# creare-com/pydem

Measured on AMD Instinct MI355X. Metric: Mcells/s (slope+aspect+UCA+TWI end-to-end) per tile; % HBM roofline, higher is better.
Workload: dtype f64

## Files before the change

include/pydem_hip.h:

```cpp
#ifndef PYDEM_HIP_H
#define PYDEM_HIP_H

#include <stdint.h>

#ifdef __cplusplus
extern "C" {
#endif

typedef struct pydem_tile pydem_tile;

enum pydem_field {
    PYDEM_ELEV = 0,
    PYDEM_MAG = 1,
    PYDEM_DIRECTION = 2,
    PYDEM_FLATS = 3,
    PYDEM_SECTION = 4,
    PYDEM_PROPORTION = 5,
    PYDEM_UCA = 6,
    PYDEM_TWI = 7,
    PYDEM_EDGE_TODO = 8,
    PYDEM_EDGE_DONE = 9,
    PYDEM_WEIGHT = 10,
    PYDEM_UCA_WEIGHTED = 11,
    PYDEM_FIELD_COUNT = 12
};

enum pydem_dtype { PYDEM_F64 = 0, PYDEM_F32 = 1, PYDEM_I16 = 2, PYDEM_I32 = 3, PYDEM_U8 = 4, PYDEM_I8 = 5 };

typedef struct pydem_options {
    int32_t drain_pits;
    int32_t drain_pits_min_border;
    int32_t drain_pits_max_iter;
    int32_t drain_pits_max_dist;
    double  drain_pits_max_dist_XY;
    int32_t apply_uca_limit_edges;
    int32_t apply_twi_limits;
    int32_t apply_twi_limits_on_uca;
    int32_t circular_ref_maxcount;
    double  uca_saturation_limit;
    double  twi_min_slope;
    double  twi_min_area;
} pydem_options;

typedef struct pydem_timings {
    double slopes_directions_ms;
    double stencil_kernel_ms;
    double flats_ms;
    double graph_ms;
    double pits_ms;
    double sweep_ms;
    double twi_ms;
    int64_t sweep_rounds;
    int64_t sweep_kernel_launches;
    int64_t n_flats;
    int64_t n_pit_edges;
    int64_t n_pits_undrained;
    int64_t n_unresolved;
    int64_t sweep_tile_passes;
    int64_t n_pits;
    int64_t n_pits_row;
    int64_t n_pits_wave;
    int64_t n_pits_big;
    double uca_weighted_ms;
} pydem_timings;

const char *pydem_hip_last_error(void);
int pydem_hip_device_count(int *count);
int pydem_hip_device_name(int device, char *buf, int buflen);
int pydem_hip_device_memory(int device, int64_t *free_bytes, int64_t *total_bytes);

int pydem_hip_release_scratch(void);

int pydem_tile_create(int64_t n_rows, int64_t n_cols, int device, pydem_tile **out);
int pydem_tile_destroy(pydem_tile *t);
int pydem_tile_set_spacing(pydem_tile *t, const double *dX, const double *dY,
                           const double *dX2, const double *dY2);
int pydem_tile_upload(pydem_tile *t, int field, const void *src, int dtype);
int pydem_tile_download(pydem_tile *t, int field, void *dst);
int pydem_tile_get_line(pydem_tile *t, int field, int axis, int64_t index, void *dst);
int pydem_tile_set_line(pydem_tile *t, int field, int axis, int64_t index, const void *src);
int pydem_tile_get_lines(pydem_tile *t, int count, const int *fields, const int *axes, const int64_t *indices,
                         void *const *dsts);
int pydem_tile_synchronize(pydem_tile *t);
int pydem_tile_timings(pydem_tile *t, pydem_timings *out);
int64_t pydem_tile_device_bytes(pydem_tile *t);

int pydem_tile_synth_fractal(pydem_tile *t, uint32_t seed, int64_t row0, int64_t col0,
                             int n_octaves, int top_shift, double zmin, double zrange);

int pydem_fill_flats(pydem_tile *t, double max_pit_area, int below_sea, double source_tol, int peaks, int pits, int artefacts_only,
                     int *needs_host);
int pydem_pit_candidates(pydem_tile *t, int below_sea, int64_t *npits);
int pydem_pit_candidates_read(pydem_tile *t, int64_t npits, int32_t *cells, double *elev);
int pydem_pit_paths(pydem_tile *t, const int32_t *order, int64_t npits, int max_iter, int max_dist, double max_dist_XY,
                    int64_t *n_failed, int64_t *iter_used, int64_t *rounds, int *needs_host);
int pydem_slopes_directions(pydem_tile *t);
int pydem_find_flats(pydem_tile *t);
int pydem_uca(pydem_tile *t, pydem_options *opt);
int pydem_uca_weighted(pydem_tile *t, pydem_options *opt, int scale_by_cell_area);
int pydem_build_graph(pydem_tile *t, pydem_options *opt);
int pydem_uca_edge_update(pydem_tile *t, pydem_options *opt,
                          const double *const data[4], const uint8_t *const done[4],
                          const uint8_t *const todo[4]);
int pydem_uca_edge_round_inc(pydem_tile *t, pydem_options *opt,
                             const double *const data[4], const uint8_t *const done[4],
                             const uint8_t *const todo[4]);
int pydem_uca_edge_round_inc_dev(pydem_tile *t, pydem_options *opt);
int pydem_uca_edge_flush(pydem_tile *t);
int pydem_twi(pydem_tile *t, pydem_options *opt);

int pydem_tile_pit_edges(pydem_tile *t, int64_t *n, int32_t *src, int32_t *dst, double *w);

int pydem_tile_graph_words(pydem_tile *t, uint32_t *out);

int pydem_tile_restore_pit_slopes(pydem_tile *t);

int pydem_bench_stencil(pydem_tile *t, int iters, double *avg_ms);

int pydem_drain_area(double *area, uint8_t *done, uint8_t *ids, const int32_t *col_indptr, const int32_t *col_indices,
                     const double *col_data, const int32_t *row_indptr, const int32_t *row_indices, int64_t n_rows,
                     int64_t n_cols, double *edge_todo, double *edge_todo_no_mask, int skip_edge, int device);
int pydem_drain_connections(uint8_t *arr, uint8_t *ids, const int32_t *indptr, const int32_t *indices, int64_t n,
                            uint8_t set_to, int device);

typedef struct pydem_comm pydem_comm;
int pydem_comm_unique_id(char *out128);
int pydem_comm_create(int world, int rank, const char *uid128, int device, pydem_comm **out);
int pydem_comm_destroy(pydem_comm *c);
int pydem_comm_begin(pydem_comm *c, int64_t n_doubles);
int pydem_comm_pack_line(pydem_comm *c, pydem_tile *t, int field, int axis, int64_t index, int64_t offset);
int pydem_comm_pack_lines(pydem_comm *c, pydem_tile *t, int count, const int *fields, const int *axes, const int64_t *indices,
                          const int64_t *offsets);
int pydem_comm_put(pydem_comm *c, const double *host_in, int64_t n_doubles, int64_t offset);
int pydem_comm_allreduce(pydem_comm *c, int64_t n_doubles, int op , double *host_out);

typedef struct pydem_board pydem_board;
int pydem_board_create(int device, int n_tiles, int64_t n_doubles, pydem_board **out);
int pydem_board_destroy(pydem_board *b);
int pydem_board_set_desc(pydem_board *b, int index, int32_t n, int32_t m, const int64_t *offsets28, const int32_t *flags8,
                         pydem_tile *tile);
int pydem_board_set_lines(pydem_board *b, int index, int64_t mb_start, int64_t size, pydem_tile *tile, int count,
                          const int *fields, const int *axes, const int64_t *indices, const int64_t *rel_offsets);
int pydem_board_refresh(pydem_board *b, pydem_comm *c, int n_wave, const int *wave_tiles);
int pydem_board_refresh_stage(pydem_board *b, int n_wave, const int *wave_tiles, double *host_out, int64_t cap, int64_t *n_doubles);
int pydem_board_refresh_unstage(pydem_board *b, int n_wave, const int *wave_tiles, const double *host_in, int64_t n_doubles);
int pydem_board_eval(pydem_board *b, int count, const int *tiles, const int *full, unsigned long long *out);
int pydem_board_run_waves(pydem_board *b, pydem_comm *c, int k_waves, unsigned long long *state, unsigned long long *scal_out);
typedef int (*pydem_exchange_fn)(void *ctx, int op, void *buf, int64_t n);
int pydem_board_prepare_waves(pydem_board *b, int staged, unsigned long long ok_tiles);
int pydem_board_run_waves_ex(pydem_board *b, pydem_comm *c, int k_waves, unsigned long long *state, unsigned long long *scal_out,
                             pydem_exchange_fn exchange, void *ctx);
int pydem_comm_count(pydem_comm *c, int *count);
int pydem_tile_edge_queue_ready(pydem_tile *t);
int pydem_board_download(pydem_board *b, double *out);

int pydem_cond_pit_artifacts(const double *elev, int64_t n_rows, int64_t n_cols, const int32_t *lab, int32_t nlab,
                             double max_area, int f32 , uint8_t *raise);
int pydem_cond_fill_flats(const double *data, double *built, int64_t n_rows, int64_t n_cols, const int32_t *lab,
                          int32_t nlab, double source_tol, int peaks, int pits);
int pydem_cond_pit_paths(double *elev, int64_t n_rows, int64_t n_cols, const int64_t *pits, int64_t npits,
                         const double *dX, int64_t n_dX, const double *dY, int max_iter, int max_dist,
                         double max_dist_XY, int dtype_mode ,
                         int64_t *n_failed, int64_t *iter_used);

int pydem_tiff_lzw_encode(const uint8_t *src, int64_t n, uint8_t *dst, int64_t cap, int64_t *out_n);

#ifdef __cplusplus
}
#endif
#endif
```

pydem_amd/_ffi.py:

```python
import ctypes as C
import os

import numpy as np

_HERE = os.path.dirname(os.path.abspath(__file__))
LIB_PATH = os.path.join(_HERE, 'lib', 'libpydem_hip.so')

ELEV, MAG, DIRECTION, FLATS, SECTION, PROPORTION, UCA, TWI, EDGE_TODO, EDGE_DONE, WEIGHT, UCA_WEIGHTED = range(12)
FIELD_DTYPE = {ELEV: np.float64, MAG: np.float64, DIRECTION: np.float64, FLATS: np.uint8,
               SECTION: np.int8, PROPORTION: np.float64, UCA: np.float64, TWI: np.float64,
               EDGE_TODO: np.uint8, EDGE_DONE: np.uint8, WEIGHT: np.float64, UCA_WEIGHTED: np.float64}
_DTYPES = {np.dtype('float64'): 0, np.dtype('float32'): 1, np.dtype('int16'): 2, np.dtype('int32'): 3,
           np.dtype('uint8'): 4, np.dtype('int8'): 5, np.dtype('bool'): 4}


class Options(C.Structure):
    _fields_ = [('drain_pits', C.c_int32), ('drain_pits_min_border', C.c_int32),
                ('drain_pits_max_iter', C.c_int32), ('drain_pits_max_dist', C.c_int32),
                ('drain_pits_max_dist_XY', C.c_double), ('apply_uca_limit_edges', C.c_int32),
                ('apply_twi_limits', C.c_int32), ('apply_twi_limits_on_uca', C.c_int32),
                ('circular_ref_maxcount', C.c_int32), ('uca_saturation_limit', C.c_double),
                ('twi_min_slope', C.c_double), ('twi_min_area', C.c_double)]


class Timings(C.Structure):
    _fields_ = [('slopes_directions_ms', C.c_double), ('stencil_kernel_ms', C.c_double),
                ('flats_ms', C.c_double), ('graph_ms', C.c_double), ('pits_ms', C.c_double),
                ('sweep_ms', C.c_double), ('twi_ms', C.c_double), ('sweep_rounds', C.c_int64),
                ('sweep_kernel_launches', C.c_int64), ('n_flats', C.c_int64), ('n_pit_edges', C.c_int64),
                ('n_pits_undrained', C.c_int64), ('n_unresolved', C.c_int64), ('sweep_tile_passes', C.c_int64),
                ('n_pits', C.c_int64), ('n_pits_row', C.c_int64), ('n_pits_wave', C.c_int64), ('n_pits_big', C.c_int64),
                ('uca_weighted_ms', C.c_double)]

    def as_dict(self):
        return {k: getattr(self, k) for k, _ in self._fields_}


_P = C.c_void_p
_PP = C.POINTER(C.c_void_p)
SYMBOLS = {
    'pydem_hip_last_error': (C.c_char_p, []),
    'pydem_hip_device_count': (C.c_int, [C.POINTER(C.c_int)]),
    'pydem_hip_device_memory': (C.c_int, [C.c_int, C.POINTER(C.c_int64), C.POINTER(C.c_int64)]),
    'pydem_hip_release_scratch': (C.c_int, []),
    'pydem_hip_device_name': (C.c_int, [C.c_int, C.c_char_p, C.c_int]),
    'pydem_tile_create': (C.c_int, [C.c_int64, C.c_int64, C.c_int, _PP]),
    'pydem_tile_destroy': (C.c_int, [_P]),
    'pydem_tile_set_spacing': (C.c_int, [_P, _P, _P, _P, _P]),
    'pydem_tile_upload': (C.c_int, [_P, C.c_int, _P, C.c_int]),
    'pydem_tile_download': (C.c_int, [_P, C.c_int, _P]),
    'pydem_tile_get_line': (C.c_int, [_P, C.c_int, C.c_int, C.c_int64, _P]),
    'pydem_tile_set_line': (C.c_int, [_P, C.c_int, C.c_int, C.c_int64, _P]),
    'pydem_tile_get_lines': (C.c_int, [_P, C.c_int, _P, _P, _P, _P]),
    'pydem_cond_pit_artifacts': (C.c_int, [_P, C.c_int64, C.c_int64, _P, C.c_int32, C.c_double, C.c_int, _P]),
    'pydem_cond_fill_flats': (C.c_int, [_P, _P, C.c_int64, C.c_int64, _P, C.c_int32, C.c_double, C.c_int, C.c_int]),
    'pydem_cond_pit_paths': (C.c_int, [_P, C.c_int64, C.c_int64, _P, C.c_int64, _P, C.c_int64, _P, C.c_int, C.c_int,
                                       C.c_double, C.c_int, _P, _P]),
    'pydem_tiff_lzw_encode': (C.c_int, [_P, C.c_int64, _P, C.c_int64, _P]),
    'pydem_tile_synchronize': (C.c_int, [_P]),
    'pydem_tile_timings': (C.c_int, [_P, C.POINTER(Timings)]),
    'pydem_tile_device_bytes': (C.c_int64, [_P]),
    'pydem_tile_synth_fractal': (C.c_int, [_P, C.c_uint32, C.c_int64, C.c_int64, C.c_int, C.c_int,
                                           C.c_double, C.c_double]),
    'pydem_fill_flats': (C.c_int, [_P, C.c_double, C.c_int, C.c_double, C.c_int, C.c_int, C.c_int, _P]),
    'pydem_pit_candidates': (C.c_int, [_P, C.c_int, C.POINTER(C.c_int64)]),
    'pydem_pit_candidates_read': (C.c_int, [_P, C.c_int64, _P, _P]),
    'pydem_pit_paths': (C.c_int, [_P, _P, C.c_int64, C.c_int, C.c_int, C.c_double, C.POINTER(C.c_int64), C.POINTER(C.c_int64), C.POINTER(C.c_int64), _P]),
    'pydem_slopes_directions': (C.c_int, [_P]),
    'pydem_find_flats': (C.c_int, [_P]),
    'pydem_uca': (C.c_int, [_P, C.POINTER(Options)]),
    'pydem_uca_weighted': (C.c_int, [_P, C.POINTER(Options), C.c_int]),
    'pydem_build_graph': (C.c_int, [_P, C.POINTER(Options)]),
    'pydem_uca_edge_update': (C.c_int, [_P, C.POINTER(Options), _PP, _PP, _PP]),
    'pydem_uca_edge_round_inc': (C.c_int, [_P, C.POINTER(Options), _PP, _PP, _PP]),
    'pydem_uca_edge_round_inc_dev': (C.c_int, [_P, C.POINTER(Options)]),
    'pydem_uca_edge_flush': (C.c_int, [_P]),
    'pydem_twi': (C.c_int, [_P, C.POINTER(Options)]),
    'pydem_tile_pit_edges': (C.c_int, [_P, C.POINTER(C.c_int64), _P, _P, _P]),
    'pydem_tile_graph_words': (C.c_int, [_P, _P]),
    'pydem_tile_restore_pit_slopes': (C.c_int, [_P]),
    'pydem_bench_stencil': (C.c_int, [_P, C.c_int, C.POINTER(C.c_double)]),
    'pydem_drain_area': (C.c_int, [_P, _P, _P, _P, _P, _P, _P, _P, C.c_int64, C.c_int64, _P, _P, C.c_int, C.c_int]),
    'pydem_drain_connections': (C.c_int, [_P, _P, _P, _P, C.c_int64, C.c_uint8, C.c_int]),
    'pydem_comm_unique_id': (C.c_int, [C.c_char_p]),
    'pydem_comm_create': (C.c_int, [C.c_int, C.c_int, C.c_char_p, C.c_int, _PP]),
    'pydem_comm_destroy': (C.c_int, [_P]),
    'pydem_comm_begin': (C.c_int, [_P, C.c_int64]),
    'pydem_comm_pack_line': (C.c_int, [_P, _P, C.c_int, C.c_int, C.c_int64, C.c_int64]),
    'pydem_comm_pack_lines': (C.c_int, [_P, _P, C.c_int, _P, _P, _P, _P]),
    'pydem_comm_put': (C.c_int, [_P, _P, C.c_int64, C.c_int64]),
    'pydem_comm_allreduce': (C.c_int, [_P, C.c_int64, C.c_int, _P]),
    'pydem_board_create': (C.c_int, [C.c_int, C.c_int, C.c_int64, _PP]),
    'pydem_board_destroy': (C.c_int, [_P]),
    'pydem_board_set_desc': (C.c_int, [_P, C.c_int, C.c_int32, C.c_int32, _P, _P, _P]),
    'pydem_board_set_lines': (C.c_int, [_P, C.c_int, C.c_int64, C.c_int64, _P, C.c_int, _P, _P, _P, _P]),
    'pydem_board_refresh': (C.c_int, [_P, _P, C.c_int, _P]),
    'pydem_board_refresh_stage': (C.c_int, [_P, C.c_int, _P, _P, C.c_int64, _P]),
    'pydem_board_refresh_unstage': (C.c_int, [_P, C.c_int, _P, _P, C.c_int64]),
    'pydem_board_eval': (C.c_int, [_P, C.c_int, _P, _P, _P]),
    'pydem_board_download': (C.c_int, [_P, _P]),
    'pydem_board_run_waves': (C.c_int, [_P, _P, C.c_int, _P, _P]),
    'pydem_board_prepare_waves': (C.c_int, [_P, C.c_int, C.c_uint64]),
    'pydem_board_run_waves_ex': (C.c_int, [_P, _P, C.c_int, _P, _P, _P, _P]),
    'pydem_comm_count': (C.c_int, [_P, _P]),
    'pydem_tile_edge_queue_ready': (C.c_int, [_P]),
}

_lib = None


def load():
    global _lib
    if _lib is None:
        if not os.path.exists(LIB_PATH):
            raise RuntimeError("libpydem_hip.so is not built (%s); run `python -m pydem_amd.build`. "
                               "There is no CPU fallback." % LIB_PATH)
        lib = C.CDLL(LIB_PATH)
        for name, (res, args) in SYMBOLS.items():
            fn = getattr(lib, name)
            fn.restype = res
            fn.argtypes = args
        _lib = lib
    return _lib


class HipError(RuntimeError):
    pass


def check(rc):
    if rc != 0:
        raise HipError("libpydem_hip error %d: %s" % (rc, load().pydem_hip_last_error().decode()))


def device_count():
    n = C.c_int(0)
    check(load().pydem_hip_device_count(C.byref(n)))
    return n.value


def release_scratch():
    check(load().pydem_hip_release_scratch())


def device_memory(device=0):
    f, tot = C.c_int64(0), C.c_int64(0)
    check(load().pydem_hip_device_memory(int(device), C.byref(f), C.byref(tot)))
    return f.value, tot.value


class Tile(object):

    def __init__(self, n_rows, n_cols, device=0):
        self.lib = load()
        self.shape = (int(n_rows), int(n_cols))
        self._h = C.c_void_p()
        check(self.lib.pydem_tile_create(n_rows, n_cols, device, C.byref(self._h)))

    def close(self):
        if self._h:
            self.lib.pydem_tile_destroy(self._h)
            self._h = C.c_void_p()

    def __del__(self):
        try:
            self.close()
        except Exception:
            pass

    def set_spacing(self, dX, dY, dX2, dY2):
        arrs = [np.ascontiguousarray(a, np.float64) for a in (dX, dY, dX2, dY2)]
        n = self.shape[0]
        assert arrs[0].size == n - 1 and arrs[1].size == n - 1 and arrs[2].size == n and arrs[3].size == n
        check(self.lib.pydem_tile_set_spacing(self._h, *[a.ctypes.data_as(_P) for a in arrs]))

    def upload(self, field, arr):
        arr = np.ascontiguousarray(arr)
        if arr.shape != self.shape:
            raise ValueError("field %d: array of shape %r uploaded to a tile of shape %r" % (field, arr.shape, self.shape))
        if FIELD_DTYPE[field] != np.float64:
            arr = np.ascontiguousarray(arr.astype(FIELD_DTYPE[field], copy=False))
            dt = _DTYPES[arr.dtype]
        else:
            if arr.dtype not in _DTYPES or arr.dtype == np.bool_:
                arr = np.ascontiguousarray(arr, np.float64)
            dt = _DTYPES[arr.dtype]
        check(self.lib.pydem_tile_upload(self._h, field, arr.ctypes.data_as(_P), dt))

    def download(self, field):
        out = np.empty(self.shape, FIELD_DTYPE[field])
        check(self.lib.pydem_tile_download(self._h, field, out.ctypes.data_as(_P)))
        return out

    def get_line(self, field, axis, index):
        out = np.empty(self.shape[1] if axis == 0 else self.shape[0], FIELD_DTYPE[field])
        check(self.lib.pydem_tile_get_line(self._h, field, axis, index, out.ctypes.data_as(_P)))
        return out

    def get_lines(self, requests):
        k = len(requests)
        outs = [np.empty(self.shape[1] if axis == 0 else self.shape[0], FIELD_DTYPE[field]) for field, axis, _ in requests]
        fields = (C.c_int * k)(*[r[0] for r in requests])
        axes = (C.c_int * k)(*[r[1] for r in requests])
        idx = (C.c_int64 * k)(*[r[2] for r in requests])
        dsts = (C.c_void_p * k)(*[o.ctypes.data for o in outs])
        check(self.lib.pydem_tile_get_lines(self._h, k, fields, axes, idx, dsts))
        return outs

    def set_line(self, field, axis, index, values):
        v = np.ascontiguousarray(values, FIELD_DTYPE[field])
        assert v.size == (self.shape[1] if axis == 0 else self.shape[0])
        check(self.lib.pydem_tile_set_line(self._h, field, axis, index, v.ctypes.data_as(_P)))

    def synth_fractal(self, seed=0, row0=0, col0=0, n_octaves=12, top_shift=12, zmin=1.0, zrange=1000.0):
        check(self.lib.pydem_tile_synth_fractal(self._h, seed, row0, col0, n_octaves, top_shift, zmin, zrange))

    def slopes_directions(self):
        check(self.lib.pydem_slopes_directions(self._h))

    def find_flats(self):
        check(self.lib.pydem_find_flats(self._h))

    def fill_flats(self, max_pit_area, below_sea, source_tol, peaks, pits, artefacts_only=False):
        flag = C.c_int(0)
        check(self.lib.pydem_fill_flats(self._h, float(max_pit_area or 0.0), int(bool(below_sea)), float(source_tol), int(bool(peaks)),
                                        int(bool(pits)), int(bool(artefacts_only)), C.byref(flag)))
        return flag.value == 0

    def pit_drain_paths(self, below_sea, max_iter, max_dist, max_dist_XY, sort_dtype=None):
        import time
        t0 = time.perf_counter()
        n = C.c_int64(0)
        check(self.lib.pydem_pit_candidates(self._h, int(bool(below_sea)), C.byref(n)))
        if n.value < 0:
            return None
        cells = np.empty(max(n.value, 1), np.int32); elev = np.empty(max(n.value, 1), np.float64)
        check(self.lib.pydem_pit_candidates_read(self._h, n.value, cells.ctypes.data_as(_P), elev.ctypes.data_as(_P)))
        cells, elev = cells[:n.value], elev[:n.value]
        t1 = time.perf_counter()
        keys = elev if sort_dtype is None or np.dtype(sort_dtype) == np.float64 else elev.astype(sort_dtype)
        order = np.ascontiguousarray(cells[np.argsort(keys)], np.int32)
        t2 = time.perf_counter()
        failed, used, rounds, flag = C.c_int64(0), C.c_int64(0), C.c_int64(0), C.c_int(0)
        check(self.lib.pydem_pit_paths(self._h, order.ctypes.data_as(_P), n.value, int(max_iter), int(max_dist or 0),
                                       float(max_dist_XY) if max_dist_XY else 0.0, C.byref(failed), C.byref(used), C.byref(rounds),
                                       C.byref(flag)))
        if os.environ.get('PYDEM_PATHS_DEBUG'):
            import sys
            sys.stderr.write("pit paths host side: candidates %.1f ms, argsort %.1f ms, pydem_pit_paths %.1f ms\n"
                             % ((t1 - t0) * 1e3, (t2 - t1) * 1e3, (time.perf_counter() - t2) * 1e3))
        if flag.value:
            return None
        return int(failed.value), int(used.value), int(rounds.value)

    def uca(self, opt):
        check(self.lib.pydem_uca(self._h, C.byref(opt)))

    def uca_weighted(self, opt, scale_by_cell_area=True):
        check(self.lib.pydem_uca_weighted(self._h, C.byref(opt), int(bool(scale_by_cell_area))))

    def build_graph(self, opt):
        check(self.lib.pydem_build_graph(self._h, C.byref(opt)))

    def uca_edge_update(self, opt, data, done, todo, incremental=False):
        n, m = self.shape
        lens = (n, n, m, m)
        d = [np.ascontiguousarray(np.asarray(a, np.float64).ravel()) for a in data]
        dn = [np.ascontiguousarray(np.asarray(a).ravel().astype(np.uint8)) for a in done]
        td = [np.ascontiguousarray(np.asarray(a).ravel().astype(np.uint8)) for a in todo]
        for arrs in (d, dn, td):
            assert [a.size for a in arrs] == list(lens), "edge strips must have n_rows / n_cols entries"
        pack = lambda xs: (C.c_void_p * 4)(*[x.ctypes.data_as(C.c_void_p) for x in xs])
        fn = self.lib.pydem_uca_edge_round_inc if incremental else self.lib.pydem_uca_edge_update
        check(fn(self._h, C.byref(opt), pack(d), pack(dn), pack(td)))

    def uca_edge_flush(self):
        check(self.lib.pydem_uca_edge_flush(self._h))

    def edge_queue_ready(self):
        return bool(self.lib.pydem_tile_edge_queue_ready(self._h))

    def uca_edge_round_dev(self, opt):
        check(self.lib.pydem_uca_edge_round_inc_dev(self._h, C.byref(opt)))

    def twi(self, opt):
        check(self.lib.pydem_twi(self._h, C.byref(opt)))

    def graph_words(self):
        out = np.empty(self.shape, np.uint32)
        check(self.lib.pydem_tile_graph_words(self._h, out.ctypes.data_as(_P)))
        return out

    def pit_edges(self):
        n = C.c_int64(0)
        check(self.lib.pydem_tile_pit_edges(self._h, C.byref(n), None, None, None))
        src = np.empty(n.value, np.int32); dst = np.empty(n.value, np.int32); w = np.empty(n.value, np.float64)
        if n.value:
            check(self.lib.pydem_tile_pit_edges(self._h, C.byref(n), src.ctypes.data_as(_P), dst.ctypes.data_as(_P),
                                                w.ctypes.data_as(_P)))
        return src, dst, w

    def restore_pit_slopes(self):
        check(self.lib.pydem_tile_restore_pit_slopes(self._h))

    def bench_stencil(self, iters):
        ms = C.c_double(0)
        check(self.lib.pydem_bench_stencil(self._h, iters, C.byref(ms)))
        return ms.value

    def synchronize(self):
        check(self.lib.pydem_tile_synchronize(self._h))

    def timings(self):
        tm = Timings()
        check(self.lib.pydem_tile_timings(self._h, C.byref(tm)))
        return tm.as_dict()

    def device_bytes(self):
        return self.lib.pydem_tile_device_bytes(self._h)


class Board(object):

    def __init__(self, device, n_tiles, n_doubles):
        self.lib = load()
        self.n_tiles, self.n_doubles = n_tiles, n_doubles
        self._h = C.c_void_p()
        check(self.lib.pydem_board_create(device, n_tiles, n_doubles, C.byref(self._h)))
        self._out = np.zeros((n_tiles, 8), np.uint64)

    def close(self):
        if self._h:
            self.lib.pydem_board_destroy(self._h)
            self._h = C.c_void_p()

# ... 124 lines not shown
```

pydem_amd/csrc/ccl.h:

```cpp
#pragma once

#define RLX_LOAD(p) __hip_atomic_load((p), __ATOMIC_RELAXED, __HIP_MEMORY_SCOPE_AGENT)

__global__ __launch_bounds__(256) void k_compact_flats(const uint8_t *__restrict__ flat0, int64_t NN,
                                                       int32_t *__restrict__ list, int32_t *__restrict__ count)
{
    __shared__ int32_t wave_tot[4][4];
    __shared__ int32_t blk_base;
    const int lane = threadIdx.x & 63, wave = threadIdx.x >> 6;
    for (int64_t base = (int64_t)blockIdx.x * 65536; base < NN; base += (int64_t)gridDim.x * 65536) {
        unsigned long long bits[4];
        int32_t mine[4], incl[4];
#pragma unroll
        for (int j = 0; j < 4; j++) {
            const int64_t c0 = base + j * 16384 + (int64_t)threadIdx.x * 64;
            bits[j] = 0;
            if (c0 + 64 <= NN) {
                uint4 v[4];
#pragma unroll
                for (int q = 0; q < 4; q++) v[q] = *reinterpret_cast<const uint4 *>(flat0 + c0 + 16 * q);
#pragma unroll
                for (int q = 0; q < 4; q++) {
                    const uint32_t w[4] = {v[q].x, v[q].y, v[q].z, v[q].w};
#pragma unroll
                    for (int k = 0; k < 16; k++)
                        bits[j] |= (unsigned long long)(((w[k >> 2] >> (8 * (k & 3))) & 0xffu) ? 1u : 0u) << (16 * q + k);
                }
            } else {
                for (int k = 0; k < 64; k++)
                    if (c0 + k < NN && flat0[c0 + k]) bits[j] |= 1ull << k;
            }
            mine[j] = __popcll(bits[j]);
            incl[j] = mine[j];
#pragma unroll
            for (int off = 1; off < 64; off <<= 1) {
                const int32_t o = __shfl_up(incl[j], off);
                if (lane >= off) incl[j] += o;
            }
            if (lane == 63) wave_tot[j][wave] = incl[j];
        }
        __syncthreads();
        if (threadIdx.x == 0) {
            int32_t tot = 0;
            for (int j = 0; j < 4; j++) for (int k = 0; k < 4; k++) tot += wave_tot[j][k];
            blk_base = tot ? atomicAdd(count, tot) : 0;
        }
        __syncthreads();
        int32_t off = blk_base;
#pragma unroll
        for (int j = 0; j < 4; j++) {
            int32_t o = off + incl[j] - mine[j];
            for (int k = 0; k < wave; k++) o += wave_tot[j][k];
            const int64_t c0 = base + j * 16384 + (int64_t)threadIdx.x * 64;
            unsigned long long b = bits[j];
            while (b) {
                const int k = __ffsll((long long)b) - 1;
                b &= b - 1;
                list[o++] = (int32_t)(c0 + k);
            }
            off += wave_tot[j][0] + wave_tot[j][1] + wave_tot[j][2] + wave_tot[j][3];
        }
        __syncthreads();
    }
}

__global__ void k_label_init(const int32_t *__restrict__ list, const int32_t *__restrict__ count, int32_t *labels, int m)
{
    const int32_t nf = *count;
    const int lane = threadIdx.x & 63;
    for (int32_t q = blockIdx.x * blockDim.x + threadIdx.x;; q += gridDim.x * blockDim.x) {
        const bool valid = q < nf;
        if (!__ballot(valid)) break;
        const int32_t c = valid ? list[q] : -1;
        const int32_t prev = __shfl_up(c, 1);
        const bool head = lane == 0 || !valid || prev != c - 1 || c % m == 0;
        const unsigned long long heads = __ballot(head);
        const int s = 63 - __clzll((long long)(heads & ((2ull << lane) - 1ull)));
        const int32_t start = __shfl(c, s);
        if (valid) labels[c] = start;
    }
}

__device__ __forceinline__ int32_t uf_find(int32_t *L, int32_t x)
{
    const int32_t x0 = x;
    int32_t p = RLX_LOAD(&L[x]);
    int hops = 0;
    while (p != x) { x = p; p = RLX_LOAD(&L[x]); hops++; }
    if (hops >= 2) atomicMin(&L[x0], x);
    return x;
}

__device__ __forceinline__ void uf_union(int32_t *L, int32_t a, int32_t b)
{
    for (;;) {
        a = uf_find(L, a);
        b = uf_find(L, b);
        if (a == b) return;
        if (a > b) { const int32_t t = a; a = b; b = t; }
        const int32_t old = atomicMin(&L[b], a);
        if (old == b) return;
        b = old;
    }
}

__global__ void k_label_union(const int32_t *__restrict__ list, const int32_t *__restrict__ count,
                              const uint8_t *__restrict__ flat0, int32_t *labels, int n, int m)
{
    const int32_t nf = *count;
    for (int32_t q = blockIdx.x * blockDim.x + threadIdx.x; q < nf; q += gridDim.x * blockDim.x) {
        const int32_t c = list[q];
        const int i = c / m, j = c - i * m;
        if (j + 1 < m && flat0[c + 1]) uf_union(labels, c, c + 1);
        if (i + 1 < n) {
            if (j > 0 && flat0[c + m - 1]) uf_union(labels, c, c + m - 1);
            if (flat0[c + m]) uf_union(labels, c, c + m);
            if (j + 1 < m && flat0[c + m + 1]) uf_union(labels, c, c + m + 1);
        }
    }
}

__global__ void k_label_flatten(const int32_t *__restrict__ list, const int32_t *__restrict__ count, int32_t *labels)
{
    const int32_t nf = *count;
    for (int32_t q = blockIdx.x * blockDim.x + threadIdx.x; q < nf; q += gridDim.x * blockDim.x) {
        const int32_t c = list[q];
        const int32_t r = uf_find(labels, c);
        if (r != c) __hip_atomic_store(&labels[c], r, __ATOMIC_RELAXED, __HIP_MEMORY_SCOPE_AGENT);
    }
}
```

pydem_amd/csrc/flats.hip:

```cpp
#include "internal.h"

namespace {

#include "ccl.h"

__global__ void k_flats_extend(const int32_t *__restrict__ list, const int32_t *__restrict__ count,
                               const uint8_t *__restrict__ flat0, const int32_t *__restrict__ labels,
                               const double *__restrict__ elev, uint8_t *__restrict__ flats, int n, int m)
{
    const int32_t nf = *count;
    for (int32_t q = blockIdx.x * blockDim.x + threadIdx.x; q < nf * 8; q += gridDim.x * blockDim.x) {
        const int32_t c = list[q >> 3];
        int d = q & 7;
        d += (d >= 4);
        const int i = c / m + d / 3 - 1, j = c % m + d % 3 - 1;
        if (i < 0 || i >= n || j < 0 || j >= m) continue;
        const int32_t J = i * m + j;
        if (!flat0[J] && !(elev[J] == elev[labels[c]])) continue;
        int32_t best = -1;
        for (int dd = 0; dd < 9; dd++) {
            if (dd == 4) continue;
            const int ii = i + dd / 3 - 1, jj = j + dd % 3 - 1;
            if (ii < 0 || ii >= n || jj < 0 || jj >= m) continue;
            const int32_t nb = ii * m + jj;
            if (flat0[nb]) { const int32_t r = labels[nb]; best = r > best ? r : best; }
        }
        flats[J] = (elev[J] == elev[best]);
    }
}

__global__ void k_flats_patch(const int32_t *__restrict__ list, const int32_t *__restrict__ count,
                              const uint8_t *__restrict__ flats, double *__restrict__ mag, double *__restrict__ dir,
                              int n, int m)
{
    const int32_t nf = *count;
    for (int32_t q = blockIdx.x * blockDim.x + threadIdx.x; q < nf * 9; q += gridDim.x * blockDim.x) {
        const int32_t c = list[q / 9];
        const int d = q % 9;
        const int i = c / m + d / 3 - 1, j = c % m + d % 3 - 1;
        if (i < 0 || i >= n || j < 0 || j >= m) continue;
        const int32_t J = i * m + j;
        if (flats[J]) { mag[J] = -1.0; dir[J] = -1.0; }
    }
}

__global__ __launch_bounds__(256) void k_count_flats(const uint8_t *__restrict__ flats, int64_t NN, int32_t *count)
{
    int32_t local = 0;
    const int64_t nvec = NN >> 4, stride = (int64_t)gridDim.x * blockDim.x, t0 = (int64_t)blockIdx.x * blockDim.x + threadIdx.x;
    for (int64_t v = t0; v < nvec; v += stride) {
        const uint4 f4 = reinterpret_cast<const uint4 *>(flats)[v];
        const uint32_t fw[4] = {f4.x, f4.y, f4.z, f4.w};
#pragma unroll
        for (int q = 0; q < 4; q++)
#pragma unroll
            for (int b = 0; b < 4; b++) local += ((fw[q] >> (8 * b)) & 0xFFu) != 0;
    }
    for (int64_t c = (nvec << 4) + t0; c < NN; c += stride) local += flats[c] != 0;
    for (int off = 32; off > 0; off >>= 1) local += __shfl_down(local, off);
    __shared__ int32_t s_w[4];
    if ((threadIdx.x & 63) == 0) s_w[threadIdx.x >> 6] = local;
    __syncthreads();
    if (threadIdx.x == 0) { const int32_t tot = s_w[0] + s_w[1] + s_w[2] + s_w[3]; if (tot) atomicAdd(count, tot); }
}

}

int stage_flats(pydem_tile *t)
{
    const int n = (int)t->n, m = (int)t->m;
    PYDEM_TRY(tile_alloc(t, &t->labels, (size_t)t->NN));
    PYDEM_TRY(tile_alloc(t, &t->flatlist, (size_t)t->NN));
    HIP_TRY(hipEventRecord(t->ev[3], t->stream));
    HIP_TRY(hipMemsetAsync(t->counters, 0, 64 * sizeof(int32_t), t->stream));
    int32_t *cnt = t->counters;
    const int big = (int)(cdiv(t->NN, 256) < 4096 ? cdiv(t->NN, 256) : 4096);
    hipLaunchKernelGGL(k_compact_flats, dim3(big), dim3(256), 0, t->stream, t->flat0, t->NN, t->flatlist, cnt);
    HIP_TRY(hipMemcpyAsync(t->flats, t->flat0, (size_t)t->NN, hipMemcpyDeviceToDevice, t->stream));
    HIP_TRY(hipMemcpyAsync(t->h_counters, cnt, sizeof(int32_t), hipMemcpyDeviceToHost, t->stream));
    HIP_TRY(hipStreamSynchronize(t->stream));
    const int32_t nf = t->h_counters[0];
    if (nf > 0) {
        const int g1 = (int)(cdiv(nf, 256) < 2048 ? cdiv(nf, 256) : 2048);
        const int g8 = (int)(cdiv((int64_t)nf * 9, 256) < 4096 ? cdiv((int64_t)nf * 9, 256) : 4096);
        hipLaunchKernelGGL(k_label_init, dim3(g1), dim3(256), 0, t->stream, t->flatlist, cnt, t->labels, m);
        hipLaunchKernelGGL(k_label_union, dim3(g1), dim3(256), 0, t->stream, t->flatlist, cnt, t->flat0, t->labels, n, m);
        hipLaunchKernelGGL(k_label_flatten, dim3(g1), dim3(256), 0, t->stream, t->flatlist, cnt, t->labels);
        hipLaunchKernelGGL(k_flats_extend, dim3(g8), dim3(256), 0, t->stream, t->flatlist, cnt, t->flat0, t->labels,
                           t->elev, t->flats, n, m);
        hipLaunchKernelGGL(k_flats_patch, dim3(g8), dim3(256), 0, t->stream, t->flatlist, cnt, t->flats, t->mag, t->dir, n, m);
    }
    hipLaunchKernelGGL(k_count_flats, dim3(big), dim3(256), 0, t->stream, t->flats, t->NN, cnt + 1);
    HIP_TRY(hipMemcpyAsync(t->h_counters, cnt, 2 * sizeof(int32_t), hipMemcpyDeviceToHost, t->stream));
    HIP_TRY(hipEventRecord(t->ev[4], t->stream));
    HIP_TRY(hipGetLastError());
    HIP_TRY(hipEventSynchronize(t->ev[4]));
    float ms = 0;
    HIP_TRY(hipEventElapsedTime(&ms, t->ev[3], t->ev[4]));
    t->tm.flats_ms = ms;
    t->tm.n_flats = t->h_counters[1];
    return 0;
}
```

pydem_amd/csrc/internal.h:

```cpp
#pragma once
#include <hip/hip_runtime.h>
#include <stdint.h>
#include <stdio.h>
#include <string>
#include <vector>
#include <utility>
#include <initializer_list>
#include "../../include/pydem_hip.h"

void pydem_set_error(const char *fmt, ...);
#define HIP_TRY(expr)                                                                          \
    do {                                                                                       \
        hipError_t e_ = (expr);                                                                \
        if (e_ != hipSuccess) {                                                                \
            pydem_set_error("%s:%d: %s -> %s", __FILE__, __LINE__, #expr, hipGetErrorString(e_)); \
            return -1;                                                                         \
        }                                                                                      \
    } while (0)
#define PYDEM_TRY(expr)            \
    do {                           \
        int r_ = (expr);           \
        if (r_ != 0) return r_;    \
    } while (0)

__host__ __device__ constexpr int fe1r(int k) { return k == 1 || k == 2 ? -1 : (k == 5 || k == 6 ? 1 : 0); }
__host__ __device__ constexpr int fe1c(int k) { return k == 0 || k == 7 ? 1 : (k == 3 || k == 4 ? -1 : 0); }
__host__ __device__ constexpr int fe2r(int k) { return k <= 3 ? -1 : 1; }
__host__ __device__ constexpr int fe2c(int k) { return (k == 0 || k == 1 || k == 6 || k == 7) ? 1 : -1; }

struct RowTab {
    double dX, dY;
    double hyp;
    double thA;
    double thB;
    double rdX, rdY, rhyp;
};

struct PitGraph {
    int32_t *raw_src = nullptr, *raw_dst = nullptr; double *raw_w = nullptr;
    int64_t raw_cap = 0, n_raw = 0;
    int64_t n_edges = 0, sorted_cap = 0;
    int32_t *src = nullptr, *dst = nullptr; double *w = nullptr;
    int32_t *in_src = nullptr, *in_dst = nullptr; double *in_w = nullptr;
    void *sort_buf = nullptr; size_t sort_bytes = 0;
};

struct pydem_tile {
    int64_t n = 0, m = 0, NN = 0;
    int device = 0;
    hipStream_t stream = nullptr;
    hipStream_t stream2 = nullptr;
    hipEvent_t ev_fork = nullptr, ev_join = nullptr, ev_snap = nullptr;
    hipEvent_t ev[8] = {};
    double *elev = nullptr, *mag = nullptr, *dir = nullptr, *prop = nullptr, *uca = nullptr, *twi = nullptr;
    double *weight = nullptr, *uca_w = nullptr;
    uint8_t *flats = nullptr, *edge_todo = nullptr, *edge_done = nullptr, *flat0 = nullptr;
    int8_t *section = nullptr;
    bool have[PYDEM_FIELD_COUNT] = {};
    double *dX = nullptr, *dY = nullptr, *dX2 = nullptr, *dY2 = nullptr;
    RowTab *rowtab = nullptr;
    double *sec_theta = nullptr;
    double *row_area = nullptr;
    std::vector<double> h_dX, h_dY, h_dX2, h_dY2;
    bool spacing_set = false;
    int stencil_exact_only = 0;
    bool elev_f32 = false;
    int elev_dtype = 0;
    uint8_t *inmask = nullptr, *gflags = nullptr, *todo_work = nullptr;
    double *contrib = nullptr;
    int32_t *indeg = nullptr, *queue[2] = {nullptr, nullptr}, *labels = nullptr, *flatlist = nullptr;
    int32_t *counters = nullptr;
    int32_t *h_counters = nullptr;
    PitGraph pits;
    int32_t *estamp = nullptr; double *edelta = nullptr, *p_delta = nullptr, *s_data = nullptr;
    uint8_t *p_flags = nullptr, *s_flags = nullptr;
    int32_t eepoch = 0;
    int32_t *eseed = nullptr;
    bool edge_clean = false;
    bool einc_compact = false;
    void *nd_rec = nullptr; int64_t nd_cap = 0; int32_t nd = 0;
    int64_t circular_cells = -1;
    int64_t einc_round = 0;
    bool einc_ready = false;
    std::vector<std::pair<int, int64_t>> watch;
    size_t watch_built = 0;
    bool cond_live = false;
    bool cond_pending = false;
    int32_t cond_nw = 0, cond_nan_cap = 0;
    void *cond_mem = nullptr; size_t cond_bytes = 0;
    void *cond_node = nullptr, *cond_edge = nullptr; double *cond_slot = nullptr;
    int32_t *cond_q0 = nullptr, *cond_q1 = nullptr, *cond_nanq = nullptr, *cond_cnt = nullptr;
    void *cb_mem[3] = {nullptr, nullptr, nullptr}; size_t cb_bytes[3] = {0, 0, 0};
    double *h_strip_d = nullptr; uint8_t *h_strip_f = nullptr; size_t h_strip_cap = 0;
    void *h_stage = nullptr; size_t h_stage_bytes = 0;
    int32_t etodo_prev = 0;
    double *line_stage = nullptr;
    void *lines_stage = nullptr; int lines_cap = 0;
    bool graph_valid = false;
    pydem_options graph_opt = {};
    void *scratch = nullptr; size_t scratch_bytes = 0;
    int64_t device_bytes = 0;
    pydem_timings tm = {};
};

template <typename T>
int tile_alloc(pydem_tile *t, T **p, size_t count);

struct ArenaLease {
    int device = -1;
    void *arena = nullptr;
    char *base = nullptr; size_t bytes = 0, off = 0, want = 0;
    std::vector<void *> extra;
    bool held = false;
    ~ArenaLease();
};
int arena_acquire(int device, ArenaLease *L);
void *arena_take(ArenaLease *L, size_t bytes);

int ensure_fields(pydem_tile *t, std::initializer_list<int> fields);
void *plane_take(int device, size_t bytes);
void plane_give(int device, void *q);
hipError_t dev_malloc(void **p, size_t bytes);
int tile_pinned(pydem_tile *t, size_t bytes, void **out);

int stage_stencil(pydem_tile *t);
int stage_flats(pydem_tile *t);
int stage_section_graph(pydem_tile *t, const pydem_options *opt);
int stage_pits(pydem_tile *t, const pydem_options *opt);
int stage_sweep(pydem_tile *t, const pydem_options *opt);
int stage_uca_weighted(pydem_tile *t, const pydem_options *opt, int scale_by_cell_area);
int stage_twi(pydem_tile *t, const pydem_options *opt);
int stage_edge_update(pydem_tile *t, const pydem_options *opt, const double *const data[4], const uint8_t *const done[4],
                      const uint8_t *const todo[4]);
int stage_edge_round_inc(pydem_tile *t, const pydem_options *opt, const double *const data[4], const uint8_t *const done[4],
                         const uint8_t *const todo[4]);
int stage_edge_flush(pydem_tile *t);
int stage_edge_catchup(pydem_tile *t);
bool tile_edge_queue_ready(const pydem_tile *t);
size_t tile_edge_queue_desc_bytes();
int tile_edge_queue_desc(pydem_tile *t, void *out, const unsigned long long *gate, int bit, const unsigned long long *round_base,
                         const unsigned long long *round_add, int64_t *nper);
int stage_edge_rounds_queued(hipStream_t s, const void *d_q, int count, int64_t max_nper);
unsigned long long tile_edge_round_counter(const pydem_tile *t);
void tile_edge_rounds_ran(pydem_tile *t, int waves);
void tile_watch_line(pydem_tile *t, int axis, int64_t index);
bool tile_line_watched(const pydem_tile *t, int axis, int64_t index);
int stage_fill_flats(pydem_tile *t, double max_pit_area, int below_sea, double source_tol, int peaks, int pits, int artefacts_only);
int stage_pit_candidates(pydem_tile *t, int below_sea, int64_t *npits);
int stage_pit_candidates_read(pydem_tile *t, int64_t npits, int32_t *cells, double *elev);
int stage_pit_paths(pydem_tile *t, const int32_t *order_host, int64_t npits, int max_iter, int max_dist, double max_dist_XY,
                    int64_t *n_failed, int64_t *iter_used, int64_t *rounds_out, int dtype_mode);
int stage_synth(pydem_tile *t, uint32_t seed, int64_t row0, int64_t col0, int n_oct, int top_shift,
                double zmin, double zrange);
int bench_stencil(pydem_tile *t, int iters, double *avg_ms);

static inline int64_t cdiv(int64_t a, int64_t b) { return (a + b - 1) / b; }
```

pydem_amd/csrc/pits.hip:

```cpp
#include "internal.h"
#include <hipcub/hipcub.hpp>
#include <math.h>
#include <stdlib.h>
#include <algorithm>
#include <vector>

namespace {

__device__ __forceinline__ double np_pairwise_leaf(const double *a, int n)
{
    if (n < 8) {
        double res = 0.;
        for (int i = 0; i < n; i++) res += a[i];
        return res;
    }
    double r0 = a[0], r1 = a[1], r2 = a[2], r3 = a[3], r4 = a[4], r5 = a[5], r6 = a[6], r7 = a[7];
    int i;
    for (i = 8; i < n - (n % 8); i += 8) {
        r0 += a[i]; r1 += a[i + 1]; r2 += a[i + 2]; r3 += a[i + 3];
        r4 += a[i + 4]; r5 += a[i + 5]; r6 += a[i + 6]; r7 += a[i + 7];
    }
    double res = ((r0 + r1) + (r2 + r3)) + ((r4 + r5) + (r6 + r7));
    for (; i < n; i++) res += a[i];
    return res;
// ... 733 lines not shown
            const bool in_a = (pos >> 5) == wa;
            const uint32_t wd = in_a ? va : vb;
            if (wd & bit) continue;
            if (nb == LN_B) { over = true; continue; }
            if (in_a) va |= bit; else vb |= bit;
            if (wb == wa) vb = va;
            lp[nb * LN_T] = (uint8_t)pos;
            nb++;
        }
        seen[wa * LN_T] = va;
        if (wb != wa) seen[wb * LN_T] = vb;
    };
    auto fetch_new = [&](int nb0) {
        constexpr int FB = 8;
        for (int base = nb0; base < nb; base += FB) {
            double e8[FB]; uint8_t pm8[FB];
#pragma unroll
            for (int k = 0; k < FB; k++) {
                e8[k] = 0.0; pm8[k] = 0;
                if (base + k < nb) {
                    const int pos = lp[(base + k) * LN_T];
                    const int64_t cell = (int64_t)(r0 + (pos >> 4)) * m + (c0 + (pos & 15));
                    e8[k] = P.elev[cell]; pm8[k] = P.pitmask[cell];
                }
            }
#pragma unroll
            for (int k = 0; k < FB; k++) {
                const int idx = base + k;
                if (idx >= nb) continue;
                le[idx * LN_T] = e8[k];
                if (e8[k] != e8[k]) has_nan = true;
                if (pm8[k]) { pitbits |= 1u << idx; if (e8[k] < epit) has_p = true; }
                else { pitbits &= ~(1u << idx); if (e8[k] < epit_border) has_np = true; }
            }
        }
    };
    const bool prof = P.prof != nullptr;
    long long acc_a = 0, acc_b = 0, acc_c = 0, acc_g = 0, trips = 0, busy = 0;
    for (;;) {
        long long tk0 = 0, tk1 = 0, tk2 = 0, tkg = 0;
        if (prof) tk0 = clock64();
        const unsigned long long idle = __ballot(!running);
        if (idle && more) {
            if (chunk_next == chunk_end) {
                int32_t b = 0;
                if (lane == 0) b = atomicAdd(P.work_next, LN_CHUNK);
                b = __shfl(b, 0);
                chunk_next = b < np ? b : np;
                chunk_end = b + LN_CHUNK < np ? b + LN_CHUNK : np;
                if (chunk_next >= chunk_end) more = false;
            }
            const int avail = chunk_end - chunk_next, want = __popcll(idle);
            const int rank = __popcll(idle & lt);
            if (!running && rank < avail) {
                pit = pits[chunk_next + rank];
                ipit = pit / m; jpit = pit - ipit * m;
                r0 = ipit - LN_W / 2; c0 = jpit - LN_W / 2;
                if (r0 > n - LN_W) r0 = n - LN_W;
                if (c0 > m - LN_W) c0 = m - LN_W;
                if (r0 < 0) r0 = 0;
                if (c0 < 0) c0 = 0;
#pragma unroll
                for (int w = 0; w < 8; w++) seen[w * LN_T] = 0;
                epit = P.elev[pit];
                epit_border = epit;
                nb = 0; pitbits = 0; it = 0;
                has_np = false; has_p = false; has_nan = false; over = false;
                {
                    const int pos = (ipit - r0) * LN_W + (jpit - c0);
                    seen[(pos >> 5) * LN_T] = 1u << (pos & 31);
                    discover(ipit - r0, jpit - c0);
                    fetch_new(0);
                }
                if (P.min_border) {
                    double mn = INFINITY;
                    for (int k = 0; k < nb; k++) mn = min_f64(mn, le[k * LN_T]);
                    if (nb) epit_border = mn;
                    has_np = false;
                }
                running = true;
            }
            chunk_next += want < avail ? want : avail;
        }
        if (!__ballot(running)) { if (more) continue; break; }
        if (prof) { tk1 = clock64(); busy += __popcll(__ballot(running)); trips++; }
        int nd = 0;
        int status = 0;
        double ssum = 0.0;
        if (running && !pending) {
            if (over) pending = 4;
            else if (it >= P.max_iter || nb == 0) pending = 3;
            else if (has_nan) pending = has_p ? 2 : 3;
            else if (has_np) pending = 1;
            else if (has_p) pending = 2;
            else {
                double mn = INFINITY;
                for (int k0 = 0; k0 < nb; k0 += 8) {
                    double v[8];
#pragma unroll
                    for (int i = 0; i < 8; i++) v[i] = k0 + i < nb ? le[(k0 + i) * LN_T] : INFINITY;
#pragma unroll
                    for (int i = 0; i < 8; i++) mn = min_f64(mn, v[i]);
                }
                uint32_t eq = 0;
                for (int k0 = 0; k0 < nb; k0 += 8) {
                    double v[8];
#pragma unroll
                    for (int i = 0; i < 8; i++) v[i] = k0 + i < nb ? le[(k0 + i) * LN_T] : INFINITY;
#pragma unroll
                    for (int i = 0; i < 8; i++) if (k0 + i < nb && v[i] == mn) eq |= 1u << (k0 + i);
                }
                int nq = 0;
                while (eq) {
                    const int k = 31 - __clz((int)eq);
                    eq &= ~(1u << k);
                    lq[nq * LN_T] = lp[k * LN_T]; nq++;
                    nb--;
                    if (k != nb) {
                        le[k * LN_T] = le[nb * LN_T]; lp[k * LN_T] = lp[nb * LN_T];
                        pitbits = (pitbits & ~(1u << k)) | (((pitbits >> nb) & 1u) << k);
                    }
                }
                const int nb0 = nb;
                for (int j = 0; j < nq; j++) { const int pos = lq[j * LN_T]; discover(pos >> 4, pos & 15); }
                fetch_new(nb0);
                it++;
            }
        }
        const unsigned long long waiting = __ballot(pending != 0), growing = __ballot(running && !pending);
        if (prof) { tkg = clock64(); acc_g += tkg - tk1; }
        if (!(__popcll(waiting) >= LN_FIN_BATCH || (waiting && !growing))) continue;
        if (pending) {
            const int mode = pending <= 2 ? pending : 0;
            status = pending == 4 ? 3 : 2;
            if (mode) {
                uint32_t mt = 0;
                for (int k0 = 0; k0 < nb; k0 += 8) {
                    double v[8];
#pragma unroll
                    for (int i = 0; i < 8; i++) v[i] = k0 + i < nb ? le[(k0 + i) * LN_T] : INFINITY;
#pragma unroll
                    for (int i = 0; i < 8; i++) {
                        const bool isp = (pitbits >> (k0 + i)) & 1u;
                        if (k0 + i < nb && (mode == 1 ? (!isp && v[i] < epit_border) : (isp && v[i] < epit))) mt |= 1u << (k0 + i);
                    }
                }
                while (mt) {
                    const int k = __ffs((int)mt) - 1;
                    mt &= mt - 1u;
                    if (k != nd) {
                        const double ek = le[k * LN_T], en = le[nd * LN_T];
                        const uint8_t pk = lp[k * LN_T], pn = lp[nd * LN_T];
                        const uint32_t bk = (pitbits >> k) & 1u, bn = (pitbits >> nd) & 1u;
                        le[k * LN_T] = en; lp[k * LN_T] = pn; le[nd * LN_T] = ek; lp[nd * LN_T] = pk;
                        pitbits = (pitbits & ~((1u << k) | (1u << nd))) | (bn << k) | (bk << nd);
                    }
                    nd++;
                }
                for (int a = 1; a < nd; a++) {
                    const double ea = le[a * LN_T]; const uint8_t pa = lp[a * LN_T]; const uint32_t ba = (pitbits >> a) & 1u;
                    int b = a - 1;
                    while (b >= 0 && lp[b * LN_T] > pa) {
                        le[(b + 1) * LN_T] = le[b * LN_T]; lp[(b + 1) * LN_T] = lp[b * LN_T];
                        pitbits = (pitbits & ~(1u << (b + 1))) | (((pitbits >> b) & 1u) << (b + 1));
                        b--;
                    }
                    le[(b + 1) * LN_T] = ea; lp[(b + 1) * LN_T] = pa;
                    pitbits = (pitbits & ~(1u << (b + 1))) | (ba << (b + 1));
                }
                const int ndX = n - 1;
                const bool xy = !isnan(P.max_dist_XY) && P.max_dist_XY != 0;
                int keep = 0;
                for (int t = 0; t < nd; t++) {
                    const int pos = lp[t * LN_T];
                    const int idr = r0 + (pos >> 4), jdr = c0 + (pos & 15);
                    if (P.max_dist) {
                        const int di = ipit - idr, dj = jpit - jdr;
                        if (!(sqrt((double)(di * di + dj * dj)) <= (double)P.max_dist)) continue;
                    }
                    const int a = ipit < idr ? ipit : idr, b = ipit < idr ? idr : ipit;
                    double dxm;
                    if (ipit == idr) dxm = P.dX[ipit < ndX - 1 ? ipit : ndX - 1];
                    else dxm = np_pairwise_leaf15(P.dX + a, b - a) / (double)(b - a);
                    const double dx = dxm * (double)(jpit - jdr);
                    const double dy = np_pairwise_leaf15(P.dY + a, b - a);
                    const double d = sqrt(dx * dx + dy * dy);
                    if (xy && !(d <= P.max_dist_XY)) continue;
                    le[keep * LN_T] = pit_drop(P, epit, le[t * LN_T]) / d;
                    lp[keep * LN_T] = (uint8_t)pos;
                    keep++;
                }
                nd = keep;
                if (nd > 0) {
                    ssum = np_pairwise_leaf_strided(le, LN_T, nd);
                    P.mag[pit] = ssum / (double)nd;
                    P.flats[pit] = 0;
                    status = 1;
                }
            }
            running = false; pending = 0;
        }
        if (prof) { tk2 = clock64(); acc_a += tk1 - tk0; acc_b += tk2 - tkg; }
        if (!__ballot(status != 0)) continue;
        int incl = nd;
        for (int off = 1; off < 64; off <<= 1) { const int o = __shfl_up(incl, off); if (lane >= off) incl += o; }
        const int tot = __shfl(incl, 63);
        int32_t wbase = 0;
        if (lane == 0 && tot) wbase = atomicAdd(&P.out_count[0], tot);
        wbase = __shfl(wbase, 0);
        if (tot) {
            if ((int64_t)wbase + tot <= P.out_cap) {
                const int32_t o = wbase + incl - nd;
                for (int t = 0; t < nd; t++) {
                    const int pos = lp[t * LN_T];
                    P.out_src[o + t] = pit;
                    P.out_dst[o + t] = (int32_t)((int64_t)(r0 + (pos >> 4)) * m + (c0 + (pos & 15)));
                    P.out_w[o + t] = le[t * LN_T] / ssum;
                }
            } else if (lane == 0) atomicAdd(&P.out_count[3], 1);
        }
        const unsigned long long b_un = __ballot(status == 2), b_ov = __ballot(status == 3);
        if (lane == 0 && b_un) atomicAdd(&P.out_count[1], __popcll(b_un));
        if (b_ov) {
            int32_t obase = 0;
            if (lane == 0) obase = atomicAdd(&P.out_count[4], __popcll(b_ov));
            obase = __shfl(obase, 0);
            if (status == 3) {
                const int32_t slot = obase + __popcll(b_ov & lt);
                P.lane_overflow[slot] = pit;
                if (P.lane_state) {
                for (int k = 0; k < nb; k++) { const int pos = lp[k * LN_T]; seen[(pos >> 5) * LN_T] &= ~(1u << (pos & 31)); }
                uint32_t *rec = P.lane_state + (size_t)slot * 12;
                rec[0] = (uint32_t)it; rec[1] = 0;
                rec[2] = (uint32_t)__double2loint(epit_border); rec[3] = (uint32_t)__double2hiint(epit_border);
#pragma unroll
                for (int w = 0; w < 8; w++) rec[4 + w] = seen[w * LN_T];
                }
            }
        }
        if (prof) acc_c += clock64() - tk2;
    }
    if (prof && lane == 0) {
        atomicAdd(P.prof + 0, (unsigned long long)acc_a); atomicAdd(P.prof + 1, (unsigned long long)acc_b);
        atomicAdd(P.prof + 2, (unsigned long long)acc_c); atomicAdd(P.prof + 3, (unsigned long long)busy);
        atomicAdd(P.prof + 4, (unsigned long long)trips); atomicAdd(P.prof + 5, (unsigned long long)acc_g);
    }
}

constexpr int W_LARGE = 640, MAXD_LARGE = 2048;

template <int CAP, int OCC>
__global__ __launch_bounds__(256, OCC) void k_pits_wave(PitParams P, const int32_t *__restrict__ pits, const int32_t *npits)
{
    __shared__ WaveLds<128, CAP, uint16_t> s_l[4];
    const int wave = threadIdx.x >> 6, lane = threadIdx.x & 63;
    const int32_t np = *npits;
    int32_t chunk_base = 0, chunk_left = 0;
    for (;;) {
        int32_t q = 0;
        if (lane == 0) q = atomicAdd(P.work_next, 1);
        q = __shfl(q, 0);
        if (q >= np) break;
        if (P.wave_index) q = P.wave_index[q];
        solve_pit_wave(P, pits[q], lane, s_l[wave], chunk_base, chunk_left, P.lane_state ? P.lane_state + (size_t)q * 12 : nullptr);
        wave_sync();
    }
}

__global__ __launch_bounds__(64) void k_pits_wave_big(PitParams P, const int32_t *__restrict__ pits, const int32_t *npits)
{
    __shared__ WaveLds<256, 2048, uint32_t> s_l;
    const int lane = threadIdx.x;
    const int32_t np = *npits;
    int32_t chunk_base = 0, chunk_left = 0;
    for (int32_t q = blockIdx.x; q < np; q += gridDim.x) {
        solve_pit_wave(P, pits[q], lane, s_l, chunk_base, chunk_left);
        wave_sync();
    }
}

#ifndef PYDEM_BLOCK_NT
#define PYDEM_BLOCK_NT 512
#endif
constexpr int BLOCK_NT = PYDEM_BLOCK_NT;
__global__ __launch_bounds__(BLOCK_NT) void k_pits_block(PitParams P, const int32_t *__restrict__ pits, const int32_t *npits,
                                                    int32_t *g_dl, double *g_dxy, double *g_sv, int maxd)
{
    constexpr int WORDS = W_LARGE * W_LARGE / 32;
    extern __shared__ __attribute__((aligned(16))) uint32_t dyn[];
    __shared__ double redd[BLOCK_NT / 64];
    __shared__ int redi[BLOCK_NT / 64];
    __shared__ int flag[4];
    __shared__ PwFrame stk[16];
    int32_t chunk_base = 0, chunk_left = 0;
    const int32_t np = *npits;
    for (int32_t q = blockIdx.x; q < np; q += gridDim.x) {
        solve_pit<BLOCK_NT, W_LARGE>(P, pits[q], threadIdx.x, dyn, dyn + WORDS, dyn + 2 * WORDS,
                                     g_dl + (size_t)blockIdx.x * maxd, g_dxy + (size_t)blockIdx.x * maxd,
                                     g_sv + (size_t)blockIdx.x * maxd, redd, redi, flag, chunk_base, chunk_left, stk, maxd);
        __syncthreads();
    }
}

__global__ void k_pitmask(const uint8_t *__restrict__ flats, const double *__restrict__ elev, int64_t NN, uint8_t *pitmask)
{
    const int64_t nvec = NN >> 4, stride = (int64_t)gridDim.x * blockDim.x, t0 = (int64_t)blockIdx.x * blockDim.x + threadIdx.x;
    for (int64_t v = t0; v < nvec; v += stride) {
        const uint4 f4 = reinterpret_cast<const uint4 *>(flats)[v];
        const uint32_t fw[4] = {f4.x, f4.y, f4.z, f4.w};
        uint32_t pw[4];
#pragma unroll
        for (int q = 0; q < 4; q++) {
            uint32_t p = 0;
            if (fw[q])
#pragma unroll
                for (int b = 0; b < 4; b++)
                    if (((fw[q] >> (8 * b)) & 0xFFu) && elev[v * 16 + q * 4 + b] > 0) p |= 1u << (8 * b);
            pw[q] = p;
        }
        reinterpret_cast<uint4 *>(pitmask)[v] = make_uint4(pw[0], pw[1], pw[2], pw[3]);
    }
    for (int64_t c = (nvec << 4) + t0; c < NN; c += stride) pitmask[c] = flats[c] && (elev[c] > 0);
}

__global__ __launch_bounds__(256) void k_compact_mask(const uint8_t *__restrict__ mask, int64_t NN,
                                                       int32_t *__restrict__ list, int32_t *__restrict__ count)
{
    __shared__ int32_t wave_tot[4][4];
    __shared__ int32_t blk_base;
    const int lane = threadIdx.x & 63, wave = threadIdx.x >> 6;
    for (int64_t base = (int64_t)blockIdx.x * 65536; base < NN; base += (int64_t)gridDim.x * 65536) {
        unsigned long long bits[4];
        int32_t mine[4], incl[4];
#pragma unroll
        for (int j = 0; j < 4; j++) {
            const int64_t c0 = base + j * 16384 + (int64_t)threadIdx.x * 64;
            bits[j] = 0;
            if (c0 + 64 <= NN) {
                uint4 v[4];
#pragma unroll
                for (int q = 0; q < 4; q++) v[q] = *reinterpret_cast<const uint4 *>(mask + c0 + 16 * q);
#pragma unroll
                for (int q = 0; q < 4; q++) {
                    const uint32_t w[4] = {v[q].x, v[q].y, v[q].z, v[q].w};
#pragma unroll
                    for (int k = 0; k < 16; k++)
                        bits[j] |= (unsigned long long)(((w[k >> 2] >> (8 * (k & 3))) & 0xffu) ? 1u : 0u) << (16 * q + k);
                }
            } else {
                for (int k = 0; k < 64; k++)
                    if (c0 + k < NN && mask[c0 + k]) bits[j] |= 1ull << k;
            }
            mine[j] = __popcll(bits[j]);
            incl[j] = mine[j];
#pragma unroll
            for (int off = 1; off < 64; off <<= 1) {
                const int32_t o = __shfl_up(incl[j], off);
                if (lane >= off) incl[j] += o;
            }
            if (lane == 63) wave_tot[j][wave] = incl[j];
        }
        __syncthreads();
        if (threadIdx.x == 0) {
            int32_t tot = 0;
            for (int j = 0; j < 4; j++) for (int k = 0; k < 4; k++) tot += wave_tot[j][k];
            blk_base = tot ? atomicAdd(count, tot) : 0;
        }
        __syncthreads();
        int32_t off = blk_base;
#pragma unroll
        for (int j = 0; j < 4; j++) {
            int32_t o = off + incl[j] - mine[j];
            for (int k = 0; k < wave; k++) o += wave_tot[j][k];
            const int64_t c0 = base + j * 16384 + (int64_t)threadIdx.x * 64;
            unsigned long long b = bits[j];
            while (b) {
                const int k = __ffsll((long long)b) - 1;
                b &= b - 1;
                list[o++] = (int32_t)(c0 + k);
            }
            off += wave_tot[j][0] + wave_tot[j][1] + wave_tot[j][2] + wave_tot[j][3];
        }
        __syncthreads();
    }
}

__global__ __launch_bounds__(256) void k_pit_keys(const int32_t *__restrict__ src, const int32_t *__restrict__ dst, const double *__restrict__ w,
                                                  const double *__restrict__ elev, int32_t ne, uint64_t *key_out, uint64_t *key_in, int32_t *idx,
                                                  int32_t *count, int kb)
{
    constexpr int PER = 4;
    __shared__ int32_t wave_tot[4];
    __shared__ int32_t blk_base;
    const int lane = threadIdx.x & 63, wave = threadIdx.x >> 6;
    for (int64_t base = (int64_t)blockIdx.x * (256 * PER); base < ne; base += (int64_t)gridDim.x * (256 * PER)) {
        uint32_t keep = 0;
        int32_t sv[PER], dv[PER];
#pragma unroll
        for (int j = 0; j < PER; j++) {
            const int64_t e = base + j * 256 + threadIdx.x;
            sv[j] = -1; dv[j] = 0;
            if (e < ne) { sv[j] = src[e]; dv[j] = dst[e]; }
        }
#pragma unroll
        for (int j = 0; j < PER; j++) {
            const int64_t e = base + j * 256 + threadIdx.x;
            if (sv[j] >= 0) {
                const double we = w[e];
                if (!isnan(we) && we > 1e-8 && elev[dv[j]] <= elev[sv[j]]) keep |= 1u << j;
            }
        }
        const int32_t mine = __popc(keep);
        int32_t incl = mine;
#pragma unroll
        for (int off = 1; off < 64; off <<= 1) { const int32_t o = __shfl_up(incl, off); if (lane >= off) incl += o; }
        if (lane == 63) wave_tot[wave] = incl;
        __syncthreads();
        if (threadIdx.x == 0) {
            const int32_t tot = wave_tot[0] + wave_tot[1] + wave_tot[2] + wave_tot[3];
            blk_base = tot ? atomicAdd(count, tot) : 0;
        }
        __syncthreads();
        int32_t o = blk_base + incl - mine;
        for (int k = 0; k < wave; k++) o += wave_tot[k];
#pragma unroll
        for (int j = 0; j < PER; j++)
            if (keep & (1u << j)) {
                key_out[o] = ((uint64_t)(uint32_t)sv[j] << kb) | (uint32_t)dv[j];
                key_in[o] = ((uint64_t)(uint32_t)dv[j] << kb) | (uint32_t)sv[j];
                idx[o] = (int32_t)(base + j * 256 + threadIdx.x);
                o++;
            }
        __syncthreads();
    }
}

__global__ void k_pit_gather(const uint64_t *__restrict__ keys, const int32_t *__restrict__ idx, const double *__restrict__ w,
                             int32_t ne, int swap, int32_t *a, int32_t *b, double *wo, int32_t *dup, int kb)
{
    for (int32_t e = blockIdx.x * blockDim.x + threadIdx.x; e < ne; e += gridDim.x * blockDim.x) {
        const uint64_t k = keys[e];
        if (dup && e > 0 && keys[e - 1] == k) atomicAdd(dup, 1);
        const int32_t hi = (int32_t)(k >> kb), lo = (int32_t)(k & ((1ull << kb) - 1ull));
        a[e] = swap ? lo : hi;
        b[e] = swap ? hi : lo;
        wo[e] = w[idx[e]];
    }
}

template <typename T>
int dev_realloc(pydem_tile *t, T **p, size_t count)
{
    if (*p) { plane_give(t->device, *p); *p = nullptr; }
    return tile_alloc(t, p, count);
}

}

int stage_pits(pydem_tile *t, const pydem_options *opt)
{
    const int n = (int)t->n, m = (int)t->m;
    if (opt->drain_pits_max_iter > 300) {
        pydem_set_error("drain_pits_max_iter > 300 is not supported by the device window (got %d)", opt->drain_pits_max_iter);
        return -2;
    }
    HIP_TRY(hipEventRecord(t->ev[4], t->stream));
    PYDEM_TRY(tile_alloc(t, &t->flat0, (size_t)t->NN));
    PYDEM_TRY(tile_alloc(t, &t->flatlist, (size_t)t->NN));
    PYDEM_TRY(tile_alloc(t, &t->labels, (size_t)t->NN));
    PYDEM_TRY(tile_alloc(t, &t->queue[0], (size_t)t->NN));
    int32_t *cnt = t->counters + 40;
    HIP_TRY(hipMemsetAsync(cnt, 0, 16 * sizeof(int32_t), t->stream));
    const int big = (int)(cdiv(t->NN, 256) < 8192 ? cdiv(t->NN, 256) : 8192);
    hipLaunchKernelGGL(k_pitmask, dim3(big), dim3(256), 0, t->stream, t->flats, t->elev, t->NN, t->flat0);
    hipLaunchKernelGGL(k_compact_mask, dim3((unsigned)(cdiv(t->NN, 4096) < 4096 ? cdiv(t->NN, 4096) : 4096)), dim3(256), 0,
                       t->stream, t->flat0, t->NN, t->flatlist, cnt);
    HIP_TRY(hipMemcpyAsync(t->h_counters, cnt, sizeof(int32_t), hipMemcpyDeviceToHost, t->stream));
    HIP_TRY(hipStreamSynchronize(t->stream));
    const int32_t npits = t->h_counters[0];
    t->tm.n_pit_edges = 0; t->tm.n_pits_undrained = 0;
    t->tm.n_pits = npits; t->tm.n_pits_row = 0; t->tm.n_pits_wave = 0; t->tm.n_pits_big = 0;
    t->pits.n_edges = 0;
    if (npits == 0) { t->tm.pits_ms = 0; return 0; }

    int64_t cap = (int64_t)npits * 2 + 16384 * 4 * OUT_CHUNK + 1024;
    for (int attempt = 0;; attempt++) {
        if (t->pits.raw_cap < cap) {
            PYDEM_TRY(dev_realloc(t, &t->pits.raw_src, (size_t)cap));
            PYDEM_TRY(dev_realloc(t, &t->pits.raw_dst, (size_t)cap));
            PYDEM_TRY(dev_realloc(t, &t->pits.raw_w, (size_t)cap));
            t->pits.raw_cap = cap;
        }
        HIP_TRY(hipMemsetAsync(cnt + 1, 0, 8 * sizeof(int32_t), t->stream));
        PitParams P;
        P.dbg = nullptr; P.prof = nullptr;
        const char *dbg_env = getenv("PYDEM_PITS_DEBUG");
        if (dbg_env && atoi(dbg_env) == 3) { HIP_TRY(hipMalloc(&P.prof, 128)); HIP_TRY(hipMemsetAsync(P.prof, 0, 128, t->stream)); }
        if (dbg_env && atoi(dbg_env) >= 2) HIP_TRY(hipMalloc(&P.dbg, (size_t)npits * 16));
        HIP_TRY(hipMemsetAsync(t->pits.raw_src, 0xFF, (size_t)t->pits.raw_cap * 4, t->stream));
        P.elev = t->elev; P.pitmask = t->flat0; P.dX = t->dX; P.dY = t->dY; P.mag = t->mag; P.flats = t->flats;
        P.n = n; P.m = m; P.max_iter = opt->drain_pits_max_iter; P.max_dist = opt->drain_pits_max_dist;
        P.min_border = opt->drain_pits_min_border; P.max_dist_XY = opt->drain_pits_max_dist_XY;
        P.elev_f32 = t->elev_f32 ? 1 : 0;
        P.out_src = t->pits.raw_src; P.out_dst = t->pits.raw_dst; P.out_w = t->pits.raw_w;
        P.out_count = cnt + 1; P.out_cap = (int32_t)(t->pits.raw_cap < INT32_MAX ? t->pits.raw_cap : INT32_MAX);
        P.overflow_list = t->labels; P.overflow_count = cnt + 3;
        P.lane_overflow = t->queue[0];
        {
            static int handover = -1;
            if (handover < 0) { const char *e = getenv("PYDEM_PITS_HANDOVER"); handover = e ? atoi(e) : 1; }
            P.lane_state = nullptr;
            if (handover && (int64_t)npits * 12 <= t->NN) { PYDEM_TRY(tile_alloc(t, &t->queue[1], (size_t)t->NN)); P.lane_state = (uint32_t *)t->queue[1]; }
        }
        HIP_TRY(hipMemsetAsync(cnt + 10, 0, sizeof(int32_t), t->stream));
        P.work_next = cnt + 10;
        const int gl_cap = 3072 * 128 / LN_T;
        const int gl = (int)(cdiv(npits, LN_T) < gl_cap ? cdiv(npits, LN_T) : gl_cap);
        hipLaunchKernelGGL(k_pits_lane, dim3(gl), dim3(LN_T), 0, t->stream, P, t->flatlist, cnt);
        HIP_TRY(hipMemcpyAsync(t->h_counters, cnt, 8 * sizeof(int32_t), hipMemcpyDeviceToHost, t->stream));
        HIP_TRY(hipStreamSynchronize(t->stream));
        const int32_t n_lane_over = t->h_counters[5];
        if (P.prof) {
            unsigned long long h[8];
            HIP_TRY(hipMemcpy(h, P.prof, 64, hipMemcpyDeviceToHost));
            fprintf(stderr, "pits/lane: %llu loop trips over all wavefronts, %.1f busy lanes per trip; cycles: refill %llu, growth %llu, drain selection %llu, output %llu\n",
                    h[4], h[4] ? (double)h[3] / (double)h[4] : 0.0, h[0], h[5], h[1], h[2]);
        }
        int32_t n_row_over = -1, n_wave_over = 0, n_over = 0;
        P.wave_index = nullptr; P.row_overflow = nullptr; P.row_overflow_count = nullptr; P.row_rec = nullptr; P.rw_target = PYDEM_RW_TARGET;
        const char *row_env = getenv("PYDEM_PITS_ROW");
        const int row_mode = row_env ? atoi(row_env) : 1;
        const bool use_row = row_mode == 2 || (row_mode == 1 && n_lane_over >= 4 * 256 * PYDEM_WV_OCC);
        if (use_row && n_lane_over > 0 && 8 * (int64_t)n_lane_over + 64 <= t->NN) {
            HIP_TRY(hipMemsetAsync(cnt + 9, 0, 4 * sizeof(int32_t), t->stream));
            P.row_overflow = t->labels; P.row_overflow_count = cnt + 12;
            P.row_rec = (int2 *)(t->labels + (((size_t)t->NN / 2) & ~(size_t)63));
            const char *tgt_env = getenv("PYDEM_RW_TARGET");
            P.rw_target = tgt_env && atoi(tgt_env) > 0 ? atoi(tgt_env) : PYDEM_RW_TARGET;
            constexpr int per = RW_NT / 16, gr_cap = 256 * (RW_OCC * 256 / RW_NT);
            const int gr = (int)(cdiv(n_lane_over, per) < gr_cap ? cdiv(n_lane_over, per) : gr_cap);
            hipLaunchKernelGGL((k_pits_row<RW_CAP, RW_OCC, RW_NT>), dim3(gr), dim3(RW_NT), 0, t->stream, P, t->queue[0], cnt + 5);
            hipLaunchKernelGGL(k_pits_row_finish, dim3((unsigned)(cdiv(n_lane_over, 256) < 2048 ? cdiv(n_lane_over, 256) : 2048)), dim3(256), 0,
                               t->stream, P, t->queue[0], cnt + 5, P.row_rec);
            if (P.prof) {
                unsigned long long h[16];
                HIP_TRY(hipMemcpy(h, P.prof, 128, hipMemcpyDeviceToHost));
                fprintf(stderr, "pits/row: %llu loop trips over all wavefronts, %.2f busy / %.2f growing rows per trip, %llu refills; cycles: refill %llu, rounds %llu, drain selection %llu, output %llu\n",
                        h[12], h[12] ? (double)h[13] / (double)h[12] : 0.0, h[12] ? (double)h[14] / (double)h[12] : 0.0, h[15], h[8], h[9], h[10], h[11]);
            }
            P.wave_index = t->labels;
            P.overflow_list = t->labels + (((size_t)n_lane_over + 63) & ~(size_t)63);
            HIP_TRY(hipMemsetAsync(cnt + 10, 0, sizeof(int32_t), t->stream));
            const int gw = (int)(cdiv(n_lane_over, 4) < 256 * 4 ? cdiv(n_lane_over, 4) : 256 * 4);
            hipLaunchKernelGGL((k_pits_wave<512, 4>), dim3(gw), dim3(256), 0, t->stream, P, t->queue[0], cnt + 12);
            const int32_t *big_in = P.overflow_list;
            P.overflow_list = t->queue[0]; P.overflow_count = cnt + 9;
            P.wave_index = nullptr;
            hipLaunchKernelGGL(k_pits_wave_big, dim3(256), dim3(64), 0, t->stream, P, big_in, cnt + 3);
            HIP_TRY(hipMemcpyAsync(t->h_counters, cnt, 16 * sizeof(int32_t), hipMemcpyDeviceToHost, t->stream));
            HIP_TRY(hipStreamSynchronize(t->stream));
            n_row_over = t->h_counters[12]; n_wave_over = t->h_counters[3]; n_over = t->h_counters[9];
        } else {
            if (n_lane_over > 0) {
                const int gw = (int)(cdiv(n_lane_over, 4) < 256 * PYDEM_WV_OCC ? cdiv(n_lane_over, 4) : 256 * PYDEM_WV_OCC);
                HIP_TRY(hipMemsetAsync(cnt + 10, 0, sizeof(int32_t), t->stream));
                hipLaunchKernelGGL((k_pits_wave<PYDEM_WV_CAP, PYDEM_WV_OCC>), dim3(gw), dim3(256), 0, t->stream, P, t->queue[0], cnt + 5);
                HIP_TRY(hipMemcpyAsync(t->h_counters, cnt, 8 * sizeof(int32_t), hipMemcpyDeviceToHost, t->stream));
                HIP_TRY(hipStreamSynchronize(t->stream));
            }
            n_wave_over = t->h_counters[3];
            if (n_wave_over > 0) {
                HIP_TRY(hipMemsetAsync(cnt + 9, 0, sizeof(int32_t), t->stream));
                P.overflow_list = t->queue[0]; P.overflow_count = cnt + 9;
                hipLaunchKernelGGL(k_pits_wave_big, dim3(n_wave_over < 4096 ? n_wave_over : 4096), dim3(64), 0, t->stream, P, t->labels, cnt + 3);
                HIP_TRY(hipMemcpyAsync(t->h_counters, cnt, 16 * sizeof(int32_t), hipMemcpyDeviceToHost, t->stream));
                HIP_TRY(hipStreamSynchronize(t->stream));
                n_over = t->h_counters[9];
            }
        }
        if (P.prof) { (void)hipFree(P.prof); P.prof = nullptr; }
        t->tm.n_pits_row = n_row_over >= 0 ? n_lane_over : 0;
        t->tm.n_pits_wave = n_row_over >= 0 ? n_row_over : n_lane_over;
        t->tm.n_pits_big = n_wave_over;
        if (dbg_env) fprintf(stderr, "pits: %d candidates, %d left the 16x16 lane window, %d left the 64x64 row pass (-1: not run), %d left the 128x128 wavefront pass, %d left the 256x256 / 2048-cell pass, %d edge slots, %d undrained\n", npits, n_lane_over, n_row_over, n_wave_over, n_over, t->h_counters[1], t->h_counters[2]);
        if (P.dbg) {
            const int nrec = t->h_counters[7];
            std::vector<int32_t> rec((size_t)nrec * 4);
            HIP_TRY(hipMemcpy(rec.data(), P.dbg, rec.size() * 4, hipMemcpyDeviceToHost));
            (void)hipFree(P.dbg); P.dbg = nullptr;
            std::vector<int> rounds, border; int reason[4] = {0, 0, 0, 0}; long long tot_rounds = 0;
            for (int i = 0; i < nrec; i++) {
                rounds.push_back(rec[4 * i]); border.push_back(rec[4 * i + 1]); reason[rec[4 * i + 2] & 3]++; tot_rounds += rec[4 * i];
            }
            {
                const int edges[7] = {16, 32, 64, 128, 200, 299, 1 << 30};
                long long cr[7] = {0}, cn[7] = {0}, cd[7] = {0}, cu[7] = {0}, co[7] = {0};
                for (int i = 0; i < nrec; i++) {
                    int b = 0; while (rec[4 * i] > edges[b]) b++;
                    cr[b] += rec[4 * i]; cn[b]++;
                    if (rec[4 * i + 2] & 3) co[b]++; else if (rec[4 * i + 3] >= 0) cd[b]++; else cu[b]++;
                }
                for (int b = 0; b < 7; b++)
                    fprintf(stderr, "pits/wave: rounds <= %d: %lld pits, %lld rounds (%.1f %%); %lld drain, %lld end without a drain, %lld handed on\n",
                            edges[b] == (1 << 30) ? 300 : edges[b], cn[b], cr[b], 100.0 * cr[b] / (tot_rounds ? tot_rounds : 1), cd[b], cu[b], co[b]);
            }
            std::sort(rounds.begin(), rounds.end()); std::sort(border.begin(), border.end());
            auto pct = [&](std::vector<int> &v, double q) { return v.empty() ? 0 : v[(size_t)(q * (v.size() - 1))]; };
            fprintf(stderr, "pits/wave: %d pits, %lld rounds; rounds p50 %d p90 %d p99 %d max %d; last border p50 %d p90 %d p99 %d max %d; "
                    "ok %d, window exit %d, border cap %d, drain cap %d\n", nrec, tot_rounds, pct(rounds, .5), pct(rounds, .9),
                    pct(rounds, .99), pct(rounds, 1.), pct(border, .5), pct(border, .9), pct(border, .99), pct(border, 1.),
                    reason[0], reason[1], reason[2], reason[3]);
        }
        if (n_over > 0) {
            const int gb = n_over < 1024 ? n_over : 1024;
            const size_t dyn = (size_t)3 * W_LARGE * W_LARGE / 8;
            HIP_TRY(hipFuncSetAttribute((const void *)k_pits_block, hipFuncAttributeMaxDynamicSharedMemorySize, (int)dyn));
            auto launch_block = [&](int blocks, int maxd, const int32_t *list, const int32_t *count) -> int {
                const size_t need = (size_t)blocks * maxd * (4 + 8 + 8);
                if (t->scratch_bytes < need) {
                    if (t->scratch) { HIP_TRY(hipFree(t->scratch)); t->device_bytes -= (int64_t)t->scratch_bytes; }
                    HIP_TRY(dev_malloc((void **)&t->scratch, need));
                    t->scratch_bytes = need; t->device_bytes += (int64_t)need;
                }
                double *g_dxy = (double *)t->scratch;
                double *g_sv = g_dxy + (size_t)blocks * maxd;
                int32_t *g_dl = (int32_t *)(g_sv + (size_t)blocks * maxd);
                hipLaunchKernelGGL(k_pits_block, dim3(blocks), dim3(BLOCK_NT), dyn, t->stream, P, list, count, g_dl, g_dxy, g_sv, maxd);
                HIP_TRY(hipMemcpyAsync(t->h_counters, cnt, 16 * sizeof(int32_t), hipMemcpyDeviceToHost, t->stream));
                HIP_TRY(hipStreamSynchronize(t->stream));
                return 0;
            };
            HIP_TRY(hipMemsetAsync(cnt + 13, 0, sizeof(int32_t), t->stream));
            P.overflow_list = t->labels; P.overflow_count = cnt + 13;
            PYDEM_TRY(launch_block(gb, MAXD_LARGE, t->queue[0], cnt + 9));
            const int32_t n_retry = t->h_counters[13];
            P.overflow_list = nullptr; P.overflow_count = nullptr;
            if (n_retry > 0) PYDEM_TRY(launch_block(n_retry < 4 ? n_retry : 4, W_LARGE * W_LARGE, t->labels, cnt + 13));
            if (dbg_env) fprintf(stderr, "pits: %d pits with more than %d drains solved again with room for %d\n", n_retry, MAXD_LARGE, W_LARGE * W_LARGE);
        }
        HIP_TRY(hipGetLastError());
        const int64_t ne = t->h_counters[1];
        if (t->h_counters[4] > 0 && ne <= t->pits.raw_cap) {
            pydem_set_error("pit->drain: %d pits exceeded the device window/drain capacity", t->h_counters[4]);
            return -5;
        }
        if (ne > t->pits.raw_cap) {
            if (attempt > 3) { pydem_set_error("pit edge buffer keeps overflowing"); return -5; }
            cap = ne + 1024;
            continue;
        }
        t->pits.n_raw = ne;
        t->tm.n_pits_undrained = t->h_counters[2];
        break;
    }
    const int32_t ne = (int32_t)t->pits.n_raw;
    t->tm.n_pit_edges = ne;
    if (ne > 0) {
        if (t->pits.sorted_cap < ne) {
            const size_t sc = ((size_t)ne + 65535) & ~(size_t)65535;
            PYDEM_TRY(dev_realloc(t, &t->pits.src, sc)); PYDEM_TRY(dev_realloc(t, &t->pits.dst, sc));
            PYDEM_TRY(dev_realloc(t, &t->pits.w, sc)); PYDEM_TRY(dev_realloc(t, &t->pits.in_src, sc));
            PYDEM_TRY(dev_realloc(t, &t->pits.in_dst, sc)); PYDEM_TRY(dev_realloc(t, &t->pits.in_w, sc));
            t->pits.sorted_cap = (int64_t)sc;
        }
        size_t tmp_bytes = 0;
        HIP_TRY(hipcub::DeviceRadixSort::SortPairs(nullptr, tmp_bytes, (uint64_t *)nullptr, (uint64_t *)nullptr, (int32_t *)nullptr,
                                                   (int32_t *)nullptr, ne, 0, 64, t->stream));
        const size_t ne8 = ((size_t)ne * 8 + 255) & ~(size_t)255, ne4 = ((size_t)ne * 4 + 255) & ~(size_t)255;
        const size_t tmp_al = (tmp_bytes + 255) & ~(size_t)255;
        const size_t need_sort = 4 * ne8 + 3 * ne4 + 2 * tmp_al + 256;
        if (t->pits.sort_bytes < need_sort) {
            if (t->pits.sort_buf) { HIP_TRY(hipFree(t->pits.sort_buf)); t->device_bytes -= (int64_t)t->pits.sort_bytes; }
            HIP_TRY(dev_malloc((void **)&t->pits.sort_buf, need_sort + need_sort / 4));
            t->pits.sort_bytes = need_sort + need_sort / 4; t->device_bytes += (int64_t)t->pits.sort_bytes;
        }
        char *sb = (char *)t->pits.sort_buf;
        uint64_t *k1 = (uint64_t *)sb, *k2 = (uint64_t *)(sb + ne8), *k1s = (uint64_t *)(sb + 2 * ne8), *k2s = (uint64_t *)(sb + 3 * ne8);
        int32_t *idx = (int32_t *)(sb + 4 * ne8), *i1 = (int32_t *)(sb + 4 * ne8 + ne4), *i2 = (int32_t *)(sb + 4 * ne8 + 2 * ne4);
        void *tmp = sb + 4 * ne8 + 3 * ne4;
        int kb = 1;
        while (((int64_t)1 << kb) < t->NN) kb++;
        HIP_TRY(hipMemsetAsync(cnt + 10, 0, sizeof(int32_t), t->stream));
        hipLaunchKernelGGL(k_pit_keys, dim3((unsigned)(cdiv(ne, 1024) < 8192 ? cdiv(ne, 1024) : 8192)), dim3(256), 0, t->stream, t->pits.raw_src,
                           t->pits.raw_dst, t->pits.raw_w, t->elev, ne, k1, k2, idx, cnt + 10, kb);
        HIP_TRY(hipMemcpyAsync(t->h_counters, cnt + 10, sizeof(int32_t), hipMemcpyDeviceToHost, t->stream));
        HIP_TRY(hipStreamSynchronize(t->stream));
        const int32_t nk = t->h_counters[0];
        if (nk > 0) {
            const int g = (int)(cdiv(nk, 256) < 1024 ? cdiv(nk, 256) : 1024);
            void *tmp2 = (char *)tmp + tmp_al;
            HIP_TRY(hipcub::DeviceRadixSort::SortPairs(tmp2, tmp_bytes, k2, k2s, idx, i2, nk, 0, 2 * kb, t->stream2));
            hipLaunchKernelGGL(k_pit_gather, dim3(g), dim3(256), 0, t->stream2, k2s, i2, t->pits.raw_w, nk, 1, t->pits.in_src,
                               t->pits.in_dst, t->pits.in_w, (int32_t *)nullptr, kb);
            HIP_TRY(hipEventRecord(t->ev_snap, t->stream2));
            HIP_TRY(hipcub::DeviceRadixSort::SortPairs(tmp, tmp_bytes, k1, k1s, idx, i1, nk, 0, 2 * kb, t->stream));
            HIP_TRY(hipMemsetAsync(cnt + 11, 0, sizeof(int32_t), t->stream));
            hipLaunchKernelGGL(k_pit_gather, dim3(g), dim3(256), 0, t->stream, k1s, i1, t->pits.raw_w, nk, 0, t->pits.src, t->pits.dst,
                               t->pits.w, cnt + 11, kb);
            HIP_TRY(hipStreamWaitEvent(t->stream, t->ev_snap, 0));
            HIP_TRY(hipMemcpyAsync(t->h_counters, cnt + 11, sizeof(int32_t), hipMemcpyDeviceToHost, t->stream));
            HIP_TRY(hipStreamSynchronize(t->stream));
            if (t->h_counters[0] != 0) { pydem_set_error("pit search: %d duplicate pit -> drain edges", t->h_counters[0]); return -5; }
        }
        HIP_TRY(hipGetLastError());
        t->pits.n_edges = nk;
        t->tm.n_pit_edges = nk;
    }
    HIP_TRY(hipEventRecord(t->ev[5], t->stream));
    HIP_TRY(hipEventSynchronize(t->ev[5]));
    float ms = 0;
    HIP_TRY(hipEventElapsedTime(&ms, t->ev[4], t->ev[5]));
    t->tm.pits_ms = ms;
    return 0;
}
```

pydem_amd/csrc/tile.hip:

```cpp
#include "internal.h"
#include <cmath>
#include <math.h>
#include <stdarg.h>
#include <string.h>
#include <stdlib.h>

static thread_local char g_err[1024] = "";

void pydem_set_error(const char *fmt, ...)
{
    va_list ap;
    va_start(ap, fmt);
    vsnprintf(g_err, sizeof(g_err), fmt, ap);
    va_end(ap);
}

#include <map>
#include <mutex>
#include <unordered_map>
namespace {
struct FreeBlock { void *p; uint64_t stamp; };
struct PlaneCache {
    std::mutex mu;
    std::multimap<size_t, FreeBlock> free_blocks;
    uint64_t clock = 0;
    std::unordered_map<void *, size_t> live;
    size_t kept = 0;
};
std::mutex g_pc_table;
std::map<int, PlaneCache *> g_pc;
PlaneCache *plane_cache(int device)
{
    std::lock_guard<std::mutex> g(g_pc_table);
    PlaneCache *&c = g_pc[device];
    if (!c) c = new PlaneCache();
    return c;
}
size_t plane_cache_limit()
{
    static const size_t lim = [] {
        const char *e = getenv("PYDEM_PLANE_CACHE_GB");
        const double gb = e ? atof(e) : 32.0;
        return (size_t)((gb > 0.0 ? gb : 0.0) * (double)((size_t)1 << 30));
    }();
    return lim;
}
void plane_cache_evict(PlaneCache *c, size_t room, std::vector<void *> &victims)
{
    const size_t lim = plane_cache_limit();
    while (!c->free_blocks.empty() && c->kept + room > lim) {
        auto old = c->free_blocks.begin();
        for (auto it = c->free_blocks.begin(); it != c->free_blocks.end(); ++it) if (it->second.stamp < old->second.stamp) old = it;
        victims.push_back(old->second.p);
        c->kept -= old->first;
        c->free_blocks.erase(old);
    }
}
constexpr size_t PLANE_MIN = (size_t)1 << 20;
void plane_cache_flush(int device)
{
    PlaneCache *c = plane_cache(device);
    std::lock_guard<std::mutex> g(c->mu);
    for (auto &kv : c->free_blocks) (void)hipFree(kv.second.p);
    c->free_blocks.clear(); c->kept = 0;
}
}

void *plane_take(int device, size_t bytes)
{
    std::vector<void *> victims;
    if (bytes >= PLANE_MIN && plane_cache_limit()) {
        PlaneCache *c = plane_cache(device);
        std::lock_guard<std::mutex> g(c->mu);
        auto it = c->free_blocks.find(bytes);
        if (it != c->free_blocks.end()) {
            void *q = it->second.p;
            c->free_blocks.erase(it); c->kept -= bytes;
            c->live[q] = bytes;
            return q;
        }
        static const bool on_miss = [] { const char *e = getenv("PYDEM_PLANE_EVICT_ON_MISS"); return e && atoi(e) > 0; }();
        if (on_miss) plane_cache_evict(c, bytes, victims);
    }
    for (void *v : victims) (void)hipFree(v);
    void *q = nullptr;
    hipError_t e = hipMalloc(&q, bytes);
    {
        static const bool dbg = [] { const char *d = getenv("PYDEM_PLANE_DEBUG"); return d && atoi(d) > 0; }();
        if (dbg) fprintf(stderr, "[pydem] plane_take: hipMalloc(%zu)\n", bytes);
    }
    if (e != hipSuccess) {
        (void)hipGetLastError();
        plane_cache_flush(device);
        e = hipMalloc(&q, bytes);
    }
    if (e != hipSuccess) { pydem_set_error("hipMalloc(%zu bytes) failed: %s", bytes, hipGetErrorString(e)); return nullptr; }
    if (bytes >= PLANE_MIN && plane_cache_limit()) {
        PlaneCache *c = plane_cache(device);
        std::lock_guard<std::mutex> g(c->mu);
        c->live[q] = bytes;
    }
    return q;
}

void plane_give(int device, void *q)
{
    if (!q) return;
    PlaneCache *c = plane_cache(device);
    std::vector<void *> victims;
    bool kept = false;
    {
        std::lock_guard<std::mutex> g(c->mu);
        auto it = c->live.find(q);
        if (it != c->live.end()) {
            const size_t bytes = it->second;
            c->live.erase(it);
            if (bytes <= plane_cache_limit()) {
                plane_cache_evict(c, bytes, victims);
                c->free_blocks.emplace(bytes, FreeBlock{q, ++c->clock}); c->kept += bytes;
                kept = true;
            }
        }
    }
    for (void *v : victims) (void)hipFree(v);
    if (!kept) (void)hipFree(q);
}

hipError_t dev_malloc(void **p, size_t bytes)
{
    hipError_t e = hipMalloc(p, bytes);
    if (e != hipSuccess) {
        int device = 0;
        (void)hipGetLastError();
        if (hipGetDevice(&device) == hipSuccess) { plane_cache_flush(device); e = hipMalloc(p, bytes); }
    }
    return e;
}

template <typename T>
int tile_alloc(pydem_tile *t, T **p, size_t count)
{
    if (*p) return 0;
    size_t bytes = count * sizeof(T);
    if (bytes == 0) bytes = sizeof(T);
    void *q = plane_take(t->device, bytes);
    if (!q) return -1;
    t->device_bytes += (int64_t)bytes;
    *p = (T *)q;
    return 0;
}
template int tile_alloc<double>(pydem_tile *, double **, size_t);
template int tile_alloc<uint8_t>(pydem_tile *, uint8_t **, size_t);
template int tile_alloc<int8_t>(pydem_tile *, int8_t **, size_t);
template int tile_alloc<int32_t>(pydem_tile *, int32_t **, size_t);
template int tile_alloc<RowTab>(pydem_tile *, RowTab **, size_t);
template int tile_alloc<uint16_t>(pydem_tile *, uint16_t **, size_t);

#include <map>
#include <time.h>
#include <mutex>
namespace {
struct DevArena { std::mutex busy; void *p = nullptr; size_t bytes = 0; };
std::mutex g_arena_table;
std::map<int, DevArena *> g_arenas;
DevArena *arena_of(int device)
{
    std::lock_guard<std::mutex> g(g_arena_table);
    DevArena *&a = g_arenas[device];
    if (!a) a = new DevArena();
    return a;
}
}

int arena_acquire(int device, ArenaLease *L)
{
    DevArena *a = arena_of(device);
    a->busy.lock();
    L->device = device; L->arena = a; L->base = (char *)a->p; L->bytes = a->bytes; L->off = 0; L->want = 0; L->held = true;
    return 0;
}

void *arena_take(ArenaLease *L, size_t bytes)
{
    const size_t need = (bytes + 255) & ~(size_t)255;
    L->want += need ? need : 256;
    if (L->base && L->off + need <= L->bytes) { void *q = L->base + L->off; L->off += need ? need : 256; return q; }
    void *q = nullptr;
    const hipError_t e = dev_malloc(&q, need ? need : 256);
    if (e != hipSuccess) { pydem_set_error("hipMalloc(%zu bytes) failed: %s", need, hipGetErrorString(e)); return nullptr; }
    L->extra.push_back(q);
    return q;
}

ArenaLease::~ArenaLease()
{
    if (!held) return;
    DevArena *a = static_cast<DevArena *>(arena);
    (void)hipSetDevice(device);
    for (void *q : extra) (void)hipFree(q);
    if (want > a->bytes) {
        if (a->p) (void)hipFree(a->p);
        a->p = nullptr; a->bytes = 0;
        void *q = nullptr;
        if (dev_malloc(&q, want + want / 8) == hipSuccess) { a->p = q; a->bytes = want + want / 8; }
    }
    a->busy.unlock();
}

namespace {

template <typename T>
__global__ void k_line_gather(const T *__restrict__ src, int64_t stride, int64_t count, T *__restrict__ dst)
{
    for (int64_t k = (int64_t)blockIdx.x * blockDim.x + threadIdx.x; k < count; k += (int64_t)gridDim.x * blockDim.x) dst[k] = src[k * stride];
}
template <typename T>
__global__ void k_line_scatter(const T *__restrict__ src, int64_t stride, int64_t count, T *__restrict__ dst)
{
    for (int64_t k = (int64_t)blockIdx.x * blockDim.x + threadIdx.x; k < count; k += (int64_t)gridDim.x * blockDim.x) dst[k * stride] = src[k];
}

__global__ void k_restore_pit_slopes(const int32_t *__restrict__ src, int64_t n, double *mag)
{
    for (int64_t e = (int64_t)blockIdx.x * blockDim.x + threadIdx.x; e < n; e += (int64_t)gridDim.x * blockDim.x)
        if (src[e] >= 0) mag[src[e]] = -1.0;
}

__global__ void k_flat_save(const uint8_t *__restrict__ flats, const double *__restrict__ mag, int64_t NN, int32_t *__restrict__ cells,
                            double *__restrict__ vals, int64_t cap, unsigned long long *count)
{
    for (int64_t c0 = (int64_t)blockIdx.x * blockDim.x; c0 < NN; c0 += (int64_t)gridDim.x * blockDim.x) {
        const int64_t c = c0 + threadIdx.x;
        const bool f = c < NN && flats[c] != 0;
        const unsigned long long b = __ballot(f);
        if (!b) continue;
        const int lane = (int)__lane_id(), leader = __ffsll((long long)b) - 1;
        unsigned long long base = 0;
        if (lane == leader) base = atomicAdd(count, (unsigned long long)__popcll(b));
        base = __shfl(base, leader);
        const int64_t k = (int64_t)base + __popcll(b & ((1ull << lane) - 1ull));
        if (f && cells && k < cap) { cells[k] = (int32_t)c; vals[k] = mag[c]; }
    }
}

__global__ void k_flat_restore(const int32_t *__restrict__ cells, const double *__restrict__ vals, int64_t n, double *__restrict__ mag,
                               uint8_t *__restrict__ flats)
{
    for (int64_t k = (int64_t)blockIdx.x * blockDim.x + threadIdx.x; k < n; k += (int64_t)gridDim.x * blockDim.x) {
        mag[cells[k]] = vals[k];
        flats[cells[k]] = 1;
    }
}

template <typename S>
__global__ void k_convert_to_f64(const S *__restrict__ src, double *__restrict__ dst, int64_t n)
{
    int64_t i = (int64_t)blockIdx.x * blockDim.x + threadIdx.x;
    const int64_t stride = (int64_t)gridDim.x * blockDim.x;
    for (; i < n; i += stride) dst[i] = (double)src[i];
}

__global__ void k_find_flats(const double *__restrict__ mag, uint8_t *__restrict__ flats, int64_t n)
{
    int64_t i = (int64_t)blockIdx.x * blockDim.x + threadIdx.x;
    const int64_t stride = (int64_t)gridDim.x * blockDim.x;
    for (; i < n; i += stride) flats[i] = (mag[i] == -1.0);
}

size_t dtype_size(int dt)
{
    switch (dt) {
        case PYDEM_F64: return 8;
        case PYDEM_F32: return 4;
        case PYDEM_I16: return 2;
        case PYDEM_I32: return 4;
        case PYDEM_U8: return 1;
        case PYDEM_I8: return 1;
    }
    return 0;
}

int field_ptr(pydem_tile *t, int field, void ***pp, size_t *elem)
{
    switch (field) {
        case PYDEM_ELEV: *pp = (void **)&t->elev; *elem = 8; return 0;
        case PYDEM_MAG: *pp = (void **)&t->mag; *elem = 8; return 0;
        case PYDEM_DIRECTION: *pp = (void **)&t->dir; *elem = 8; return 0;
        case PYDEM_FLATS: *pp = (void **)&t->flats; *elem = 1; return 0;
        case PYDEM_SECTION: *pp = (void **)&t->section; *elem = 1; return 0;
        case PYDEM_PROPORTION: *pp = (void **)&t->prop; *elem = 8; return 0;
        case PYDEM_UCA: *pp = (void **)&t->uca; *elem = 8; return 0;
        case PYDEM_TWI: *pp = (void **)&t->twi; *elem = 8; return 0;
        case PYDEM_EDGE_TODO: *pp = (void **)&t->edge_todo; *elem = 1; return 0;
        case PYDEM_EDGE_DONE: *pp = (void **)&t->edge_done; *elem = 1; return 0;
        case PYDEM_WEIGHT: *pp = (void **)&t->weight; *elem = 8; return 0;
        case PYDEM_UCA_WEIGHTED: *pp = (void **)&t->uca_w; *elem = 8; return 0;
    }
    pydem_set_error("unknown field id %d", field);
    return -2;
}

int ensure_field(pydem_tile *t, int field)
{
    void **pp; size_t elem;
    PYDEM_TRY(field_ptr(t, field, &pp, &elem));
    if (*pp) return 0;
    if (elem == 8) return tile_alloc(t, (double **)pp, (size_t)t->NN);
    return tile_alloc(t, (uint8_t **)pp, (size_t)t->NN);
}

}

int tile_pinned(pydem_tile *t, size_t bytes, void **out)
{
    if (t->h_stage_bytes < bytes) {
        if (t->h_stage) { (void)hipHostFree(t->h_stage); t->h_stage = nullptr; t->h_stage_bytes = 0; }
        const size_t want = bytes + bytes / 4 + 4096;
        HIP_TRY(hipHostMalloc(&t->h_stage, want, hipHostMallocDefault));
        t->h_stage_bytes = want;
    }
    *out = t->h_stage;
    return 0;
}

#include <thread>
#include <sys/mman.h>
namespace {
constexpr size_t XFER_CHUNK = (size_t)8 << 20;
constexpr size_t XFER_MIN = (size_t)32 << 20;
constexpr int XFER_TMAX = 16;
struct XferLane { void *pin[2] = {nullptr, nullptr}; hipStream_t stream = nullptr; hipEvent_t ev[2] = {nullptr, nullptr}; };
struct XferPool { std::mutex busy; XferLane lane[XFER_TMAX]; int ready = 0; };
std::mutex g_xfer_table;
std::map<int, XferPool *> g_xfer;

int xfer_threads()
{
    static const int n = [] {
        const char *e = getenv("PYDEM_XFER_THREADS");
        int v = e ? atoi(e) : 8;
        return v < 0 ? 0 : (v > XFER_TMAX ? XFER_TMAX : v);
    }();
    return n;
}

int xfer_pool(int device, int T, XferPool **out)
{
    XferPool *P;
    {
        std::lock_guard<std::mutex> g(g_xfer_table);
        XferPool *&p = g_xfer[device];
        if (!p) p = new XferPool();
        P = p;
    }
    *out = P;
    return 0;
}

int xfer_prepare(XferPool *P, int T)
{
    for (int k = P->ready; k < T; ++k) {
        XferLane &L = P->lane[k];
        for (int b = 0; b < 2; ++b) {
            if (!L.pin[b]) HIP_TRY(hipHostMalloc(&L.pin[b], XFER_CHUNK, hipHostMallocDefault));
            if (!L.ev[b]) HIP_TRY(hipEventCreateWithFlags(&L.ev[b], hipEventDisableTiming));
        }
        if (!L.stream) HIP_TRY(hipStreamCreateWithFlags(&L.stream, hipStreamNonBlocking));
        P->ready = k + 1;
    }
    return 0;
}

hipError_t xfer_lane_run(int device, XferLane &L, char *dev, char *host, size_t bytes, int k, int T, bool to_host)
{
    hipError_t e = hipSetDevice(device);
    if (e != hipSuccess) return e;
    const size_t nchunk = (bytes + XFER_CHUNK - 1) / XFER_CHUNK;
    size_t prev_off = 0, prev_len = 0; int prev_b = -1;
    int it = 0;
    for (size_t c = (size_t)k; c < nchunk; c += (size_t)T, ++it) {
        const int b = it & 1;
        const size_t off = c * XFER_CHUNK, len = (bytes - off < XFER_CHUNK) ? bytes - off : XFER_CHUNK;
        if (!to_host) {
            if (it >= 2 && (e = hipEventSynchronize(L.ev[b])) != hipSuccess) return e;
            memcpy(L.pin[b], host + off, len);
            if ((e = hipMemcpyAsync(dev + off, L.pin[b], len, hipMemcpyHostToDevice, L.stream)) != hipSuccess) return e;
            if ((e = hipEventRecord(L.ev[b], L.stream)) != hipSuccess) return e;
        } else {
            if ((e = hipMemcpyAsync(L.pin[b], dev + off, len, hipMemcpyDeviceToHost, L.stream)) != hipSuccess) return e;
            if ((e = hipEventRecord(L.ev[b], L.stream)) != hipSuccess) return e;
            if (prev_b >= 0) {
                if ((e = hipEventSynchronize(L.ev[prev_b])) != hipSuccess) return e;
                memcpy(host + prev_off, L.pin[prev_b], prev_len);
            }
            prev_b = b; prev_off = off; prev_len = len;
        }
    }
    if (to_host && prev_b >= 0) {
        if ((e = hipEventSynchronize(L.ev[prev_b])) != hipSuccess) return e;
        memcpy(host + prev_off, L.pin[prev_b], prev_len);
    }
    return hipStreamSynchronize(L.stream);
}
}

int tile_plane_copy(pydem_tile *t, void *dev, void *host, size_t bytes, bool to_host)
{
    const int T = xfer_threads();
    if (T == 0 || bytes < XFER_MIN) {
        if (to_host) HIP_TRY(hipMemcpyAsync(host, dev, bytes, hipMemcpyDeviceToHost, t->stream));
        else HIP_TRY(hipMemcpyAsync(dev, host, bytes, hipMemcpyHostToDevice, t->stream));
        HIP_TRY(hipStreamSynchronize(t->stream));
        return 0;
    }
    HIP_TRY(hipStreamSynchronize(t->stream));
    if (to_host) {
        const uintptr_t a = ((uintptr_t)host + 4095) & ~(uintptr_t)4095, b = ((uintptr_t)host + bytes) & ~(uintptr_t)4095;
        if (b > a) (void)madvise((void *)a, b - a, MADV_HUGEPAGE);
    }
    XferPool *P;
    PYDEM_TRY(xfer_pool(t->device, T, &P));
    std::lock_guard<std::mutex> g(P->busy);
    PYDEM_TRY(xfer_prepare(P, T));
    hipError_t err[XFER_TMAX];
    std::thread th[XFER_TMAX];
    for (int k = 1; k < T; ++k)
        th[k] = std::thread([&, k] { err[k] = xfer_lane_run(t->device, P->lane[k], (char *)dev, (char *)host, bytes, k, T, to_host); });
    err[0] = xfer_lane_run(t->device, P->lane[0], (char *)dev, (char *)host, bytes, 0, T, to_host);
    for (int k = 1; k < T; ++k) th[k].join();
    for (int k = 0; k < T; ++k)
        if (err[k] != hipSuccess) { pydem_set_error("plane transfer: %s", hipGetErrorString(err[k])); return -1; }
    return 0;
}

int ensure_fields(pydem_tile *t, std::initializer_list<int> fields)
{
    for (int f : fields) PYDEM_TRY(ensure_field(t, f));
    return 0;
}

extern "C" {

const char *pydem_hip_last_error(void) { return g_err; }

int pydem_hip_release_scratch(void)
{
    std::vector<std::pair<int, DevArena *>> all;
    {
        std::lock_guard<std::mutex> g(g_arena_table);
        for (auto &kv : g_arenas) all.push_back(kv);
    }
    for (auto &kv : all) {
        std::lock_guard<std::mutex> b(kv.second->busy);
        if (kv.second->p) { (void)hipSetDevice(kv.first); (void)hipFree(kv.second->p); kv.second->p = nullptr; kv.second->bytes = 0; }
    }
    std::vector<int> devs;
    {
        std::lock_guard<std::mutex> g(g_pc_table);
        for (auto &kv : g_pc) devs.push_back(kv.first);
    }
    for (int d : devs) { (void)hipSetDevice(d); plane_cache_flush(d); }
    std::vector<std::pair<int, XferPool *>> pools;
    {
        std::lock_guard<std::mutex> g(g_xfer_table);
        for (auto &kv : g_xfer) pools.push_back(kv);
    }
    for (auto &kv : pools) {
        std::lock_guard<std::mutex> b(kv.second->busy);
        (void)hipSetDevice(kv.first);
        for (int k = 0; k < kv.second->ready; k++) {
            XferLane &L = kv.second->lane[k];
            for (int q = 0; q < 2; q++) {
                if (L.pin[q]) { (void)hipHostFree(L.pin[q]); L.pin[q] = nullptr; }
                if (L.ev[q]) { (void)hipEventDestroy(L.ev[q]); L.ev[q] = nullptr; }
            }
            if (L.stream) { (void)hipStreamDestroy(L.stream); L.stream = nullptr; }
        }
        kv.second->ready = 0;
    }
    return 0;
}

int pydem_hip_device_count(int *count)
{
    HIP_TRY(hipGetDeviceCount(count));
    return 0;
}

int pydem_hip_device_memory(int device, int64_t *free_bytes, int64_t *total_bytes)
{
    size_t f = 0, tot = 0;
    HIP_TRY(hipSetDevice(device));
    HIP_TRY(hipMemGetInfo(&f, &tot));
    if (free_bytes) *free_bytes = (int64_t)f;
    if (total_bytes) *total_bytes = (int64_t)tot;
    return 0;
}

int pydem_hip_device_name(int device, char *buf, int buflen)
{
    hipDeviceProp_t p;
    HIP_TRY(hipGetDeviceProperties(&p, device));
    snprintf(buf, buflen, "%s (%s, %d CUs)", p.name, p.gcnArchName, p.multiProcessorCount);
    return 0;
}

int pydem_tile_create(int64_t n_rows, int64_t n_cols, int device, pydem_tile **out)
{
    if (n_rows < 3 || n_cols < 3) { pydem_set_error("tile must be at least 3x3 (got %lld x %lld)", (long long)n_rows, (long long)n_cols); return -2; }
    if (n_rows * n_cols >= (int64_t)INT32_MAX) { pydem_set_error("tile too large for int32 cell ids"); return -2; }
    HIP_TRY(hipSetDevice(device));
    pydem_tile *t = new pydem_tile();
    t->n = n_rows; t->m = n_cols; t->NN = n_rows * n_cols; t->device = device;
    HIP_TRY(hipStreamCreateWithFlags(&t->stream, hipStreamNonBlocking));
    HIP_TRY(hipStreamCreateWithFlags(&t->stream2, hipStreamNonBlocking));
    HIP_TRY(hipEventCreateWithFlags(&t->ev_fork, hipEventDisableTiming));
    HIP_TRY(hipEventCreateWithFlags(&t->ev_join, hipEventDisableTiming));
    HIP_TRY(hipEventCreateWithFlags(&t->ev_snap, hipEventDisableTiming));
    for (int i = 0; i < 8; i++) HIP_TRY(hipEventCreate(&t->ev[i]));
    PYDEM_TRY(tile_alloc(t, &t->counters, 64));
    HIP_TRY(hipHostMalloc((void **)&t->h_counters, 64 * sizeof(int32_t), hipHostMallocDefault));
    *out = t;
    return 0;
}

int pydem_tile_destroy(pydem_tile *t)
{
    if (!t) return 0;
    (void)hipSetDevice(t->device);
    (void)hipStreamSynchronize(t->stream);
    if (t->stream2) (void)hipStreamSynchronize(t->stream2);
    void *ptrs[] = {t->elev, t->mag, t->dir, t->prop, t->uca, t->twi, t->weight, t->uca_w, t->flats, t->edge_todo, t->edge_done,
                    t->flat0, t->section, t->dX, t->dY, t->dX2, t->dY2, t->rowtab, t->sec_theta, t->row_area, t->inmask,
                    t->gflags, t->todo_work, t->indeg, t->queue[0], t->queue[1], t->labels, t->flatlist,
                    t->counters, t->scratch, t->pits.src, t->pits.dst, t->pits.w, t->pits.in_src,
                    t->pits.in_dst, t->pits.in_w, t->pits.raw_src, t->pits.raw_dst, t->pits.raw_w,
                    t->estamp, t->edelta, t->p_delta, t->s_data, t->p_flags, t->s_flags, t->line_stage, t->contrib,
                    t->eseed, t->lines_stage, t->pits.sort_buf, t->nd_rec, t->cond_mem, t->cb_mem[0], t->cb_mem[1], t->cb_mem[2]};
    for (void *p : ptrs) if (p) plane_give(t->device, p);
    if (t->h_counters) (void)hipHostFree(t->h_counters);
    if (t->h_strip_d) (void)hipHostFree(t->h_strip_d);
    if (t->h_stage) (void)hipHostFree(t->h_stage);
    if (t->h_strip_f) (void)hipHostFree(t->h_strip_f);
    for (int i = 0; i < 8; i++) if (t->ev[i]) (void)hipEventDestroy(t->ev[i]);
    if (t->ev_fork) (void)hipEventDestroy(t->ev_fork);
    if (t->ev_join) (void)hipEventDestroy(t->ev_join);
    if (t->ev_snap) (void)hipEventDestroy(t->ev_snap);
    if (t->stream2) { (void)hipStreamSynchronize(t->stream2); (void)hipStreamDestroy(t->stream2); }
    if (t->stream) (void)hipStreamDestroy(t->stream);
    delete t;
    return 0;
}

int pydem_tile_set_spacing(pydem_tile *t, const double *dX, const double *dY, const double *dX2, const double *dY2)
{
    HIP_TRY(hipSetDevice(t->device));
    const int64_t n = t->n;
    for (int64_t r = 0; r < n - 1; r++)
        if (!(dX[r] > 0 && dY[r] > 0 && std::isfinite(dX[r]) && std::isfinite(dY[r]))) {
            pydem_set_error("pydem_tile_set_spacing: dX / dY must be finite and > 0 (row %lld: %g, %g)", (long long)r, dX[r], dY[r]);
            return -2;
        }
    for (int64_t r = 0; r < n; r++)
        if (!(dX2[r] * dY2[r] > 0 && std::isfinite(dX2[r] * dY2[r]))) {
            pydem_set_error("pydem_tile_set_spacing: dX2 * dY2 (cell area) must be finite and > 0 (row %lld: %g, %g)", (long long)r, dX2[r], dY2[r]);
            return -2;
        }
    t->h_dX.assign(dX, dX + n - 1); t->h_dY.assign(dY, dY + n - 1);
    t->h_dX2.assign(dX2, dX2 + n); t->h_dY2.assign(dY2, dY2 + n);
    std::vector<RowTab> tab((size_t)(n - 1));
    int exotic = 0;
    for (int64_t r = 0; r < n - 1; r++) {
        RowTab &e = tab[(size_t)r];
        e.dX = dX[r]; e.dY = dY[r];
        e.hyp = sqrt(dX[r] * dX[r] + dY[r] * dY[r]);
        e.thA = atan2(dY[r], dX[r]);
        e.thB = atan2(dX[r], dY[r]);
        e.rdX = 1.0 / e.dX; e.rdY = 1.0 / e.dY; e.rhyp = 1.0 / e.hyp;
        if (!(e.dX > 0x1p-500 && e.dX < 0x1p500 && e.dY > 0x1p-500 && e.dY < 0x1p500 && e.hyp < 0x1p500)) exotic = 1;
    }
    { const char *ev = getenv("PYDEM_STENCIL_EXACT"); if (ev && *ev == '1') exotic = 1; }
    t->stencil_exact_only = exotic;
    std::vector<double> st((size_t)n);
    for (int64_t i = 0; i < n; i++) {
        int64_t r = i - 1;
        if (r < 0) r = 0;
        if (r > n - 3) r = n - 3;
        st[(size_t)i] = atan2(dY[r], dX[r]);
    }
    PYDEM_TRY(tile_alloc(t, &t->dX, (size_t)n)); PYDEM_TRY(tile_alloc(t, &t->dY, (size_t)n));
    PYDEM_TRY(tile_alloc(t, &t->dX2, (size_t)n)); PYDEM_TRY(tile_alloc(t, &t->dY2, (size_t)n));
    PYDEM_TRY(tile_alloc(t, &t->rowtab, (size_t)n)); PYDEM_TRY(tile_alloc(t, &t->sec_theta, (size_t)n));
    HIP_TRY(hipMemcpyAsync(t->dX, dX, (n - 1) * 8, hipMemcpyHostToDevice, t->stream));
    HIP_TRY(hipMemcpyAsync(t->dY, dY, (n - 1) * 8, hipMemcpyHostToDevice, t->stream));
    HIP_TRY(hipMemcpyAsync(t->dX2, dX2, n * 8, hipMemcpyHostToDevice, t->stream));
    HIP_TRY(hipMemcpyAsync(t->dY2, dY2, n * 8, hipMemcpyHostToDevice, t->stream));
    HIP_TRY(hipMemcpyAsync(t->rowtab, tab.data(), (n - 1) * sizeof(RowTab), hipMemcpyHostToDevice, t->stream));
    HIP_TRY(hipMemcpyAsync(t->sec_theta, st.data(), n * 8, hipMemcpyHostToDevice, t->stream));
    HIP_TRY(hipStreamSynchronize(t->stream));
    t->spacing_set = true;
    return 0;
}

int pydem_tile_upload(pydem_tile *t, int field, const void *src, int dtype)
{
    HIP_TRY(hipSetDevice(t->device));
    if (t->einc_ready && field != PYDEM_UCA) PYDEM_TRY(stage_edge_flush(t));
    t->edge_clean = false;
    t->einc_ready = false;
    void **pp; size_t elem;
    PYDEM_TRY(field_ptr(t, field, &pp, &elem));
    PYDEM_TRY(ensure_field(t, field));
    const size_t ds = dtype_size(dtype);
    if (!ds) { pydem_set_error("unknown dtype %d", dtype); return -2; }
    if (ds == elem && (elem == 1 || dtype == PYDEM_F64)) {
        PYDEM_TRY(tile_plane_copy(t, *pp, const_cast<void *>(src), (size_t)t->NN * elem, false));
    } else {
        if (elem != 8) { pydem_set_error("dtype conversion is only supported for float64 fields"); return -2; }
        const size_t bytes = (size_t)t->NN * ds;
        if (t->scratch_bytes < bytes) {
            if (t->scratch) { HIP_TRY(hipFree(t->scratch)); t->device_bytes -= (int64_t)t->scratch_bytes; }
            HIP_TRY(dev_malloc(&t->scratch, bytes));
            t->scratch_bytes = bytes; t->device_bytes += (int64_t)bytes;
        }
        PYDEM_TRY(tile_plane_copy(t, t->scratch, const_cast<void *>(src), bytes, false));
        const int grid = (int)(cdiv(t->NN, 256) < 8192 ? cdiv(t->NN, 256) : 8192);
        double *dst = (double *)*pp;
        switch (dtype) {
            case PYDEM_F32: hipLaunchKernelGGL(k_convert_to_f64<float>, dim3(grid), dim3(256), 0, t->stream, (const float *)t->scratch, dst, t->NN); break;
            case PYDEM_I16: hipLaunchKernelGGL(k_convert_to_f64<int16_t>, dim3(grid), dim3(256), 0, t->stream, (const int16_t *)t->scratch, dst, t->NN); break;
            case PYDEM_I32: hipLaunchKernelGGL(k_convert_to_f64<int32_t>, dim3(grid), dim3(256), 0, t->stream, (const int32_t *)t->scratch, dst, t->NN); break;
            case PYDEM_U8: hipLaunchKernelGGL(k_convert_to_f64<uint8_t>, dim3(grid), dim3(256), 0, t->stream, (const uint8_t *)t->scratch, dst, t->NN); break;
            case PYDEM_I8: hipLaunchKernelGGL(k_convert_to_f64<int8_t>, dim3(grid), dim3(256), 0, t->stream, (const int8_t *)t->scratch, dst, t->NN); break;
            default: pydem_set_error("bad dtype"); return -2;
        }
        HIP_TRY(hipGetLastError());
        HIP_TRY(hipStreamSynchronize(t->stream));
    }
    t->have[field] = true;
    if (field == PYDEM_ELEV) { t->elev_f32 = (dtype == PYDEM_F32); t->elev_dtype = dtype; }
    if (field == PYDEM_ELEV || field == PYDEM_MAG || field == PYDEM_DIRECTION || field == PYDEM_FLATS) t->graph_valid = false;
    return 0;
}

int pydem_tile_download(pydem_tile *t, int field, void *dst)
{
    HIP_TRY(hipSetDevice(t->device));
    void **pp; size_t elem;
    PYDEM_TRY(field_ptr(t, field, &pp, &elem));
    if (!*pp || !t->have[field]) { pydem_set_error("field %d has not been computed or uploaded", field); return -3; }
    if (field == PYDEM_UCA) PYDEM_TRY(stage_edge_flush(t));
    if (field == PYDEM_EDGE_DONE || field == PYDEM_EDGE_TODO) PYDEM_TRY(stage_edge_catchup(t));
    PYDEM_TRY(tile_plane_copy(t, *pp, dst, (size_t)t->NN * elem, true));
    return 0;
}

static int line_copy(pydem_tile *t, int field, int axis, int64_t index, void *host, bool to_host)
{
    HIP_TRY(hipSetDevice(t->device));
    void **pp; size_t elem;
    PYDEM_TRY(field_ptr(t, field, &pp, &elem));
    if (!*pp || !t->have[field]) { pydem_set_error("field %d has not been computed or uploaded", field); return -3; }
    const int64_t lim = axis == 0 ? t->n : t->m;
    if (index < 0) index += lim;
    if (index < 0 || index >= lim || (axis != 0 && axis != 1)) { pydem_set_error("line index out of range"); return -2; }
    if (to_host && (field == PYDEM_UCA || field == PYDEM_EDGE_DONE || field == PYDEM_EDGE_TODO) && !tile_line_watched(t, axis, index))
        PYDEM_TRY(stage_edge_catchup(t));
    char *base = (char *)*pp;
    const size_t nbytes = (size_t)(axis == 0 ? t->m : t->n) * elem;
    void *pin = nullptr;
    PYDEM_TRY(tile_pinned(t, nbytes, &pin));
    void *user = host;
    host = pin;
    if (!to_host) memcpy(pin, user, nbytes);
    if (axis == 0) {
        char *row = base + (size_t)index * t->m * elem;
        if (to_host) HIP_TRY(hipMemcpyAsync(host, row, (size_t)t->m * elem, hipMemcpyDeviceToHost, t->stream));
        else HIP_TRY(hipMemcpyAsync(row, host, (size_t)t->m * elem, hipMemcpyHostToDevice, t->stream));
    } else {
        const int64_t cnt = t->n;
        if (!t->line_stage) PYDEM_TRY(tile_alloc(t, &t->line_stage, (size_t)(t->n > t->m ? t->n : t->m)));
        const int g = (int)(cdiv(cnt, 256) < 64 ? cdiv(cnt, 256) : 64);
        char *col = base + (size_t)index * elem;
        if (to_host) {
            if (elem == 8) hipLaunchKernelGGL(k_line_gather<double>, dim3(g), dim3(256), 0, t->stream, (const double *)col, t->m, cnt, t->line_stage);
            else hipLaunchKernelGGL(k_line_gather<uint8_t>, dim3(g), dim3(256), 0, t->stream, (const uint8_t *)col, t->m, cnt, (uint8_t *)t->line_stage);
            HIP_TRY(hipMemcpyAsync(host, t->line_stage, (size_t)cnt * elem, hipMemcpyDeviceToHost, t->stream));
        } else {
            HIP_TRY(hipMemcpyAsync(t->line_stage, host, (size_t)cnt * elem, hipMemcpyHostToDevice, t->stream));
            if (elem == 8) hipLaunchKernelGGL(k_line_scatter<double>, dim3(g), dim3(256), 0, t->stream, (const double *)t->line_stage, t->m, cnt, (double *)col);
            else hipLaunchKernelGGL(k_line_scatter<uint8_t>, dim3(g), dim3(256), 0, t->stream, (const uint8_t *)t->line_stage, t->m, cnt, (uint8_t *)col);
        }
        HIP_TRY(hipGetLastError());
    }
    HIP_TRY(hipStreamSynchronize(t->stream));
    if (to_host) memcpy(user, pin, nbytes);
    if (!to_host && (field == PYDEM_ELEV || field == PYDEM_MAG || field == PYDEM_DIRECTION || field == PYDEM_FLATS)) t->graph_valid = false;
    return 0;
}

int pydem_tile_get_line(pydem_tile *t, int field, int axis, int64_t index, void *dst) { return line_copy(t, field, axis, index, dst, true); }

int pydem_tile_get_lines(pydem_tile *t, int count, const int *fields, const int *axes, const int64_t *indices, void *const *dsts)
{
    HIP_TRY(hipSetDevice(t->device));
    const size_t L = (size_t)(t->n > t->m ? t->n : t->m);
    if (count > 0 && t->lines_cap < count) {
        if (t->lines_stage) { HIP_TRY(hipFree(t->lines_stage)); t->device_bytes -= (int64_t)((size_t)t->lines_cap * L * 8); }
        const int cap = count < 16 ? 16 : count;
        HIP_TRY(dev_malloc(&t->lines_stage, (size_t)cap * L * 8));
        t->lines_cap = cap; t->device_bytes += (int64_t)((size_t)cap * L * 8);
    }
    void *pin_v = nullptr;
    PYDEM_TRY(tile_pinned(t, (size_t)(count > 0 ? count : 1) * L * 8, &pin_v));
    char *pin = (char *)pin_v;
    std::vector<size_t> nbytes((size_t)(count > 0 ? count : 0));
    for (int k = 0; k < count; k++) {
        void **pp; size_t elem;
        PYDEM_TRY(field_ptr(t, fields[k], &pp, &elem));
        if (!*pp || !t->have[fields[k]]) { pydem_set_error("field %d has not been computed or uploaded", fields[k]); return -3; }
        const int64_t lim = axes[k] == 0 ? t->n : t->m;
        int64_t index = indices[k];
        if (index < 0) index += lim;
        if (index < 0 || index >= lim || (axes[k] != 0 && axes[k] != 1)) { pydem_set_error("line index out of range"); return -2; }
        if ((fields[k] == PYDEM_UCA || fields[k] == PYDEM_EDGE_DONE || fields[k] == PYDEM_EDGE_TODO) && !tile_line_watched(t, axes[k], index))
            PYDEM_TRY(stage_edge_catchup(t));
        char *base = (char *)*pp;
        if (axes[k] == 0) {
            nbytes[(size_t)k] = (size_t)t->m * elem;
            HIP_TRY(hipMemcpyAsync(pin + (size_t)k * L * 8, base + (size_t)index * t->m * elem, (size_t)t->m * elem, hipMemcpyDeviceToHost, t->stream));
        } else {
            const int64_t cnt = t->n;
            const int g = (int)(cdiv(cnt, 256) < 64 ? cdiv(cnt, 256) : 64);
            char *col = base + (size_t)index * elem;
            double *stage = (double *)t->lines_stage + (size_t)k * L;
            if (elem == 8) hipLaunchKernelGGL(k_line_gather<double>, dim3(g), dim3(256), 0, t->stream, (const double *)col, t->m, cnt, stage);
            else hipLaunchKernelGGL(k_line_gather<uint8_t>, dim3(g), dim3(256), 0, t->stream, (const uint8_t *)col, t->m, cnt, (uint8_t *)stage);
            nbytes[(size_t)k] = (size_t)cnt * elem;
            HIP_TRY(hipMemcpyAsync(pin + (size_t)k * L * 8, stage, (size_t)cnt * elem, hipMemcpyDeviceToHost, t->stream));
        }
    }
    HIP_TRY(hipGetLastError());
    HIP_TRY(hipStreamSynchronize(t->stream));
    for (int k = 0; k < count; k++) memcpy(dsts[k], pin + (size_t)k * L * 8, nbytes[(size_t)k]);
    return 0;
}
int pydem_tile_set_line(pydem_tile *t, int field, int axis, int64_t index, const void *src) { return line_copy(t, field, axis, index, (void *)src, false); }

int pydem_tile_synchronize(pydem_tile *t)
{
    HIP_TRY(hipSetDevice(t->device));
    HIP_TRY(hipStreamSynchronize(t->stream));
    return 0;
}

int pydem_tile_timings(pydem_tile *t, pydem_timings *out) { *out = t->tm; return 0; }
int64_t pydem_tile_device_bytes(pydem_tile *t) { return t->device_bytes; }

int pydem_tile_synth_fractal(pydem_tile *t, uint32_t seed, int64_t row0, int64_t col0, int n_octaves,
                             int top_shift, double zmin, double zrange)
{
    HIP_TRY(hipSetDevice(t->device));
    t->graph_valid = false;
    PYDEM_TRY(ensure_field(t, PYDEM_ELEV));
    PYDEM_TRY(stage_synth(t, seed, row0, col0, n_octaves, top_shift, zmin, zrange));
    t->have[PYDEM_ELEV] = true;
    t->elev_f32 = false; t->elev_dtype = PYDEM_F64;
    for (int f = PYDEM_MAG; f < PYDEM_FIELD_COUNT; f++) t->have[f] = false;
    return 0;
}

static int need(pydem_tile *t, int field, const char *what)
{
    if (!t->have[field]) { pydem_set_error("%s: required input field %d is missing", what, field); return -3; }
    return 0;
}

int pydem_slopes_directions(pydem_tile *t)
{
    HIP_TRY(hipSetDevice(t->device));
    if (t->einc_ready) PYDEM_TRY(stage_edge_flush(t));
    t->edge_clean = false;
    t->einc_ready = false;
    PYDEM_TRY(need(t, PYDEM_ELEV, "pydem_slopes_directions"));
    if (!t->spacing_set) { pydem_set_error("pydem_slopes_directions: call pydem_tile_set_spacing first"); return -3; }
    PYDEM_TRY(ensure_fields(t, {PYDEM_MAG, PYDEM_DIRECTION, PYDEM_FLATS}));
    PYDEM_TRY(tile_alloc(t, &t->flat0, (size_t)t->NN));
    t->graph_valid = false;
    PYDEM_TRY(stage_stencil(t));
    PYDEM_TRY(stage_flats(t));
    t->have[PYDEM_MAG] = t->have[PYDEM_DIRECTION] = t->have[PYDEM_FLATS] = true;
    return 0;
}

int pydem_fill_flats(pydem_tile *t, double max_pit_area, int below_sea, double source_tol, int peaks, int pits, int artefacts_only,
                     int *needs_host)
{
    t->edge_clean = false;
    t->einc_ready = false;
    HIP_TRY(hipSetDevice(t->device));
    PYDEM_TRY(need(t, PYDEM_ELEV, "pydem_fill_flats"));
    t->graph_valid = false;
    const int r = stage_fill_flats(t, max_pit_area, below_sea, source_tol, peaks, pits, artefacts_only);
    if (r < 0) return r;
    if (needs_host) *needs_host = r;
    for (int f = PYDEM_MAG; f < PYDEM_FIELD_COUNT; f++) t->have[f] = false;
    return 0;
}

int pydem_pit_candidates(pydem_tile *t, int below_sea, int64_t *npits)
{
    HIP_TRY(hipSetDevice(t->device));
    PYDEM_TRY(need(t, PYDEM_ELEV, "pydem_pit_candidates"));
    return stage_pit_candidates(t, below_sea, npits);
}

int pydem_pit_candidates_read(pydem_tile *t, int64_t npits, int32_t *cells, double *elev)
{
    HIP_TRY(hipSetDevice(t->device));
    return stage_pit_candidates_read(t, npits, cells, elev);
}

int pydem_pit_paths(pydem_tile *t, const int32_t *order, int64_t npits, int max_iter, int max_dist, double max_dist_XY,
                    int64_t *n_failed, int64_t *iter_used, int64_t *rounds, int *needs_host)
{
    t->edge_clean = false;
    t->einc_ready = false;
    HIP_TRY(hipSetDevice(t->device));
    PYDEM_TRY(need(t, PYDEM_ELEV, "pydem_pit_paths"));
    const int dtype_mode = t->elev_dtype == PYDEM_F64 ? 0 : (t->elev_dtype == PYDEM_F32 ? 2 : 1);
    t->graph_valid = false;
    const int r = stage_pit_paths(t, order, npits, max_iter, max_dist, max_dist_XY, n_failed, iter_used, rounds, dtype_mode);
    if (r < 0) return r;
    if (needs_host) *needs_host = r;
    for (int f = PYDEM_MAG; f < PYDEM_FIELD_COUNT; f++) t->have[f] = false;
    return 0;
}

int pydem_find_flats(pydem_tile *t)
{
    t->edge_clean = false;
    HIP_TRY(hipSetDevice(t->device));
    PYDEM_TRY(need(t, PYDEM_MAG, "pydem_find_flats"));
    PYDEM_TRY(ensure_field(t, PYDEM_FLATS));
    const int grid = (int)(cdiv(t->NN, 256) < 8192 ? cdiv(t->NN, 256) : 8192);
    hipLaunchKernelGGL(k_find_flats, dim3(grid), dim3(256), 0, t->stream, t->mag, t->flats, t->NN);
    HIP_TRY(hipGetLastError());
    HIP_TRY(hipStreamSynchronize(t->stream));
    t->have[PYDEM_FLATS] = true;
    return 0;
}

int pydem_uca(pydem_tile *t, pydem_options *opt)
{
    t->edge_clean = false;
    t->einc_ready = false;
    HIP_TRY(hipSetDevice(t->device));
    PYDEM_TRY(need(t, PYDEM_ELEV, "pydem_uca"));
    PYDEM_TRY(need(t, PYDEM_MAG, "pydem_uca"));
    PYDEM_TRY(need(t, PYDEM_DIRECTION, "pydem_uca"));
    PYDEM_TRY(need(t, PYDEM_FLATS, "pydem_uca"));
    if (!t->spacing_set) { pydem_set_error("pydem_uca: call pydem_tile_set_spacing first"); return -3; }
    PYDEM_TRY(ensure_fields(t, {PYDEM_SECTION, PYDEM_PROPORTION, PYDEM_UCA, PYDEM_EDGE_TODO, PYDEM_EDGE_DONE}));
    PYDEM_TRY(stage_section_graph(t, opt));
    t->graph_valid = true;
    PYDEM_TRY(stage_sweep(t, opt));
    double mn = opt->twi_min_area;
    for (int64_t i = 0; i < t->n; i++) {
        const double a = t->h_dX2[(size_t)i] * t->h_dY2[(size_t)i];
        if (a < mn) mn = a;
    }
    opt->twi_min_area = mn;
    t->have[PYDEM_SECTION] = t->have[PYDEM_PROPORTION] = t->have[PYDEM_UCA] = true;
    t->have[PYDEM_EDGE_TODO] = t->have[PYDEM_EDGE_DONE] = true;
    return 0;
}

static int ensure_graph(pydem_tile *t, pydem_options *opt, const char *who)
{
    if (t->graph_valid) return 0;
    PYDEM_TRY(need(t, PYDEM_ELEV, who));
    PYDEM_TRY(need(t, PYDEM_MAG, who));
    PYDEM_TRY(need(t, PYDEM_DIRECTION, who));
    if (!t->spacing_set) { pydem_set_error("%s: call pydem_tile_set_spacing first", who); return -3; }
    PYDEM_TRY(ensure_fields(t, {PYDEM_SECTION, PYDEM_PROPORTION}));
    PYDEM_TRY(stage_section_graph(t, opt));
    t->graph_valid = true;
    t->have[PYDEM_SECTION] = t->have[PYDEM_PROPORTION] = true;
    return 0;
}

static bool same_graph_options(const pydem_options &a, const pydem_options &b)
{
    if (!a.drain_pits && !b.drain_pits) return true;
    const bool xy = (a.drain_pits_max_dist_XY == b.drain_pits_max_dist_XY) ||
                    (a.drain_pits_max_dist_XY != a.drain_pits_max_dist_XY && b.drain_pits_max_dist_XY != b.drain_pits_max_dist_XY);
    return a.drain_pits == b.drain_pits && a.drain_pits_min_border == b.drain_pits_min_border &&
           a.drain_pits_max_iter == b.drain_pits_max_iter && a.drain_pits_max_dist == b.drain_pits_max_dist && xy;
}

namespace {
struct DevScratch {
    void *p = nullptr;
    ~DevScratch() { if (p) (void)hipFree(p); }
};
}

int pydem_uca_weighted(pydem_tile *t, pydem_options *opt, int scale_by_cell_area)
{
    HIP_TRY(hipSetDevice(t->device));
    PYDEM_TRY(need(t, PYDEM_WEIGHT, "pydem_uca_weighted"));
    const pydem_timings keep = t->tm;
    const bool own_graph = !t->graph_valid || !same_graph_options(t->graph_opt, *opt);
    DevScratch save, planes;
    struct Kept { void *dst; size_t bytes; size_t off; };
    std::vector<Kept> kept;
    int32_t *save_cells = nullptr;
    double *save_vals = nullptr;
    int64_t nsave = 0;
    if (own_graph) {
        PYDEM_TRY(need(t, PYDEM_FLATS, "pydem_uca_weighted"));
        PYDEM_TRY(need(t, PYDEM_MAG, "pydem_uca_weighted"));
        PYDEM_TRY(ensure_fields(t, {PYDEM_EDGE_TODO, PYDEM_EDGE_DONE}));
        unsigned long long *cnt = reinterpret_cast<unsigned long long *>(t->counters + 62);
        const int g = (int)(cdiv(t->NN, 256) < 4096 ? cdiv(t->NN, 256) : 4096);
        HIP_TRY(hipMemsetAsync(cnt, 0, 8, t->stream));
        hipLaunchKernelGGL(k_flat_save, dim3(g), dim3(256), 0, t->stream, (const uint8_t *)t->flats, (const double *)t->mag, t->NN,
                           (int32_t *)nullptr, (double *)nullptr, (int64_t)0, cnt);
        unsigned long long hn = 0;
        HIP_TRY(hipMemcpyAsync(&hn, cnt, 8, hipMemcpyDeviceToHost, t->stream));
        HIP_TRY(hipStreamSynchronize(t->stream));
        nsave = (int64_t)hn;
        if (nsave > 0) {
            HIP_TRY(dev_malloc(&save.p, (size_t)nsave * 12));
            save_vals = (double *)save.p;
            save_cells = (int32_t *)((char *)save.p + (size_t)nsave * 8);
            HIP_TRY(hipMemsetAsync(cnt, 0, 8, t->stream));
            hipLaunchKernelGGL(k_flat_save, dim3(g), dim3(256), 0, t->stream, (const uint8_t *)t->flats, (const double *)t->mag, t->NN,
                               save_cells, save_vals, nsave, cnt);
            HIP_TRY(hipGetLastError());
        }
        size_t off = 0;
        if (t->have[PYDEM_SECTION]) { kept.push_back({t->section, (size_t)t->NN, off}); off += (size_t)t->NN; }
        if (t->have[PYDEM_EDGE_TODO]) { kept.push_back({t->edge_todo, (size_t)t->NN, off}); off += (size_t)t->NN; }
        off = (off + 255) & ~(size_t)255;
        if (t->have[PYDEM_PROPORTION]) { kept.push_back({t->prop, (size_t)t->NN * 8, off}); off += (size_t)t->NN * 8; }
        if (off) HIP_TRY(dev_malloc(&planes.p, off));
        for (const Kept &k : kept)
            HIP_TRY(hipMemcpyAsync((char *)planes.p + k.off, k.dst, k.bytes, hipMemcpyDeviceToDevice, t->stream));
        t->graph_valid = false;
    }
    int rc = own_graph ? ensure_graph(t, opt, "pydem_uca_weighted") : 0;
    if (rc == 0) {
        if (t->einc_ready) rc = stage_edge_flush(t);
        t->einc_ready = false;
    }
    if (rc == 0) rc = ensure_field(t, PYDEM_UCA_WEIGHTED);
    if (rc == 0) rc = stage_uca_weighted(t, opt, scale_by_cell_area);
    t->have[PYDEM_WEIGHT] = false;
    const double w_ms = t->tm.uca_weighted_ms;
    t->tm = keep;
    if (rc == 0) t->tm.uca_weighted_ms = w_ms;
    if (own_graph) {
        if (nsave > 0) {
            const int64_t g = cdiv(nsave, 256);
            hipLaunchKernelGGL(k_flat_restore, dim3((unsigned)(g < 4096 ? g : 4096)), dim3(256), 0, t->stream, (const int32_t *)save_cells,
                               (const double *)save_vals, nsave, t->mag, t->flats);
        }
        for (const Kept &k : kept)
            HIP_TRY(hipMemcpyAsync(k.dst, (char *)planes.p + k.off, k.bytes, hipMemcpyDeviceToDevice, t->stream));
        HIP_TRY(hipGetLastError());
        HIP_TRY(hipStreamSynchronize(t->stream));
        t->graph_valid = false;
    }
    if (rc != 0) return rc;
    t->have[PYDEM_UCA_WEIGHTED] = true;
    return 0;
}

int pydem_build_graph(pydem_tile *t, pydem_options *opt)
{
    HIP_TRY(hipSetDevice(t->device));
    PYDEM_TRY(need(t, PYDEM_FLATS, "pydem_build_graph"));
    PYDEM_TRY(ensure_fields(t, {PYDEM_EDGE_TODO, PYDEM_EDGE_DONE}));
    return ensure_graph(t, opt, "pydem_build_graph");
}

int pydem_uca_edge_update(pydem_tile *t, pydem_options *opt, const double *const data[4],
                          const uint8_t *const done[4], const uint8_t *const todo[4])
{
    HIP_TRY(hipSetDevice(t->device));
    PYDEM_TRY(need(t, PYDEM_UCA, "pydem_uca_edge_update"));
    PYDEM_TRY(need(t, PYDEM_FLATS, "pydem_uca_edge_update"));
    PYDEM_TRY(ensure_fields(t, {PYDEM_EDGE_TODO, PYDEM_EDGE_DONE}));
    PYDEM_TRY(ensure_graph(t, opt, "pydem_uca_edge_update"));
    PYDEM_TRY(stage_edge_update(t, opt, data, done, todo));
    t->have[PYDEM_EDGE_TODO] = t->have[PYDEM_EDGE_DONE] = true;
    return 0;
}

int pydem_uca_edge_round_inc(pydem_tile *t, pydem_options *opt, const double *const data[4],
                             const uint8_t *const done[4], const uint8_t *const todo[4])
{
    HIP_TRY(hipSetDevice(t->device));
    PYDEM_TRY(need(t, PYDEM_UCA, "pydem_uca_edge_round_inc"));
    PYDEM_TRY(need(t, PYDEM_FLATS, "pydem_uca_edge_round_inc"));
    PYDEM_TRY(need(t, PYDEM_EDGE_TODO, "pydem_uca_edge_round_inc"));
    PYDEM_TRY(need(t, PYDEM_EDGE_DONE, "pydem_uca_edge_round_inc"));
    PYDEM_TRY(ensure_graph(t, opt, "pydem_uca_edge_round_inc"));
    PYDEM_TRY(stage_edge_round_inc(t, opt, data, done, todo));
    return 0;
}

int pydem_uca_edge_round_inc_dev(pydem_tile *t, pydem_options *opt)
{
    HIP_TRY(hipSetDevice(t->device));
    PYDEM_TRY(need(t, PYDEM_UCA, "pydem_uca_edge_round_inc_dev"));
    PYDEM_TRY(need(t, PYDEM_FLATS, "pydem_uca_edge_round_inc_dev"));
    PYDEM_TRY(need(t, PYDEM_EDGE_TODO, "pydem_uca_edge_round_inc_dev"));
    PYDEM_TRY(need(t, PYDEM_EDGE_DONE, "pydem_uca_edge_round_inc_dev"));
    PYDEM_TRY(ensure_graph(t, opt, "pydem_uca_edge_round_inc_dev"));
    if (!t->s_data || !t->s_flags) { pydem_set_error("pydem_uca_edge_round_inc_dev: no strips (pydem_board_set_desc + pydem_board_eval first)"); return -3; }
    PYDEM_TRY(stage_edge_round_inc(t, opt, nullptr, nullptr, nullptr));
    return 0;
}

int pydem_uca_edge_flush(pydem_tile *t)
{
    HIP_TRY(hipSetDevice(t->device));
    return stage_edge_flush(t);
}

int pydem_twi(pydem_tile *t, pydem_options *opt)
{
    HIP_TRY(hipSetDevice(t->device));
    PYDEM_TRY(stage_edge_flush(t));
    PYDEM_TRY(need(t, PYDEM_UCA, "pydem_twi"));
    PYDEM_TRY(need(t, PYDEM_MAG, "pydem_twi"));
    PYDEM_TRY(ensure_field(t, PYDEM_TWI));
    PYDEM_TRY(stage_twi(t, opt));
    t->have[PYDEM_TWI] = true;
    return 0;
}

int pydem_tile_pit_edges(pydem_tile *t, int64_t *n, int32_t *src, int32_t *dst, double *w)
{
    HIP_TRY(hipSetDevice(t->device));
    const int64_t nr = t->pits.n_raw;
    std::vector<int32_t> hs((size_t)nr), hd((size_t)nr);
    std::vector<double> hw((size_t)nr);
    if (nr) {
        HIP_TRY(hipMemcpyAsync(hs.data(), t->pits.raw_src, nr * 4, hipMemcpyDeviceToHost, t->stream));
        HIP_TRY(hipMemcpyAsync(hd.data(), t->pits.raw_dst, nr * 4, hipMemcpyDeviceToHost, t->stream));
        HIP_TRY(hipMemcpyAsync(hw.data(), t->pits.raw_w, nr * 8, hipMemcpyDeviceToHost, t->stream));
        HIP_TRY(hipStreamSynchronize(t->stream));
    }
    int64_t k = 0;
    for (int64_t e = 0; e < nr; e++) {
        if (hs[(size_t)e] < 0) continue;
        if (src) { src[k] = hs[(size_t)e]; dst[k] = hd[(size_t)e]; w[k] = hw[(size_t)e]; }
        k++;
    }
    *n = k;
    return 0;
}

int pydem_tile_graph_words(pydem_tile *t, uint32_t *out)
{
    HIP_TRY(hipSetDevice(t->device));
    if (!t->graph_valid || !t->indeg) { pydem_set_error("pydem_tile_graph_words: no flow graph on this tile (pydem_uca / pydem_build_graph first)"); return -3; }
    HIP_TRY(hipMemcpyAsync(out, t->indeg, (size_t)t->NN * 4, hipMemcpyDeviceToHost, t->stream));
    HIP_TRY(hipStreamSynchronize(t->stream));
    for (int64_t c = 0; c < t->NN; c++) out[c] &= 0x7FFFu;
    return 0;
}

int pydem_tile_restore_pit_slopes(pydem_tile *t)
{
    t->edge_clean = false;
    HIP_TRY(hipSetDevice(t->device));
    if (t->pits.n_raw == 0) return 0;
    const int64_t g = cdiv(t->pits.n_raw, 256);
    hipLaunchKernelGGL(k_restore_pit_slopes, dim3((unsigned)(g < 1024 ? g : 1024)), dim3(256), 0, t->stream, t->pits.raw_src,
                       t->pits.n_raw, t->mag);
    HIP_TRY(hipGetLastError());
    HIP_TRY(hipStreamSynchronize(t->stream));
    return 0;
}

int pydem_bench_stencil(pydem_tile *t, int iters, double *avg_ms)
{
    t->edge_clean = false;
    t->einc_ready = false;
    HIP_TRY(hipSetDevice(t->device));
    PYDEM_TRY(need(t, PYDEM_ELEV, "pydem_bench_stencil"));
    if (!t->spacing_set) { pydem_set_error("pydem_bench_stencil: call pydem_tile_set_spacing first"); return -3; }
    PYDEM_TRY(ensure_fields(t, {PYDEM_MAG, PYDEM_DIRECTION}));
    PYDEM_TRY(tile_alloc(t, &t->flat0, (size_t)t->NN));
    return bench_stencil(t, iters, avg_ms);
}

}
```

pydem_amd/csrc/uca.hip:

```cpp
#include "internal.h"
#include <hipcub/hipcub.hpp>
#include <algorithm>
#include <functional>
#include <memory>
#include <thread>
#include <vector>
#include <math.h>
#include <stdlib.h>
#include <string.h>
#include <time.h>

#define PI_D 3.141592653589793

namespace {

constexpr uint32_t CI_OUT1 = 1u << 8, CI_OUT2 = 1u << 9, CI_PIT_OUT = 1u << 10, CI_PIT_IN = 1u << 11;
constexpr int CI_SEC_SHIFT = 12, CI_LEVEL_SHIFT = 15;
constexpr uint32_t CI_LEVEL_INF = 0x1FFFFu, CI_STATIC_MASK = 0x7FFFu;
__device__ __forceinline__ uint32_t ci_level(uint32_t w) { return w >> CI_LEVEL_SHIFT; }
__device__ __forceinline__ int ci_section(uint32_t w) { return (int)((w >> CI_SEC_SHIFT) & 7u); }
__device__ __forceinline__ uint32_t ci_with_level(uint32_t w, uint32_t lv) { return (w & CI_STATIC_MASK) | (lv << CI_LEVEL_SHIFT); }

__device__ __constant__ const int NB_DI[8] = {-1, -1, -1, 0, 0, 1, 1, 1};
__device__ __constant__ const int NB_DJ[8] = {-1, 0, 1, -1, 1, -1, 0, 1};
// ... 2256 lines not shown
    R.flag = 0; R.delta = 0.0; R.seed_round = 0; R.wid = -1;
}

__global__ __launch_bounds__(256) void k_nd_assign(CIncArgs E, int64_t NN, int32_t *counter)
{
    const int64_t n16 = NN / 16;
    const uint4 *v = reinterpret_cast<const uint4 *>(E.edge_done);
    const int lane = threadIdx.x & 63;
    for (int64_t i0 = (int64_t)blockIdx.x * blockDim.x; i0 < n16; i0 += (int64_t)gridDim.x * blockDim.x) {
        const int64_t i = i0 + threadIdx.x;
        const uint4 x = i < n16 ? v[i] : make_uint4(~0u, ~0u, ~0u, ~0u);
        const uint32_t w[4] = {zero_bytes(x.x), zero_bytes(x.y), zero_bytes(x.z), zero_bytes(x.w)};
        const int nz = __popc(w[0]) + __popc(w[1]) + __popc(w[2]) + __popc(w[3]);
        if (__ballot(nz > 0) == 0) continue;
        int incl = nz;
#pragma unroll
        for (int o = 1; o < 64; o <<= 1) { const int t = __shfl_up(incl, o); if (lane >= o) incl += t; }
        int32_t base = 0;
        if (lane == 63) base = atomicAdd(counter, incl);
        int32_t k = __shfl(base, 63) + incl - nz;
#pragma unroll
        for (int q = 0; q < 4; q++) {
            uint32_t z = w[q];
            while (z) { const int b = __ffs((int)z) - 1; z &= z - 1; nd_assign_cell(E, i * 16 + q * 4 + (b >> 3), k++); }
        }
    }
    if (blockIdx.x == 0) for (int64_t c64 = n16 * 16 + threadIdx.x; c64 < NN; c64 += blockDim.x) if (!E.edge_done[c64]) nd_assign_cell(E, c64, atomicAdd(counter, 1));
}

__global__ __launch_bounds__(256) void k_nd_link(CIncArgs E)
{
    const SweepArgs &A = E.G;
    const int m = A.m;
    if (blockIdx.x == 0 && threadIdx.x == 0) {
        NDRec &S = E.rec[E.nd];
        S.cell = -1; S.cw = 0; S.out_id[0] = S.out_id[1] = -1; S.out_slot[0] = S.out_slot[1] = 0; S.cnt = 1 << 30; S.flag = 0; S.delta = 0.0; S.wid = -1;
    }
    for (int32_t k = blockIdx.x * blockDim.x + threadIdx.x; k < E.nd; k += gridDim.x * blockDim.x) {
        NDRec &R = E.rec[k];
        const int32_t c = R.cell;
        const uint32_t cw = R.cw;
        int32_t cnt = 0;
#pragma unroll
        for (int d = 0; d < 8; d++) {
            if (cw & (1u << d)) cnt += E.cid[c + NB_DI[d] * m + NB_DJ[d]] != 0;
            R.in_delta[d] = 0.0;
        }
        if (cw & CI_PIT_IN)
            for (int32_t e = E.pit_off[c].x; e < A.n_pit && A.pin_dst[e] == c; e++) cnt += E.cid[A.pin_src[e]] != 0;
        const int s = ci_section(cw);
        const double p = A.prop[c];
        const int dr[2] = {fe1r(s), fe2r(s)}, dc[2] = {fe1c(s), fe2c(s)};
        const uint32_t has[2] = {cw & CI_OUT1, cw & CI_OUT2};
        for (int j = 0; j < 2; j++) {
            int32_t id = -1; int slot = 0;
            if (has[j]) {
                id = E.cid[c + dr[j] * m + dc[j]] - 1;
                for (int d = 0; d < 8; d++) if (NB_DI[d] == -dr[j] && NB_DJ[d] == -dc[j]) slot = d;
            }
            R.out_id[j] = id; R.out_slot[j] = (uint8_t)slot;
        }
        R.out_w[0] = p; R.out_w[1] = 1 - p;
        if (E.edge_todo[c]) cnt += 1;
        R.cnt = cnt;
    }
}

__global__ void k_cinc_seed(CIncArgs E, const double *__restrict__ sdata, const uint8_t *__restrict__ sdone,
                            const uint8_t *__restrict__ stodo, int L, QE *q, int32_t *nq)
{
    const int n = E.G.n, m = E.G.m;
    const int64_t nper = 2 * (int64_t)m + 2 * (int64_t)(n - 2);
    const int64_t p = (int64_t)blockIdx.x * blockDim.x + threadIdx.x;
    if (p >= nper) return;
    int i, j;
    perim_cell(p, n, m, i, j);
    const int32_t c = i * m + j;
    bool dn = false, td = false;
    double init = 0.0;
    if (j == 0) { dn |= sdone[0 * L + i] != 0; init += sdata[0 * L + i] * (double)(sdone[0 * L + i] != 0); td |= stodo[0 * L + i] != 0; }
    if (j == m - 1) { dn |= sdone[1 * L + i] != 0; init += sdata[1 * L + i] * (double)(sdone[1 * L + i] != 0); td |= stodo[1 * L + i] != 0; }
    if (i == 0) { dn |= sdone[2 * L + j] != 0; init += sdata[2 * L + j] * (double)(sdone[2 * L + j] != 0); td |= stodo[2 * L + j] != 0; }
    if (i == n - 1) { dn |= sdone[3 * L + j] != 0; init += sdata[3 * L + j] * (double)(sdone[3 * L + j] != 0); td |= stodo[3 * L + j] != 0; }
    const bool own_todo = E.edge_todo[c] != 0;
    const bool own_done = E.edge_done[c] != 0;
    const int32_t k = E.cid[c] - 1;
    if (dn) {
        const double d = E.flats[c] ? NAN : init - E.uca[c];
        E.uca[c] += d;
        E.edge_todo[c] = 0;
        if (k >= 0 && !own_done) E.rec[k].seed_round = (uint16_t)E.round16;
        if (k >= 0 && !own_done && !(E.rec[k].flag & NF_FINAL)) {
            NDRec &R = E.rec[k];
            R.delta = d;
            R.flag = (R.flag & NF_NAN) | NF_FINAL | NF_SEED;
            if (d != d) E.nanq[atomicAdd(E.n_nan, 1)] = k;
            if (own_todo) {
                const int32_t old = atomicSub(&R.cnt, 1);
                if (old == 1) { QE e; e.c = k; e.cw = 0; q[agg_slot(nq)] = e; }
            }
        } else if (k >= 0 && !own_done) {
            E.rec[k].delta += d;
            if (d != d) E.nanq[atomicAdd(E.n_nan, 1)] = k;
        }
    } else if (own_todo && !td) {
        E.edge_todo[c] = 0;
        if (k >= 0) {
            const int32_t old = atomicSub(&E.rec[k].cnt, 1);
            if (old == 1) { QE e; e.c = k; e.cw = 0; q[agg_slot(nq)] = e; }
        }
    }
}

__global__ void k_cinc_release_todo(CIncArgs E, QE *q, int32_t *nq)
{
    const int n = E.G.n, m = E.G.m;
    const int64_t nper = 2 * (int64_t)m + 2 * (int64_t)(n - 2);
    const int64_t p = (int64_t)blockIdx.x * blockDim.x + threadIdx.x;
    if (p >= nper) return;
    int i, j;
    perim_cell(p, n, m, i, j);
    const int32_t c = i * m + j;
    const int32_t k = E.cid[c] - 1;
    if (k < 0 || !E.edge_todo[c] || (E.rec[k].flag & NF_FINAL)) return;
    const int32_t old = atomicSub(&E.rec[k].cnt, 1);
    if (old == 1) { QE e; e.c = k; e.cw = 0; q[agg_slot(nq)] = e; }
}

template <typename Push>
__device__ __forceinline__ void cinc_cell(const CIncArgs &E, QE q, Push push)
{
    const int32_t k = q.c;
    NDRec &R = E.rec[k];
    const uint4 *line = reinterpret_cast<const uint4 *>(&R);
    uint4 L[8];
#pragma unroll
    for (int i = 0; i < 8; i++) L[i] = line[i];
    NDRec V;
    __builtin_memcpy(&V, L, sizeof(V));
    const uint32_t cw = V.cw;
    double delta = V.delta;
    if (!(V.flag & NF_FINAL)) {
        double acc = (cw & ND_FLAT) ? NAN : 0.0;
#pragma unroll
        for (int d = 0; d < 8; d++) acc += V.in_delta[d];
        if (cw & CI_PIT_IN) {
            const SweepArgs &A = E.G;
            for (int32_t e = E.pit_off[V.cell].x; e < A.n_pit && A.pin_dst[e] == V.cell; e++) {
                const int32_t ks = E.cid[A.pin_src[e]] - 1;
                if (ks >= 0 && (E.rec[ks].flag & NF_FINAL)) acc += E.rec[ks].delta * A.pin_w[e];
            }
        }
        delta = acc;
        R.delta = acc;
        R.flag = (V.flag & NF_NAN) | NF_FINAL | NF_DONE;
    } else {
        R.flag = V.flag | NF_DONE;
    }
    const int32_t o0 = V.out_id[0] >= 0 ? V.out_id[0] : E.nd, o1 = V.out_id[1] >= 0 ? V.out_id[1] : E.nd;
    E.rec[o0].in_delta[V.out_slot[0]] = delta * V.out_w[0];
    E.rec[o1].in_delta[V.out_slot[1]] = delta * V.out_w[1];
    const int32_t old0 = atomicSub(&E.rec[o0].cnt, 1);
    const int32_t old1 = atomicSub(&E.rec[o1].cnt, 1);
    if (old0 == 1) push(o0, 0u);
    if (old1 == 1) push(o1, 0u);
    if (cw & CI_PIT_OUT) {
        const SweepArgs &A = E.G;
        for (int32_t e = E.pit_off[V.cell].y; e < A.n_pit && A.pit_src[e] == V.cell; e++) {
            const int32_t kt = E.cid[A.pit_dst[e]] - 1;
            if (kt >= 0 && atomicSub(&E.rec[kt].cnt, 1) == 1) push(kt, 0u);
        }
    }
}

__global__ __launch_bounds__(1024) void k_cinc_nan_flood(CIncArgs E)
{
    __shared__ int32_t s_tail;
    if (threadIdx.x == 0) s_tail = *E.n_nan;
    __syncthreads();
    int32_t head = 0, tail = s_tail;
    const int32_t n_origin = tail;
    while (head < tail) {
        for (int32_t q = head + threadIdx.x; q < tail; q += blockDim.x) {
            const int32_t k = E.nanq[q];
            NDRec &R = E.rec[k];
            if (q >= n_origin && R.seed_round == (uint16_t)E.round16) continue;
            if (atomicOr(&R.flag, NF_NAN) & NF_NAN) continue;
            E.uca[R.cell] = NAN;
            for (int o = 0; o < 2; o++) {
                const int32_t t = R.out_id[o];
                if (t >= 0 && !(E.rec[t].flag & NF_NAN)) E.nanq[atomicAdd(&s_tail, 1)] = t;
            }
            if (R.cw & CI_PIT_OUT) {
                const SweepArgs &A = E.G;
                for (int32_t e = E.pit_off[R.cell].y; e < A.n_pit && A.pit_src[e] == R.cell; e++) {
                    const int32_t t = E.cid[A.pit_dst[e]] - 1;
                    if (t >= 0 && !(E.rec[t].flag & NF_NAN)) E.nanq[atomicAdd(&s_tail, 1)] = t;
                }
            }
        }
        __syncthreads();
        head = tail; tail = s_tail;
        __syncthreads();
    }
    if (threadIdx.x == 0) *E.n_nan = 0;
}

__global__ __launch_bounds__(256) void k_cinc_level(CIncArgs E, const QE *__restrict__ qc, QE *__restrict__ qn, int32_t *cnt3, int r)
{
    const int32_t nq = cnt3[r % 3];
    if (blockIdx.x == 0 && threadIdx.x == 0) cnt3[(r + 2) % 3] = 0;
    if (nq == 0) return;
    int32_t *cn = &cnt3[(r + 1) % 3];
    for (int32_t k = blockIdx.x * blockDim.x + threadIdx.x; k < nq; k += gridDim.x * blockDim.x) {
        auto push = [&](int32_t t, uint32_t ct) { QE e; e.c = t; e.cw = ct; qn[agg_slot(cn)] = e; };
        cinc_cell(E, qc[k], push);
    }
}

__global__ __launch_bounds__(1024) void k_cinc_small(CIncArgs E, QE *q0, QE *q1, int32_t *cnt3, int r_start, int32_t *state, int cap)
{
    __shared__ QE s_q[2][SMALL_CAP];
    __shared__ int32_t s_cnt[3];
    int r = r_start;
    int32_t nq = cnt3[r % 3];
    if (nq > 0 && nq <= cap) {
        const QE *qc = (r % 2) ? q1 : q0;
        for (int32_t k = threadIdx.x; k < nq; k += blockDim.x) s_q[r % 2][k] = qc[k];
    }
    if (threadIdx.x == 0) { s_cnt[0] = s_cnt[1] = s_cnt[2] = 0; }
#ifdef PYDEM_EINC_PROF
    long long prof_t[4] = {0, 0, 0, 0}; int prof_n[4] = {0, 0, 0, 0};
#endif
    __syncthreads();
    while (nq > 0 && nq <= cap) {
#ifdef PYDEM_EINC_PROF
        const long long t0 = wall_clock64();
        const int cls = nq <= 8 ? 0 : (nq <= 64 ? 1 : (nq <= 512 ? 2 : 3));
#endif
        int32_t *cn = &s_cnt[(r + 1) % 3];
        if (threadIdx.x == 0) s_cnt[(r + 2) % 3] = 0;
        QE *qn = (r % 2) ? q0 : q1;
        QE *ln = s_q[(r + 1) % 2];
        for (int32_t k = threadIdx.x; k < nq; k += blockDim.x) {
            auto push = [&](int32_t t, uint32_t ct) {
                QE e; e.c = t; e.cw = ct;
                const int32_t slot = agg_slot(cn);
                if (slot < SMALL_CAP) ln[slot] = e;
                else qn[slot] = e;
            };
            cinc_cell(E, s_q[r % 2][k], push);
        }
        __syncthreads();
        nq = *cn;
        r++;
#ifdef PYDEM_EINC_PROF
        prof_t[cls] += wall_clock64() - t0; prof_n[cls]++;
#endif
    }
    if (nq > cap && r > r_start) {
        QE *qg = (r % 2) ? q1 : q0;
        for (int32_t k = threadIdx.x; k < SMALL_CAP; k += blockDim.x) qg[k] = s_q[r % 2][k];
    }
    if (threadIdx.x == 0) {
        cnt3[r % 3] = nq; cnt3[(r + 1) % 3] = 0; cnt3[(r + 2) % 3] = 0;
        state[0] = r;
#ifdef PYDEM_EINC_PROF
        for (int k = 0; k < 4; k++) { atomicAdd(&E.prof[k], prof_n[k]); atomicAdd(&E.prof[4 + k], (int)prof_t[k]); }
#endif
    }
}

__global__ __launch_bounds__(256) void k_cinc_apply(CIncArgs E)
{
    for (int32_t k = blockIdx.x * blockDim.x + threadIdx.x; k < E.nd; k += gridDim.x * blockDim.x) {
        NDRec &R = E.rec[k];
        const uint32_t f = R.flag;
        if ((f & NF_DONE) && !(f & NF_APPLIED)) {
            if (!(f & NF_SEED)) E.uca[R.cell] += R.delta;
            if (E.set_done) E.edge_done[R.cell] = 1;
            R.flag = f | NF_APPLIED;
        }
    }
}

int grid_for(int64_t work, int cap) { const int64_t g = cdiv(work, 256); return (int)(g < cap ? (g > 0 ? g : 1) : cap); }

#include "uca_cond.inl"
#include "uca_cbuild.inl"

}

int stage_section_graph(pydem_tile *t, const pydem_options *opt)
{
    const int n = (int)t->n, m = (int)t->m;
    t->graph_opt = *opt;
    t->edge_clean = false;
    t->einc_ready = false;
    PYDEM_TRY(tile_alloc(t, &t->todo_work, (size_t)t->NN));
    PYDEM_TRY(tile_alloc(t, &t->indeg, (size_t)t->NN));
    const dim3 grid2((unsigned)(cdiv(m, 256) < 64 ? cdiv(m, 256) : 64), (unsigned)(n < 16384 ? n : 16384));
    t->tm.n_pit_edges = 0; t->tm.n_pits_undrained = 0; t->tm.pits_ms = 0;
    t->pits.n_edges = 0; t->pits.n_raw = 0;
    double *corner_sums = (double *)(t->counters + 16);
    HIP_TRY(hipEventRecord(t->ev_fork, t->stream));
    HIP_TRY(hipStreamWaitEvent(t->stream2, t->ev_fork, 0));
    HIP_TRY(hipMemcpyAsync(t->todo_work, t->flats, (size_t)t->NN, hipMemcpyDeviceToDevice, t->stream2));
    HIP_TRY(hipEventRecord(t->ev_snap, t->stream2));
    HIP_TRY(hipStreamWaitEvent(t->stream, t->ev_snap, 0));
    hipLaunchKernelGGL(k_section_proportion, grid2, dim3(256), 0, t->stream2, t->dir, (const uint8_t *)t->todo_work, t->sec_theta,
                       t->NN, n, m, t->elev, t->section, t->prop, (uint32_t *)t->indeg);
    HIP_TRY(hipMemsetAsync(t->counters + 16, 0, 24 * sizeof(int32_t), t->stream2));
    HIP_TRY(hipMemsetAsync(t->edge_todo, 0, (size_t)t->NN, t->stream2));
    HIP_TRY(hipMemsetAsync(t->todo_work, 0, (size_t)t->NN, t->stream2));
    hipLaunchKernelGGL(k_graph_inmask, grid2, dim3(256), 0, t->stream2, t->prop, t->elev, n, m,
                       (uint32_t *)t->indeg, t->edge_todo, t->todo_work, corner_sums);
    HIP_TRY(hipEventRecord(t->ev_join, t->stream2));
    static int graph_serial = -1;
    if (graph_serial < 0) { const char *e = getenv("PYDEM_GRAPH_SERIAL"); graph_serial = e ? atoi(e) : 0; }
    if (graph_serial) HIP_TRY(hipStreamWaitEvent(t->stream, t->ev_join, 0));
    HIP_TRY(hipEventRecord(t->ev[0], t->stream));
    if (opt->drain_pits) PYDEM_TRY(stage_pits(t, opt));
    HIP_TRY(hipEventRecord(t->ev[2], t->stream));
    HIP_TRY(hipStreamWaitEvent(t->stream, t->ev_join, 0));
    if (t->pits.n_edges > 0) {
        hipLaunchKernelGGL(k_graph_add_pits, dim3(grid_for(t->pits.n_edges, 1024)), dim3(256), 0, t->stream, t->pits.src,
                           t->pits.dst, t->pits.w, t->pits.n_edges, n, m, (uint32_t *)t->indeg, corner_sums);
    }
    hipLaunchKernelGGL(k_corner_todo, dim3(1), dim3(64), 0, t->stream, corner_sums, t->elev, n, m, t->edge_todo, t->todo_work);
    HIP_TRY(hipEventRecord(t->ev[3], t->stream));
    HIP_TRY(hipGetLastError());
    HIP_TRY(hipEventSynchronize(t->ev[3]));
    float a = 0, b = 0;
    HIP_TRY(hipEventElapsedTime(&a, t->ev[0], t->ev[2]));
    HIP_TRY(hipEventElapsedTime(&b, t->ev[2], t->ev[3]));
    (void)a;
    t->tm.graph_ms = b;
    return 0;
}

static void fill_sweep_args(pydem_tile *t, SweepArgs &A)
{
    A.cinfo = (uint32_t *)t->indeg; A.prop = t->prop; A.a0 = t->row_area; A.area = t->uca;
    A.contrib = (double2 *)t->contrib; A.todo_work = t->todo_work; A.n = (int)t->n; A.m = (int)t->m;
    A.pit_src = t->pits.src; A.pit_dst = t->pits.dst; A.n_pit = t->pits.n_edges;
    A.pin_dst = t->pits.in_dst; A.pin_src = t->pits.in_src; A.pin_w = t->pits.in_w;
    A.qcap = (int32_t)(t->NN / 2 < INT32_MAX ? t->NN / 2 : INT32_MAX);
    A.err = t->counters + 15;
    A.tile_open = nullptr;
    { const char *e = getenv("PYDEM_TILE_DEBUG"); A.dbg = e ? atoi(e) : 0; }
}

static int64_t reseed_replay_host(std::vector<ReseedHost> &H, std::vector<uint8_t> &done, int n, int m, int maxcount, bool tile_has_nan,
                                  const std::vector<int32_t> &pit_src, const std::vector<int32_t> &pit_dst, const std::vector<double> &pit_w,
                                  const std::vector<int32_t> &pin_dst, const std::vector<int32_t> &pin_src)
{
    const int32_t nU = (int32_t)H.size();
    const int64_t n_pit = (int64_t)pit_src.size();
    static const int DI[8] = {-1, -1, -1, 0, 0, 1, 1, 1}, DJ[8] = {-1, 0, 1, -1, 1, -1, 0, 1};
    auto find = [&](int32_t c) -> int32_t {
        int32_t lo = 0, hi = nU - 1;
        while (lo <= hi) { const int32_t mid = (lo + hi) >> 1; if (H[(size_t)mid].c == c) return mid; if (H[(size_t)mid].c < c) lo = mid + 1; else hi = mid - 1; }
        return -1;
    };
    auto on_edge = [&](int32_t c) { const int i = c / m, j = c - i * m; return i == 0 || i == n - 1 || j == 0 || j == m - 1; };
    auto is_done = [&](int32_t c) -> bool { const int32_t k = find(c); return k < 0 || done[(size_t)k]; };
    done.assign((size_t)nU, 0);
    std::vector<uint8_t> in_cur((size_t)nU, 0);
    std::vector<int32_t> cur, prev;
    int64_t n_done = 0, done_prev = -1;
    for (int count = 2; n_done < nU && count < maxcount && n_done != done_prev; count++) {
        done_prev = n_done;
        double mx = 0.0;
        for (int32_t k = 0; k < nU; k++) if (!done[(size_t)k] && H[(size_t)k].elev > mx) mx = H[(size_t)k].elev;
        if (tile_has_nan) mx = NAN;
        cur.clear();
        for (int32_t k = 0; k < nU; k++) {
            const double v = done[(size_t)k] ? 0.0 : H[(size_t)k].elev;
            if ((v - mx) / mx > -0.01) cur.push_back(k);
        }
        for (int64_t guard = 0; guard < 8 * (int64_t)nU + 64; guard++) {
            for (int32_t k : cur) { if (!done[(size_t)k]) n_done++; done[(size_t)k] = 1; }
            prev.swap(cur); cur.clear();
            for (int32_t k : prev) {
                const ReseedHost &S = H[(size_t)k];
                const int32_t i = S.c;
                int32_t tg[2]; double fc[2]; int nt = 0;
                if (S.cw & (CI_OUT1 | CI_OUT2)) {
                    const int sct = (int)((S.cw >> CI_SEC_SHIFT) & 7u);
                    if (S.cw & CI_OUT1) { tg[nt] = i + fe1r(sct) * m + fe1c(sct); fc[nt] = S.prop; nt++; }
                    if (S.cw & CI_OUT2) { tg[nt] = i + fe2r(sct) * m + fe2c(sct); fc[nt] = 1 - S.prop; nt++; }
                    if (nt == 2 && tg[1] < tg[0]) { std::swap(tg[0], tg[1]); std::swap(fc[0], fc[1]); }
                }
                int64_t e = (S.cw & CI_PIT_OUT) ? S.pout_first : 0;
                for (int q = 0;; q++) {
                    int32_t row; double factor;
                    if (S.cw & CI_PIT_OUT) { if (!(e < n_pit && pit_src[(size_t)e] == i)) break; row = pit_dst[(size_t)e]; factor = pit_w[(size_t)e]; e++; }
                    else { if (q >= nt) break; row = tg[q]; factor = fc[q]; }
                    const int32_t kr = find(row);
                    if (kr < 0) continue;
                    if (done[(size_t)kr] && on_edge(row)) continue;
                    H[(size_t)kr].area += S.area * factor;
                    if (S.td) H[(size_t)kr].td = 1;
                    bool wait = false;
                    const uint32_t cwr = H[(size_t)kr].cw;
                    for (int d = 0; d < 8 && !wait; d++)
                        if ((cwr & (1u << d)) && !is_done(row + DI[d] * m + DJ[d])) wait = true;
                    if (!wait && (cwr & CI_PIT_IN))
                        for (int64_t e2 = H[(size_t)kr].pin_first; e2 < n_pit && pin_dst[(size_t)e2] == row; e2++)
                            if (!is_done(pin_src[(size_t)e2])) { wait = true; break; }
                    if (!wait && !in_cur[(size_t)kr]) { in_cur[(size_t)kr] = 1; cur.push_back(kr); }
                }
            }
            std::sort(cur.begin(), cur.end());
            for (int32_t k : cur) in_cur[(size_t)k] = 0;
            if (cur == prev) break;
        }
        cur.clear();
    }
    return n_done;
}

template <bool WT>
static int sweep_schedule(pydem_tile *t, const pydem_options *opt, double *seed)
{
    const int n = (int)t->n, m = (int)t->m;
    if (m >= (1 << 22)) { pydem_set_error("uca: tiles wider than 4 194 303 columns are not supported (this one has %d)", m); return -2; }
    PYDEM_TRY(tile_alloc(t, &t->queue[0], (size_t)t->NN));
    PYDEM_TRY(tile_alloc(t, &t->queue[1], (size_t)t->NN));
    PYDEM_TRY(tile_alloc(t, &t->row_area, (size_t)t->n));
    PYDEM_TRY(tile_alloc(t, &t->contrib, (size_t)t->NN * 2));
    t->circular_cells = 0;
    int32_t *total = t->counters + 3;
#ifdef PYDEM_SWEEP_QUEUE
    int32_t *cnt3 = t->counters;
    int32_t *nsrc = t->counters + 4;
    int64_t done_prev = 0;
#endif
    HIP_TRY(hipEventRecord(t->ev[0], t->stream));
    HIP_TRY(hipMemsetAsync(t->counters, 0, 16 * sizeof(int32_t), t->stream));
    if (!WT) hipLaunchKernelGGL(k_row_area, dim3((unsigned)cdiv(n, 256)), dim3(256), 0, t->stream, t->dX2, t->dY2, n, t->row_area);
    SweepArgs A;
    fill_sweep_args(t, A);
    if (WT) { A.a0 = seed; A.area = t->uca_w; }
    if (A.n_pit > 0)
        hipLaunchKernelGGL(k_pit_stash, dim3(grid_for(A.n_pit, 2048)), dim3(256), 0, t->stream, A.pin_dst, A.pit_src, A.n_pit, A.area);
    const int tiles_x = (int)cdiv(m, TT), tiles_total = tiles_x * (int)cdiv(n, TH);
    const size_t tiles_pad = ((size_t)tiles_total + 255) & ~(size_t)255;
    const size_t scratch_need = tiles_pad * (1 + 4 + 4 + 4 + 4 + 4) + 64 * sizeof(int32_t);
    if (t->scratch_bytes < scratch_need) {
        if (t->scratch) { HIP_TRY(hipFree(t->scratch)); t->device_bytes -= (int64_t)t->scratch_bytes; }
        HIP_TRY(dev_malloc((void **)&t->scratch, scratch_need));
        t->scratch_bytes = scratch_need; t->device_bytes += (int64_t)scratch_need;
    }
    uint8_t *tile_done = (uint8_t *)t->scratch;
    int32_t *tile_flag = (int32_t *)(tile_done + tiles_pad);
    int32_t *tile_list[2] = {tile_flag + tiles_pad, tile_flag + 2 * tiles_pad};
    int32_t *cntT = t->counters + 56;
    A.tile_open = tile_flag + 3 * tiles_pad;
    static int64_t sym_switch = -1;
    if (sym_switch < 0) { const char *e = getenv("PYDEM_SWEEP_SYM"); sym_switch = e ? atoll(e) : 4096; if (sym_switch < 0) sym_switch = 0; }
    SymArgs Y;
    memset(&Y, 0, sizeof(Y));
    int32_t *symc = tile_flag + 4 * tiles_pad + tiles_pad;
    const bool sym_on = sym_switch > 0 && TH == 32 && t->NN / 2 < ((int64_t)1 << 31);
    if (sym_on) {
        Y.pool0 = (double *)t->queue[0]; Y.pool1 = (double *)t->queue[1];
        Y.nreg = t->NN >= ((int64_t)1 << 22) ? 16 : 2;
        Y.reg_cap = (uint32_t)((t->NN / 2) / (Y.nreg / 2));
        Y.ctr = symc; Y.tile_sym = (uint32_t *)(tile_flag + 4 * tiles_pad); Y.stat = symc + 32;
        HIP_TRY(hipMemsetAsync(Y.tile_sym, 0xff, tiles_pad * 4, t->stream));
        HIP_TRY(hipMemsetAsync(symc, 0, 64 * sizeof(int32_t), t->stream));
    }
    HIP_TRY(hipMemsetAsync(tile_done, 0, tiles_pad * 5, t->stream));
    HIP_TRY(hipMemsetAsync(A.tile_open, 0x7f, tiles_pad * 4, t->stream));
    HIP_TRY(hipMemsetAsync(cntT, 0, 4 * sizeof(int32_t), t->stream));
    if (A.dbg & 4) HIP_TRY(hipMemsetAsync(t->counters + 32, 0, 24 * sizeof(int32_t), t->stream));
    int64_t launches = 0;
    uint32_t pass = 0;
    int32_t *work16 = t->counters + 16, *work3 = t->counters + 16;
    HIP_TRY(hipMemsetAsync(work16, 0, 16 * sizeof(int32_t), t->stream));
    static int lds_pad = -1;
    if (lds_pad < 0) { const char *e = getenv("PYDEM_TILE_LDS_PAD"); lds_pad = e ? atoi(e) : 0; }
    static int res_switch = -1;
    if (res_switch < 0) { const char *e = getenv("PYDEM_SWEEP_RESIDENT"); res_switch = e ? atoi(e) : 4096; }
    int64_t listed_left = 0;
    auto run_listed = [&](int p, int64_t ntiles, int64_t stop_at) -> int {
        TileNext N;
        N.flag = tile_flag;
        listed_left = ntiles;
        while (ntiles > stop_at) {
            static int dbg_each = -1;
            if (dbg_each < 0) { const char *e = getenv("PYDEM_SWEEP_DEBUG"); dbg_each = (e && atoi(e) >= 2) ? 1 : 0; }
            const int batch = dbg_each ? 1 : ntiles < 2048 ? 16 : 8;
#ifndef PYDEM_LISTED_DYNAMIC
            const int grid = (int)(ntiles < 8192 ? (ntiles > 64 ? ntiles : 64) : 8192) * (4 / LWPB);
#else
            const int64_t want = cdiv(ntiles, 4);
            const int grid = (int)(want < 256 * PYDEM_LISTED_OCC ? (want > 16 ? want : 16) : 256 * PYDEM_LISTED_OCC);
#endif
            const bool resident = ntiles <= res_switch;
            for (int b = 0; b < batch; b++, p++) {
                N.list = tile_list[(p + 1) % 2]; N.count = &cntT[(p + 1) % 3];
                if (resident)
                    hipLaunchKernelGGL(HIP_KERNEL_NAME(k_sweep_tiles_resident<WT>), dim3((unsigned)(ntiles > 256 ? ntiles : 256)), dim3(64), 0, t->stream, A, (uint32_t)p, tiles_x,
                                       (const int32_t *)tile_list[p % 2], (const int32_t *)&cntT[p % 3], tile_done, total, N,
                                       &cntT[(p + 2) % 3], Y);
                else
                    hipLaunchKernelGGL(HIP_KERNEL_NAME(k_sweep_tiles_listed<WT>), dim3(grid), dim3(64 * LWPB), (size_t)lds_pad, t->stream, A, (uint32_t)p, tiles_x,
                                       (const int32_t *)tile_list[p % 2], (const int32_t *)&cntT[p % 3], tile_done, total, N,
                                       &cntT[(p + 2) % 3], work3, Y);
                launches++;
            }
            if (hipMemcpyAsync(t->h_counters, t->counters, 64 * sizeof(int32_t), hipMemcpyDeviceToHost, t->stream) != hipSuccess) return -1;
            if (hipStreamSynchronize(t->stream) != hipSuccess) return -1;
            ntiles = t->h_counters[56 + p % 3];
            listed_left = ntiles;
            if (getenv("PYDEM_SWEEP_DEBUG")) fprintf(stderr, "listed tile pass %d: %lld tiles listed next, processed %d\n", p, (long long)ntiles, t->h_counters[3]);
            if (p > (int)CI_LEVEL_INF - 256) return -2;
        }
        return p;
    };
    auto replay_unfinished = [&](uint32_t pass) -> int {
        HIP_TRY(hipMemcpyAsync(t->h_counters, t->counters, 64 * sizeof(int32_t), hipMemcpyDeviceToHost, t->stream));
        HIP_TRY(hipStreamSynchronize(t->stream));
        if ((int64_t)t->h_counters[3] >= t->NN) return 0;
        {
            ReseedCell *U = (ReseedCell *)t->queue[0];
            const int64_t cap64 = std::min<int64_t>(t->NN * 4 / (int64_t)sizeof(ReseedCell), (int64_t)1 << 22);
            uint8_t *stf = (uint8_t *)t->queue[1];
            int32_t *rc = t->counters + 60;
            HIP_TRY(hipMemsetAsync(rc, 0, 3 * sizeof(int32_t), t->stream));
            hipLaunchKernelGGL(k_reseed_collect, dim3(grid_for(t->NN, 4096)), dim3(256), 0, t->stream, A, U, rc, (int32_t)cap64,
                               (const double *)t->elev, rc + 1);
            HIP_TRY(hipMemcpyAsync(t->h_counters, t->counters, 64 * sizeof(int32_t), hipMemcpyDeviceToHost, t->stream));
            HIP_TRY(hipStreamSynchronize(t->stream));
            const int64_t unfinished = (int64_t)t->h_counters[60];
            if (unfinished == 0) {
                pydem_set_error("sweep: %lld cells were scheduled but never processed (PYDEM_SWEEP_MODE=queue does not support this tile's "
                                "circular drainage; use the default schedule)", (long long)(t->NN - (int64_t)t->h_counters[3]));
                return -5;
            }
            t->circular_cells = unfinished;
            static int64_t host_above = -1;
            if (host_above < 0) { const char *e = getenv("PYDEM_RESEED_HOST_ABOVE"); host_above = e ? atoll(e) : ((int64_t)1 << 22); }
            if (unfinished > cap64 || unfinished > host_above) {
                fprintf(stderr, "pydem: circular drainage with %lld unfinished cells: the re-seed loop runs on the host\n", (long long)unfinished);
                if (unfinished > INT32_MAX / 2) { pydem_set_error("circular drainage: %lld unfinished cells", (long long)unfinished); return -5; }
                const int32_t nU = (int32_t)unfinished;
                void *d_tmp = nullptr;
                HIP_TRY(dev_malloc((void **)&d_tmp, (size_t)nU * (sizeof(ReseedCell) + sizeof(ReseedHost))));
                ReseedCell *U2 = (ReseedCell *)d_tmp;
                ReseedHost *dH = (ReseedHost *)((char *)d_tmp + (size_t)nU * sizeof(ReseedCell));
                HIP_TRY(hipMemsetAsync(rc, 0, 3 * sizeof(int32_t), t->stream));
                hipLaunchKernelGGL(k_reseed_collect, dim3(grid_for(t->NN, 4096)), dim3(256), 0, t->stream, A, U2, rc, nU, (const double *)t->elev, rc + 1);
                hipLaunchKernelGGL(HIP_KERNEL_NAME(k_reseed_gather<WT>), dim3(grid_for(nU, 1024)), dim3(256), 0, t->stream, A, (const ReseedCell *)U2, nU, (const double *)t->elev, dH);
                std::vector<ReseedHost> H((size_t)nU);
                HIP_TRY(hipMemcpyAsync(H.data(), dH, (size_t)nU * sizeof(ReseedHost), hipMemcpyDeviceToHost, t->stream));
                HIP_TRY(hipMemcpyAsync(t->h_counters, t->counters, 64 * sizeof(int32_t), hipMemcpyDeviceToHost, t->stream));
                HIP_TRY(hipStreamSynchronize(t->stream));
                const bool has_nan = t->h_counters[61] != 0;
                std::sort(H.begin(), H.end(), [](const ReseedHost &a, const ReseedHost &b) { return a.c < b.c; });
                const size_t np = (size_t)A.n_pit;
                std::vector<int32_t> h_ps(np), h_pd(np), h_is(np), h_id(np); std::vector<double> h_pw(np);
                if (np) {
                    HIP_TRY(hipMemcpy(h_ps.data(), A.pit_src, np * 4, hipMemcpyDeviceToHost));
                    HIP_TRY(hipMemcpy(h_pd.data(), A.pit_dst, np * 4, hipMemcpyDeviceToHost));
                    HIP_TRY(hipMemcpy(h_pw.data(), t->pits.w, np * 8, hipMemcpyDeviceToHost));
                    HIP_TRY(hipMemcpy(h_id.data(), A.pin_dst, np * 4, hipMemcpyDeviceToHost));
                    HIP_TRY(hipMemcpy(h_is.data(), A.pin_src, np * 4, hipMemcpyDeviceToHost));
                }
                std::vector<uint8_t> dn;
                const int64_t n_done = reseed_replay_host(H, dn, n, m, (int)opt->circular_ref_maxcount, has_nan, h_ps, h_pd, h_pw, h_id, h_is);
                std::vector<ReseedBack> back((size_t)nU);
                for (int32_t k = 0; k < nU; k++) { back[(size_t)k].c = H[(size_t)k].c; back[(size_t)k].area = H[(size_t)k].area; back[(size_t)k].flags = (dn[(size_t)k] ? 1 : 0) | (H[(size_t)k].td ? 2 : 0); }
                static_assert(sizeof(ReseedBack) <= sizeof(ReseedHost), "the gather buffer is reused for the results");
                HIP_TRY(hipMemcpy(dH, back.data(), (size_t)nU * sizeof(ReseedBack), hipMemcpyHostToDevice));
                hipLaunchKernelGGL(k_reseed_scatter, dim3(grid_for(nU, 1024)), dim3(256), 0, t->stream, A, (const ReseedBack *)dH, nU, pass);
                HIP_TRY(hipStreamSynchronize(t->stream));
                HIP_TRY(hipFree(d_tmp));
                t->h_counters[3] += (int32_t)n_done;
                HIP_TRY(hipMemcpy(t->counters + 3, t->h_counters + 3, sizeof(int32_t), hipMemcpyHostToDevice));
                if (getenv("PYDEM_SWEEP_DEBUG")) fprintf(stderr, "circular drainage: %lld unfinished cells, %lld finished by the re-seed replay on the host\n", (long long)unfinished, (long long)n_done);
                return 0;
            }
            std::vector<ReseedCell> hu((size_t)unfinished);
            HIP_TRY(hipMemcpyAsync(hu.data(), U, hu.size() * sizeof(ReseedCell), hipMemcpyDeviceToHost, t->stream));
            HIP_TRY(hipStreamSynchronize(t->stream));
            std::sort(hu.begin(), hu.end(), [](const ReseedCell &a, const ReseedCell &b) { return a.c < b.c; });
            HIP_TRY(hipMemcpyAsync(U, hu.data(), hu.size() * sizeof(ReseedCell), hipMemcpyHostToDevice, t->stream));
            hipLaunchKernelGGL(HIP_KERNEL_NAME(k_reseed_replay<WT>), dim3(1), dim3(64), 0, t->stream, A, (const ReseedCell *)U, (int32_t)unfinished,
                               (const double *)t->elev, (const double *)t->pits.w, stf, stf + unfinished, t->h_counters[61],
                               (int)opt->circular_ref_maxcount, pass, total, rc + 2);
            launches += 2;
            HIP_TRY(hipMemcpyAsync(t->h_counters, t->counters, 64 * sizeof(int32_t), hipMemcpyDeviceToHost, t->stream));
            HIP_TRY(hipStreamSynchronize(t->stream));
            if (getenv("PYDEM_SWEEP_DEBUG")) fprintf(stderr, "circular drainage: %lld unfinished cells, %d finished by the re-seed replay\n", (long long)unfinished, t->h_counters[62]);
        }
        return 0;
    };
#ifdef PYDEM_SWEEP_QUEUE
    static int sweep_mode = -1;
    if (sweep_mode < 0) { const char *e = getenv("PYDEM_SWEEP_MODE"); sweep_mode = (e && !strcmp(e, "queue")) ? 1 : 0; }
    if (WT && sweep_mode == 1) { pydem_set_error("pydem_uca_weighted: PYDEM_SWEEP_MODE=queue is not supported (the weighted sweep runs the tile passes)"); return -6; }
#else
    constexpr int sweep_mode = 0;
#endif
#ifdef PYDEM_SWEEP_STATIC
    const unsigned full_grid = (unsigned)(((tiles_total + 31) / 32) * 8);
#else
    const unsigned full_grid = (unsigned)std::min<int64_t>(((tiles_total + 31) / 32) * 8, 256 * (32 / FWPB));
#endif

    if (sweep_mode == 0) {
        static int first_kind = -1;
        if (first_kind < 0) { const char *e = getenv("PYDEM_SWEEP_FIRST"); first_kind = (e && !strcmp(e, "lds")) ? 1 : 0; }
        static int dense_levels = -1;
        if (dense_levels < 0) { const char *e = getenv("PYDEM_SWEEP_DENSE"); dense_levels = e ? atoi(e) : 0; if (dense_levels < 0) dense_levels = 0; }
        for (int lv = 1; !WT && lv <= dense_levels; lv++) {
            hipLaunchKernelGGL(k_sweep_dense_level, dim3((unsigned)cdiv(m, 256), (unsigned)cdiv(n, DENSE_BAND)), dim3(256), 0, t->stream,
                               A, (uint32_t)lv, total);
            launches++;
        }
        const uint32_t pb = WT ? 0u : (uint32_t)dense_levels;
        if (!WT && first_kind == 1 && TH == 32 && pb == 0)
// ... 1268 lines not shown
```

Baseline: 5651.

## Track flats/mag consistency to skip dense find_flats and fuse flats passes

Adds a flats_rel state that records when the flats field is known to equal (mag == -1). pydem_find_flats can then skip its dense full-tile pass, or patch only the pit cells after slopes are restored. Several passes are also fused: the flat0-to-flats copy goes into the compaction kernel, the separate count kernel is replaced by a change counter inside flats_extend, and the pit mask is combined with its compaction. The state must be invalidated on every path that writes mag or flats, and a missed path would leave flats stale.

Result: no change. 5679 (median of 2 runs) (+0.5%).

```diff
diff --git a/include/pydem_hip.h b/include/pydem_hip.h
--- a/include/pydem_hip.h
+++ b/include/pydem_hip.h
@@ -61,6 +61,7 @@
     int64_t n_pits_row;
     int64_t n_pits_wave;
     int64_t n_pits_big;
+    int64_t n_find_flats_dense;
     double uca_weighted_ms;
 } pydem_timings;
 
diff --git a/pydem_amd/_ffi.py b/pydem_amd/_ffi.py
--- a/pydem_amd/_ffi.py
+++ b/pydem_amd/_ffi.py
@@ -30,7 +30,7 @@
                 ('sweep_kernel_launches', C.c_int64), ('n_flats', C.c_int64), ('n_pit_edges', C.c_int64),
                 ('n_pits_undrained', C.c_int64), ('n_unresolved', C.c_int64), ('sweep_tile_passes', C.c_int64),
                 ('n_pits', C.c_int64), ('n_pits_row', C.c_int64), ('n_pits_wave', C.c_int64), ('n_pits_big', C.c_int64),
-                ('uca_weighted_ms', C.c_double)]
+                ('n_find_flats_dense', C.c_int64), ('uca_weighted_ms', C.c_double)]
 
     def as_dict(self):
         return {k: getattr(self, k) for k, _ in self._fields_}
diff --git a/pydem_amd/csrc/ccl.h b/pydem_amd/csrc/ccl.h
--- a/pydem_amd/csrc/ccl.h
+++ b/pydem_amd/csrc/ccl.h
@@ -2,8 +2,9 @@
 
 #define RLX_LOAD(p) __hip_atomic_load((p), __ATOMIC_RELAXED, __HIP_MEMORY_SCOPE_AGENT)
 
-__global__ __launch_bounds__(256) void k_compact_flats(const uint8_t *__restrict__ flat0, int64_t NN,
-                                                       int32_t *__restrict__ list, int32_t *__restrict__ count)
+template <bool COPY>
+__device__ __forceinline__ void compact_flats_body(const uint8_t *__restrict__ flat0, int64_t NN, int32_t *__restrict__ list,
+                                                   int32_t *__restrict__ count, uint8_t *__restrict__ copy)
 {
     __shared__ int32_t wave_tot[4][4];
     __shared__ int32_t blk_base;
@@ -19,6 +20,10 @@
                 uint4 v[4];
 #pragma unroll
                 for (int q = 0; q < 4; q++) v[q] = *reinterpret_cast<const uint4 *>(flat0 + c0 + 16 * q);
+                if (COPY) {
+#pragma unroll
+                    for (int q = 0; q < 4; q++) *reinterpret_cast<uint4 *>(copy + c0 + 16 * q) = v[q];
+                }
 #pragma unroll
                 for (int q = 0; q < 4; q++) {
                     const uint32_t w[4] = {v[q].x, v[q].y, v[q].z, v[q].w};
@@ -28,7 +33,11 @@
                 }
             } else {
                 for (int k = 0; k < 64; k++)
-                    if (c0 + k < NN && flat0[c0 + k]) bits[j] |= 1ull << k;
+                    if (c0 + k < NN) {
+                        const uint8_t f = flat0[c0 + k];
+                        if (COPY) copy[c0 + k] = f;
+                        if (f) bits[j] |= 1ull << k;
+                    }
             }
             mine[j] = __popcll(bits[j]);
             incl[j] = mine[j];
@@ -62,6 +71,12 @@
         }
         __syncthreads();
     }
+}
+
+__global__ __launch_bounds__(256) void k_compact_flats(const uint8_t *__restrict__ flat0, int64_t NN,
+                                                       int32_t *__restrict__ list, int32_t *__restrict__ count)
+{
+    compact_flats_body<false>(flat0, NN, list, count, nullptr);
 }
 
 __global__ void k_label_init(const int32_t *__restrict__ list, const int32_t *__restrict__ count, int32_t *labels, int m)
diff --git a/pydem_amd/csrc/flats.hip b/pydem_amd/csrc/flats.hip
--- a/pydem_amd/csrc/flats.hip
+++ b/pydem_amd/csrc/flats.hip
@@ -4,11 +4,19 @@
 
 #include "ccl.h"
 
-__global__ void k_flats_extend(const int32_t *__restrict__ list, const int32_t *__restrict__ count,
+__global__ __launch_bounds__(256) void k_compact_copy_flats(const uint8_t *__restrict__ flat0, int64_t NN, int32_t *__restrict__ list,
+                                                            int32_t *__restrict__ count, uint8_t *__restrict__ flats)
+{
+    compact_flats_body<true>(flat0, NN, list, count, flats);
+}
+
+__global__ __launch_bounds__(256) void k_flats_extend(const int32_t *__restrict__ list, const int32_t *__restrict__ count,
                                const uint8_t *__restrict__ flat0, const int32_t *__restrict__ labels,
-                               const double *__restrict__ elev, uint8_t *__restrict__ flats, int n, int m)
+                               const double *__restrict__ elev, uint8_t *__restrict__ flats, int n, int m,
+                               int32_t *__restrict__ turned_off, int32_t *__restrict__ changed)
 {
     const int32_t nf = *count;
+    int32_t local = 0;
     for (int32_t q = blockIdx.x * blockDim.x + threadIdx.x; q < nf * 8; q += gridDim.x * blockDim.x) {
         const int32_t c = list[q >> 3];
         int d = q & 7;
@@ -16,7 +24,8 @@
         const int i = c / m + d / 3 - 1, j = c % m + d % 3 - 1;
         if (i < 0 || i >= n || j < 0 || j >= m) continue;
         const int32_t J = i * m + j;
-        if (!flat0[J] && !(elev[J] == elev[labels[c]])) continue;
+        const bool fJ = flat0[J] != 0;
+        if (!fJ && !(elev[J] == elev[labels[c]])) continue;
         int32_t best = -1;
         for (int dd = 0; dd < 9; dd++) {
             if (dd == 4) continue;
@@ -25,8 +34,25 @@
             const int32_t nb = ii * m + jj;
             if (flat0[nb]) { const int32_t r = labels[nb]; best = r > best ? r : best; }
         }
-        flats[J] = (elev[J] == elev[best]);
+        const bool f = (elev[J] == elev[best]);
+        flats[J] = f;
+        if (f == fJ) continue;
+        if (fJ) *turned_off = 1;
+        int32_t first = -1;
+        for (int dd = 0; dd < 9 && first < 0; dd++) {
+            if (dd == 4) continue;
+            const int ii = i + dd / 3 - 1, jj = j + dd % 3 - 1;
+            if (ii < 0 || ii >= n || jj < 0 || jj >= m) continue;
+            const int32_t nb = ii * m + jj;
+            if (flat0[nb] && (fJ || elev[J] == elev[labels[nb]])) first = nb;
+        }
+        if (first == c) local += f ? 1 : -1;
     }
+    for (int off = 32; off > 0; off >>= 1) local += __shfl_down(local, off);
+    __shared__ int32_t s_w[4];
+    if ((threadIdx.x & 63) == 0) s_w[threadIdx.x >> 6] = local;
+    __syncthreads();
+    if (threadIdx.x == 0) { const int32_t tot = s_w[0] + s_w[1] + s_w[2] + s_w[3]; if (tot) atomicAdd(changed, tot); }
 }
 
 __global__ void k_flats_patch(const int32_t *__restrict__ list, const int32_t *__restrict__ count,
@@ -44,26 +70,6 @@
     }
 }
 
-__global__ __launch_bounds__(256) void k_count_flats(const uint8_t *__restrict__ flats, int64_t NN, int32_t *count)
-{
-    int32_t local = 0;
-    const int64_t nvec = NN >> 4, stride = (int64_t)gridDim.x * blockDim.x, t0 = (int64_t)blockIdx.x * blockDim.x + threadIdx.x;
-    for (int64_t v = t0; v < nvec; v += stride) {
-        const uint4 f4 = reinterpret_cast<const uint4 *>(flats)[v];
-        const uint32_t fw[4] = {f4.x, f4.y, f4.z, f4.w};
-#pragma unroll
-        for (int q = 0; q < 4; q++)
-#pragma unroll
-            for (int b = 0; b < 4; b++) local += ((fw[q] >> (8 * b)) & 0xFFu) != 0;
-    }
-    for (int64_t c = (nvec << 4) + t0; c < NN; c += stride) local += flats[c] != 0;
-    for (int off = 32; off > 0; off >>= 1) local += __shfl_down(local, off);
-    __shared__ int32_t s_w[4];
-    if ((threadIdx.x & 63) == 0) s_w[threadIdx.x >> 6] = local;
-    __syncthreads();
-    if (threadIdx.x == 0) { const int32_t tot = s_w[0] + s_w[1] + s_w[2] + s_w[3]; if (tot) atomicAdd(count, tot); }
-}
-
 }
 
 int stage_flats(pydem_tile *t)
@@ -75,8 +81,7 @@
     HIP_TRY(hipMemsetAsync(t->counters, 0, 64 * sizeof(int32_t), t->stream));
     int32_t *cnt = t->counters;
     const int big = (int)(cdiv(t->NN, 256) < 4096 ? cdiv(t->NN, 256) : 4096);
-    hipLaunchKernelGGL(k_compact_flats, dim3(big), dim3(256), 0, t->stream, t->flat0, t->NN, t->flatlist, cnt);
-    HIP_TRY(hipMemcpyAsync(t->flats, t->flat0, (size_t)t->NN, hipMemcpyDeviceToDevice, t->stream));
+    hipLaunchKernelGGL(k_compact_copy_flats, dim3(big), dim3(256), 0, t->stream, t->flat0, t->NN, t->flatlist, cnt, t->flats);
     HIP_TRY(hipMemcpyAsync(t->h_counters, cnt, sizeof(int32_t), hipMemcpyDeviceToHost, t->stream));
     HIP_TRY(hipStreamSynchronize(t->stream));
     const int32_t nf = t->h_counters[0];
@@ -87,17 +92,17 @@
         hipLaunchKernelGGL(k_label_union, dim3(g1), dim3(256), 0, t->stream, t->flatlist, cnt, t->flat0, t->labels, n, m);
         hipLaunchKernelGGL(k_label_flatten, dim3(g1), dim3(256), 0, t->stream, t->flatlist, cnt, t->labels);
         hipLaunchKernelGGL(k_flats_extend, dim3(g8), dim3(256), 0, t->stream, t->flatlist, cnt, t->flat0, t->labels,
-                           t->elev, t->flats, n, m);
+                           t->elev, t->flats, n, m, cnt + 2, cnt + 1);
         hipLaunchKernelGGL(k_flats_patch, dim3(g8), dim3(256), 0, t->stream, t->flatlist, cnt, t->flats, t->mag, t->dir, n, m);
     }
-    hipLaunchKernelGGL(k_count_flats, dim3(big), dim3(256), 0, t->stream, t->flats, t->NN, cnt + 1);
-    HIP_TRY(hipMemcpyAsync(t->h_counters, cnt, 2 * sizeof(int32_t), hipMemcpyDeviceToHost, t->stream));
+    HIP_TRY(hipMemcpyAsync(t->h_counters, cnt, 3 * sizeof(int32_t), hipMemcpyDeviceToHost, t->stream));
     HIP_TRY(hipEventRecord(t->ev[4], t->stream));
     HIP_TRY(hipGetLastError());
     HIP_TRY(hipEventSynchronize(t->ev[4]));
     float ms = 0;
     HIP_TRY(hipEventElapsedTime(&ms, t->ev[3], t->ev[4]));
     t->tm.flats_ms = ms;
-    t->tm.n_flats = t->h_counters[1];
+    t->tm.n_flats = (int64_t)t->h_counters[0] + t->h_counters[1];
+    t->flats_rel = t->h_counters[2] ? FLATS_REL_UNKNOWN : FLATS_REL_HOLDS;
     return 0;
 }
diff --git a/pydem_amd/csrc/internal.h b/pydem_amd/csrc/internal.h
--- a/pydem_amd/csrc/internal.h
+++ b/pydem_amd/csrc/internal.h
@@ -45,6 +45,8 @@
     void *sort_buf = nullptr; size_t sort_bytes = 0;
 };
 
+enum { FLATS_REL_UNKNOWN = 0, FLATS_REL_HOLDS = 1, FLATS_REL_PITS = 2 };
+
 struct pydem_tile {
     int64_t n = 0, m = 0, NN = 0;
     int device = 0;
@@ -57,6 +59,7 @@
     uint8_t *flats = nullptr, *edge_todo = nullptr, *edge_done = nullptr, *flat0 = nullptr;
     int8_t *section = nullptr;
     bool have[PYDEM_FIELD_COUNT] = {};
+    int flats_rel = FLATS_REL_UNKNOWN;
     double *dX = nullptr, *dY = nullptr, *dX2 = nullptr, *dY2 = nullptr;
     RowTab *rowtab = nullptr;
     double *sec_theta = nullptr;
diff --git a/pydem_amd/csrc/pits.hip b/pydem_amd/csrc/pits.hip
--- a/pydem_amd/csrc/pits.hip
+++ b/pydem_amd/csrc/pits.hip
@@ -1059,84 +1059,89 @@
     }
 }
 
-__global__ void k_pitmask(const uint8_t *__restrict__ flats, const double *__restrict__ elev, int64_t NN, uint8_t *pitmask)
-{
-    const int64_t nvec = NN >> 4, stride = (int64_t)gridDim.x * blockDim.x, t0 = (int64_t)blockIdx.x * blockDim.x + threadIdx.x;
-    for (int64_t v = t0; v < nvec; v += stride) {
-        const uint4 f4 = reinterpret_cast<const uint4 *>(flats)[v];
-        const uint32_t fw[4] = {f4.x, f4.y, f4.z, f4.w};
-        uint32_t pw[4];
-#pragma unroll
-        for (int q = 0; q < 4; q++) {
-            uint32_t p = 0;
-            if (fw[q])
-#pragma unroll
-                for (int b = 0; b < 4; b++)
-                    if (((fw[q] >> (8 * b)) & 0xFFu) && elev[v * 16 + q * 4 + b] > 0) p |= 1u << (8 * b);
-            pw[q] = p;
-        }
-        reinterpret_cast<uint4 *>(pitmask)[v] = make_uint4(pw[0], pw[1], pw[2], pw[3]);
-    }
-    for (int64_t c = (nvec << 4) + t0; c < NN; c += stride) pitmask[c] = flats[c] && (elev[c] > 0);
-}
-
-__global__ __launch_bounds__(256) void k_compact_mask(const uint8_t *__restrict__ mask, int64_t NN,
-                                                       int32_t *__restrict__ list, int32_t *__restrict__ count)
-{
-    __shared__ int32_t wave_tot[4][4];
+__global__ __launch_bounds__(256) void k_pitmask_compact(const uint8_t *__restrict__ flats, const double *__restrict__ elev, int64_t NN,
+                                                          uint8_t *__restrict__ pitmask, int32_t *__restrict__ list,
+                                                          int32_t *__restrict__ count)
+{
+    constexpr int ROWS = 16;
+    __shared__ int32_t wave_tot[ROWS][4];
+    __shared__ int32_t wave_all[4];
     __shared__ int32_t blk_base;
     const int lane = threadIdx.x & 63, wave = threadIdx.x >> 6;
     for (int64_t base = (int64_t)blockIdx.x * 65536; base < NN; base += (int64_t)gridDim.x * 65536) {
-        unsigned long long bits[4];
-        int32_t mine[4], incl[4];
-#pragma unroll
-        for (int j = 0; j < 4; j++) {
-            const int64_t c0 = base + j * 16384 + (int64_t)threadIdx.x * 64;
-            bits[j] = 0;
-            if (c0 + 64 <= NN) {
-                uint4 v[4];
-#pragma unroll
-                for (int q = 0; q < 4; q++) v[q] = *reinterpret_cast<const uint4 *>(mask + c0 + 16 * q);
-#pragma unroll
-                for (int q = 0; q < 4; q++) {
-                    const uint32_t w[4] = {v[q].x, v[q].y, v[q].z, v[q].w};
-#pragma unroll
-                    for (int k = 0; k < 16; k++)
-                        bits[j] |= (unsigned long long)(((w[k >> 2] >> (8 * (k & 3))) & 0xffu) ? 1u : 0u) << (16 * q + k);
-                }
+        uint32_t bits[ROWS];
+#pragma unroll
+        for (int r = 0; r < ROWS; r++) {
+            const int64_t c0 = base + r * 4096 + (int64_t)threadIdx.x * 16;
+            uint32_t b16 = 0;
+            if (c0 + 16 <= NN) {
+                const uint4 f4 = *reinterpret_cast<const uint4 *>(flats + c0);
+                const uint32_t w[4] = {f4.x, f4.y, f4.z, f4.w};
+                double2 e[8];
+#pragma unroll
+                for (int g = 0; g < 4; g++) {
+                    e[2 * g] = e[2 * g + 1] = make_double2(0.0, 0.0);
+                    if (w[g]) {
+                        e[2 * g] = *reinterpret_cast<const double2 *>(elev + c0 + 4 * g);
+                        e[2 * g + 1] = *reinterpret_cast<const double2 *>(elev + c0 + 4 * g + 2);
+                    }
+                }
+                uint32_t pw[4];
+#pragma unroll
+                for (int g = 0; g < 4; g++) {
+                    const double ev[4] = {e[2 * g].x, e[2 * g].y, e[2 * g + 1].x, e[2 * g + 1].y};
+                    uint32_t p = 0;
+#pragma unroll
+                    for (int b = 0; b < 4; b++)
+                        if (((w[g] >> (8 * b)) & 0xFFu) && ev[b] > 0) { p |= 1u << (8 * b); b16 |= 1u << (4 * g + b); }
+                    pw[g] = p;
+                }
+                *reinterpret_cast<uint4 *>(pitmask + c0) = make_uint4(pw[0], pw[1], pw[2], pw[3]);
             } else {
-                for (int k = 0; k < 64; k++)
-                    if (c0 + k < NN && mask[c0 + k]) bits[j] |= 1ull << k;
-            }
-            mine[j] = __popcll(bits[j]);
-            incl[j] = mine[j];
+                for (int k = 0; k < 16; k++)
+                    if (c0 + k < NN) {
+                        const bool p = flats[c0 + k] && (elev[c0 + k] > 0);
+                        pitmask[c0 + k] = p;
+                        if (p) b16 |= 1u << k;
+                    }
+            }
+            bits[r] = b16;
+        }
+        uint32_t incl2[ROWS / 2];
+        int32_t wsum = 0;
+#pragma unroll
+        for (int h = 0; h < ROWS / 2; h++) {
+            uint32_t v = (uint32_t)__popc(bits[2 * h]) | ((uint32_t)__popc(bits[2 * h + 1]) << 16);
 #pragma unroll
             for (int off = 1; off < 64; off <<= 1) {
-                const int32_t o = __shfl_up(incl[j], off);
-                if (lane >= off) incl[j] += o;
-            }
-            if (lane == 63) wave_tot[j][wave] = incl[j];
-        }
+                const uint32_t o = __shfl_up(v, off);
+                if (lane >= off) v += o;
+            }
+            incl2[h] = v;
+            if (lane == 63) { wave_tot[2 * h][wave] = (int32_t)(v & 0xFFFFu); wave_tot[2 * h + 1][wave] = (int32_t)(v >> 16); }
+            wsum += (int32_t)(v & 0xFFFFu) + (int32_t)(v >> 16);
+        }
+        if (lane == 63) wave_all[wave] = wsum;
         __syncthreads();
         if (threadIdx.x == 0) {
-            int32_t tot = 0;
-            for (int j = 0; j < 4; j++) for (int k = 0; k < 4; k++) tot += wave_tot[j][k];
+            const int32_t tot = wave_all[0] + wave_all[1] + wave_all[2] + wave_all[3];
             blk_base = tot ? atomicAdd(count, tot) : 0;
         }
         __syncthreads();
         int32_t off = blk_base;
 #pragma unroll
-        for (int j = 0; j < 4; j++) {
-            int32_t o = off + incl[j] - mine[j];
-            for (int k = 0; k < wave; k++) o += wave_tot[j][k];
-            const int64_t c0 = base + j * 16384 + (int64_t)threadIdx.x * 64;
-            unsigned long long b = bits[j];
+        for (int r = 0; r < ROWS; r++) {
+            const int32_t in = (int32_t)((incl2[r >> 1] >> (16 * (r & 1))) & 0xFFFFu);
+            uint32_t b = bits[r];
+            int32_t o = off + in - __popc(b);
+            for (int k = 0; k < wave; k++) o += wave_tot[r][k];
+            const int64_t c0 = base + r * 4096 + (int64_t)threadIdx.x * 16;
             while (b) {
-                const int k = __ffsll((long long)b) - 1;
+                const int k = __ffs((int)b) - 1;
                 b &= b - 1;
                 list[o++] = (int32_t)(c0 + k);
             }
-            off += wave_tot[j][0] + wave_tot[j][1] + wave_tot[j][2] + wave_tot[j][3];
+            off += wave_tot[r][0] + wave_tot[r][1] + wave_tot[r][2] + wave_tot[r][3];
         }
         __syncthreads();
     }
@@ -1228,10 +1233,8 @@
     PYDEM_TRY(tile_alloc(t, &t->queue[0], (size_t)t->NN));
     int32_t *cnt = t->counters + 40;
     HIP_TRY(hipMemsetAsync(cnt, 0, 16 * sizeof(int32_t), t->stream));
-    const int big = (int)(cdiv(t->NN, 256) < 8192 ? cdiv(t->NN, 256) : 8192);
-    hipLaunchKernelGGL(k_pitmask, dim3(big), dim3(256), 0, t->stream, t->flats, t->elev, t->NN, t->flat0);
-    hipLaunchKernelGGL(k_compact_mask, dim3((unsigned)(cdiv(t->NN, 4096) < 4096 ? cdiv(t->NN, 4096) : 4096)), dim3(256), 0,
-                       t->stream, t->flat0, t->NN, t->flatlist, cnt);
+    hipLaunchKernelGGL(k_pitmask_compact, dim3((unsigned)(cdiv(t->NN, 4096) < 4096 ? cdiv(t->NN, 4096) : 4096)), dim3(256), 0,
+                       t->stream, (const uint8_t *)t->flats, (const double *)t->elev, t->NN, t->flat0, t->flatlist, cnt);
     HIP_TRY(hipMemcpyAsync(t->h_counters, cnt, sizeof(int32_t), hipMemcpyDeviceToHost, t->stream));
     HIP_TRY(hipStreamSynchronize(t->stream));
     const int32_t npits = t->h_counters[0];
diff --git a/pydem_amd/csrc/tile.hip b/pydem_amd/csrc/tile.hip
--- a/pydem_amd/csrc/tile.hip
+++ b/pydem_amd/csrc/tile.hip
@@ -265,6 +265,14 @@
     int64_t i = (int64_t)blockIdx.x * blockDim.x + threadIdx.x;
     const int64_t stride = (int64_t)gridDim.x * blockDim.x;
     for (; i < n; i += stride) flats[i] = (mag[i] == -1.0);
+}
+
+__global__ void k_find_flats_listed(const int32_t *__restrict__ src, int64_t n, const double *__restrict__ mag, uint8_t *__restrict__ flats)
+{
+    for (int64_t e = (int64_t)blockIdx.x * blockDim.x + threadIdx.x; e < n; e += (int64_t)gridDim.x * blockDim.x) {
+        const int32_t c = src[e];
+        if (c >= 0) flats[c] = (mag[c] == -1.0);
+    }
 }
 
 size_t dtype_size(int dt)
@@ -611,6 +619,7 @@
     void **pp; size_t elem;
     PYDEM_TRY(field_ptr(t, field, &pp, &elem));
     PYDEM_TRY(ensure_field(t, field));
+    if (field == PYDEM_MAG || field == PYDEM_FLATS) t->flats_rel = FLATS_REL_UNKNOWN;
     const size_t ds = dtype_size(dtype);
     if (!ds) { pydem_set_error("unknown dtype %d", dtype); return -2; }
     if (ds == elem && (elem == 1 || dtype == PYDEM_F64)) {
@@ -670,6 +679,7 @@
     const size_t nbytes = (size_t)(axis == 0 ? t->m : t->n) * elem;
     void *pin = nullptr;
     PYDEM_TRY(tile_pinned(t, nbytes, &pin));
+    if (!to_host && (field == PYDEM_MAG || field == PYDEM_FLATS)) t->flats_rel = FLATS_REL_UNKNOWN;
     void *user = host;
     host = pin;
     if (!to_host) memcpy(pin, user, nbytes);
@@ -762,6 +772,7 @@
 {
     HIP_TRY(hipSetDevice(t->device));
     t->graph_valid = false;
+    t->flats_rel = FLATS_REL_UNKNOWN;
     PYDEM_TRY(ensure_field(t, PYDEM_ELEV));
     PYDEM_TRY(stage_synth(t, seed, row0, col0, n_octaves, top_shift, zmin, zrange));
     t->have[PYDEM_ELEV] = true;
@@ -787,6 +798,7 @@
     PYDEM_TRY(ensure_fields(t, {PYDEM_MAG, PYDEM_DIRECTION, PYDEM_FLATS}));
     PYDEM_TRY(tile_alloc(t, &t->flat0, (size_t)t->NN));
     t->graph_valid = false;
+    t->flats_rel = FLATS_REL_UNKNOWN;
     PYDEM_TRY(stage_stencil(t));
     PYDEM_TRY(stage_flats(t));
     t->have[PYDEM_MAG] = t->have[PYDEM_DIRECTION] = t->have[PYDEM_FLATS] = true;
@@ -801,6 +813,7 @@
     HIP_TRY(hipSetDevice(t->device));
     PYDEM_TRY(need(t, PYDEM_ELEV, "pydem_fill_flats"));
     t->graph_valid = false;
+    t->flats_rel = FLATS_REL_UNKNOWN;
     const int r = stage_fill_flats(t, max_pit_area, below_sea, source_tol, peaks, pits, artefacts_only);
     if (r < 0) return r;
     if (needs_host) *needs_host = r;
@@ -830,6 +843,7 @@
     PYDEM_TRY(need(t, PYDEM_ELEV, "pydem_pit_paths"));
     const int dtype_mode = t->elev_dtype == PYDEM_F64 ? 0 : (t->elev_dtype == PYDEM_F32 ? 2 : 1);
     t->graph_valid = false;
+    t->flats_rel = FLATS_REL_UNKNOWN;
     const int r = stage_pit_paths(t, order, npits, max_iter, max_dist, max_dist_XY, n_failed, iter_used, rounds, dtype_mode);
     if (r < 0) return r;
     if (needs_host) *needs_host = r;
@@ -842,12 +856,27 @@
     t->edge_clean = false;
     HIP_TRY(hipSetDevice(t->device));
     PYDEM_TRY(need(t, PYDEM_MAG, "pydem_find_flats"));
+    if (t->flats_rel == FLATS_REL_HOLDS && t->flats && t->have[PYDEM_FLATS]) return 0;
+    if (t->flats_rel == FLATS_REL_PITS && t->flats && t->have[PYDEM_FLATS]) {
+        if (t->pits.n_raw > 0) {
+            const int64_t g = cdiv(t->pits.n_raw, 256);
+            hipLaunchKernelGGL(k_find_flats_listed, dim3((unsigned)(g < 4096 ? g : 4096)), dim3(256), 0, t->stream,
+                               (const int32_t *)t->pits.raw_src, t->pits.n_raw, (const double *)t->mag, t->flats);
+            HIP_TRY(hipGetLastError());
+            HIP_TRY(hipStreamSynchronize(t->stream));
+        }
+        t->flats_rel = FLATS_REL_HOLDS;
+        return 0;
+    }
+    t->flats_rel = FLATS_REL_UNKNOWN;
     PYDEM_TRY(ensure_field(t, PYDEM_FLATS));
     const int grid = (int)(cdiv(t->NN, 256) < 8192 ? cdiv(t->NN, 256) : 8192);
     hipLaunchKernelGGL(k_find_flats, dim3(grid), dim3(256), 0, t->stream, t->mag, t->flats, t->NN);
     HIP_TRY(hipGetLastError());
     HIP_TRY(hipStreamSynchronize(t->stream));
     t->have[PYDEM_FLATS] = true;
+    t->flats_rel = FLATS_REL_HOLDS;
+    t->tm.n_find_flats_dense++;
     return 0;
 }
 
@@ -918,7 +947,9 @@
     int32_t *save_cells = nullptr;
     double *save_vals = nullptr;
     int64_t nsave = 0;
+    const int rel_before = t->flats_rel;
     if (own_graph) {
+        t->flats_rel = FLATS_REL_UNKNOWN;
         PYDEM_TRY(need(t, PYDEM_FLATS, "pydem_uca_weighted"));
         PYDEM_TRY(need(t, PYDEM_MAG, "pydem_uca_weighted"));
         PYDEM_TRY(ensure_fields(t, {PYDEM_EDGE_TODO, PYDEM_EDGE_DONE}));
@@ -972,6 +1003,7 @@
         HIP_TRY(hipGetLastError());
         HIP_TRY(hipStreamSynchronize(t->stream));
         t->graph_valid = false;
+        t->flats_rel = (rc == 0 && rel_before == FLATS_REL_HOLDS) ? FLATS_REL_HOLDS : FLATS_REL_UNKNOWN;
     }
     if (rc != 0) return rc;
     t->have[PYDEM_UCA_WEIGHTED] = true;
@@ -1080,6 +1112,7 @@
     t->edge_clean = false;
     HIP_TRY(hipSetDevice(t->device));
     if (t->pits.n_raw == 0) return 0;
+    if (t->flats_rel == FLATS_REL_HOLDS) t->flats_rel = FLATS_REL_PITS;
     const int64_t g = cdiv(t->pits.n_raw, 256);
     hipLaunchKernelGGL(k_restore_pit_slopes, dim3((unsigned)(g < 1024 ? g : 1024)), dim3(256), 0, t->stream, t->pits.raw_src,
                        t->pits.n_raw, t->mag);
@@ -1097,6 +1130,7 @@
     if (!t->spacing_set) { pydem_set_error("pydem_bench_stencil: call pydem_tile_set_spacing first"); return -3; }
     PYDEM_TRY(ensure_fields(t, {PYDEM_MAG, PYDEM_DIRECTION}));
     PYDEM_TRY(tile_alloc(t, &t->flat0, (size_t)t->NN));
+    t->flats_rel = FLATS_REL_UNKNOWN;
     return bench_stencil(t, iters, avg_ms);
 }
 
diff --git a/pydem_amd/csrc/uca.hip b/pydem_amd/csrc/uca.hip
--- a/pydem_amd/csrc/uca.hip
+++ b/pydem_amd/csrc/uca.hip
@@ -2582,6 +2582,7 @@
     const dim3 grid2((unsigned)(cdiv(m, 256) < 64 ? cdiv(m, 256) : 64), (unsigned)(n < 16384 ? n : 16384));
     t->tm.n_pit_edges = 0; t->tm.n_pits_undrained = 0; t->tm.pits_ms = 0;
     t->pits.n_edges = 0; t->pits.n_raw = 0;
+    if (t->flats_rel == FLATS_REL_PITS) t->flats_rel = FLATS_REL_UNKNOWN;
     double *corner_sums = (double *)(t->counters + 16);
     HIP_TRY(hipEventRecord(t->ev_fork, t->stream));
     HIP_TRY(hipStreamWaitEvent(t->stream2, t->ev_fork, 0));
@@ -2600,7 +2601,12 @@
     if (graph_serial < 0) { const char *e = getenv("PYDEM_GRAPH_SERIAL"); graph_serial = e ? atoi(e) : 0; }
     if (graph_serial) HIP_TRY(hipStreamWaitEvent(t->stream, t->ev_join, 0));
     HIP_TRY(hipEventRecord(t->ev[0], t->stream));
-    if (opt->drain_pits) PYDEM_TRY(stage_pits(t, opt));
+    if (opt->drain_pits) {
+        const int rel = t->flats_rel;
+        t->flats_rel = FLATS_REL_UNKNOWN;
+        PYDEM_TRY(stage_pits(t, opt));
+        if (rel == FLATS_REL_HOLDS) t->flats_rel = FLATS_REL_PITS;
+    }
     HIP_TRY(hipEventRecord(t->ev[2], t->stream));
     HIP_TRY(hipStreamWaitEvent(t->stream, t->ev_join, 0));
     if (t->pits.n_edges > 0) {
```
